# henryxrl/Listening-to-Sound-of-Silence-for-Speech-Denoising

Measured on AMD Instinct MI355X. Metric: utterances/sec (2 s clips), training step: detector + denoiser forward/backward/Adam, higher is better.
Workload: dtype fp16

## Files before the change

### include/sos_hip.h

```cpp
#ifndef SOS_HIP_H
#define SOS_HIP_H

#include <stdint.h>

#ifdef __cplusplus
extern "C" {
#endif

typedef void* sos_stream_t;

enum { SOS_OK = 0, SOS_EINVAL = -22, SOS_ELAUNCH = -5, SOS_ENOSPC = -28 };

enum { SOS_ACT_NONE = 0, SOS_ACT_RELU = 1, SOS_ACT_PRELU = 2, SOS_ACT_SIGMOID = 3 };
enum { SOS_PAD_ZERO = 0, SOS_PAD_REFLECT = 1 };
enum { SOS_DT_BF16 = 0, SOS_DT_BF16X3 = 1, SOS_DT_F32 = 2 };

int sos_abi_version(void);
int sos_struct_size(int which);
const char* sos_last_error(void);
const char* sos_storage_dtype(void);

int64_t sos_stft_matrix_bytes(int n_fft, int hop, int win_length);
int sos_stft_pack_matrix(int n_fft, int hop, int win_length, void* hi , void* lo );
int sos_stft_f32(const float* wave, int64_t batch, int64_t n_samples, int64_t wave_stride,
// ... 18 lines not shown
int sos_crm_target_f32(const float* clean, const float* mix, float* out, int64_t batch, int64_t plane,
                       float a, float b, sos_stream_t stream);

int sos_bits_to_mask(const uint8_t* bits, int64_t batch, int64_t n_frames, double ratio,
                     int64_t n_samples, float* mask, const float* sig, float* masked,
                     const int32_t* clip_frames, const int32_t* clip_samples ,
                     sos_stream_t stream);

int sos_add_signals_f32(const float* signal, const float* noises, const float* snr_db, int64_t batch, int n_noises,
                        int64_t n, float norm, float* mixed, float* signal_out, float* noises_out, sos_stream_t stream);

int sos_threshold_bits(const float* logits, int64_t n, float threshold, uint8_t* bits, float* conf,
                       sos_stream_t stream);
int sos_logit_band_mark(const float* logits, const float* scale, int64_t batch, int64_t n, const int32_t* n_valid,
                        float band_rel, const int32_t* tabs_in, int32_t* tabs_out, int ntab, int32_t* mark, int32_t* count,
                        sos_stream_t stream);

int sos_pack_nchw_to_nhwc(const float* in, int64_t B, int C, int64_t H, int64_t W, void* out, int cs,
                          int dtype, const float* mul ,
                          sos_stream_t stream);
int sos_pack_nchw_wtaps(const float* in, int64_t B, int C, int64_t H, int64_t W, int kw, int pad_left, int pad_mode,
                        const int32_t* clip_w, void* out, int cs, int dtype, const float* mul, sos_stream_t stream);

typedef struct sos_conv_desc {
    const void* in;
    int32_t B, H, W;
    int32_t in_cs;
    int32_t cin_off, cin;
    int32_t in_nseg;
    int32_t in_seg_stride;
    const int32_t* w_gather;
    int32_t Wl;
    const void* wgt;
    int32_t kh, kw, cout, cout_pad;
    int32_t stride, dil_h, dil_w, pad_top, pad_left, pad_mode;
    int32_t Ho, Wo;
    void* out;
    int32_t out_dtype;
    int64_t out_sb, out_sh, out_sw, out_sc;
    int32_t out_c_off;
    int32_t cout_store;
    int64_t out_third;
    const float* scale;
    const float* shift;
    int32_t act;
    const float* act_param;
    int32_t accumulate;
    float* stats;
    int32_t stats_c;
    const int32_t* wl_tab;
    const int32_t* wo_tab;
    int32_t w_gather_stride;
    int32_t t_frames, t_taps, t_pad;
    void* fold_pad_out;
    int32_t fold_pad, fold_H, fold_W, fold_sy, fold_oy, fold_sx, fold_ox, fold_row;
    int64_t fold_third;
    const float* in_scale;
    const float* in_shift;
} sos_conv_desc;

int sos_conv2d_fwd(const sos_conv_desc* desc , sos_stream_t stream);
int64_t sos_conv2d_tile_count(const sos_conv_desc* desc);

int sos_conv2d_tune(const sos_conv_desc* desc, int max_candidates, int iters, float* best_ms,
                    sos_stream_t stream);
int sos_conv2d_tune_save(const char* path);
int sos_conv2d_tune_load(const char* path);

int64_t sos_lstm_pack_bytes(int H, int backward);
int sos_lstm_pack_whh(const float* whh, int H, void* fwd_hi, void* fwd_lo, void* bwd_hi, void* bwd_lo,
                      sos_stream_t stream);
int sos_lstm_bidir_fwd(const float* xproj, const void* wpk_hi, const void* wpk_lo , int64_t B, int64_t T,
                       int H, void* out_bf16, int out_cs, int out_dtype, int64_t out_third,
                       float* save_gates ,
                       float* save_c ,
                       const int32_t* lengths ,
                       sos_stream_t stream);

typedef struct sos_view {
    void* ptr;
    int64_t npix;
    int32_t row, c_off, C, x3;
    int64_t third;
} sos_view;

int sos_bn_stats_blocks(int64_t npix);
int sos_bn_stats(const sos_view* x, float* partial, sos_stream_t stream);
int sos_bn_finalize(const float* partial, int nblk, int C, int64_t count, const float* gamma, const float* beta,
                    float eps, float momentum, float* running_mean, float* running_var, int64_t* num_batches_tracked,
                    float* scale, float* shift, float* save_mean, float* save_invstd, sos_stream_t stream);
int sos_bn_act_apply(const sos_view* x, const float* scale, const float* shift, int act, const float* slope,
                     const sos_view* y, int feat_H, int feat_W, int feat_Wo, const int32_t* gather,
                     sos_stream_t stream);

typedef struct sos_wgrad_desc {
    const void* g;
    int32_t B, Hg, Wg, g_cs, g_off;
    const void* x;
    int32_t Hx, Wx, x_cs, x_off;
    int32_t M, N, kh, kw, stride, dil_h, dil_w, pad_top, pad_left, pad_mode;
    int32_t ksplit;
    float* partial;
    float* dw;
    int32_t accumulate;
    float scale;
    const float* scale_dev;
    int32_t t_frames, t_taps, t_pad, t_cin;
} sos_wgrad_desc;
int64_t sos_wgrad_workspace_bytes(const sos_wgrad_desc* desc);
int sos_conv2d_wgrad(const sos_wgrad_desc* desc, sos_stream_t stream);
int sos_conv2d_wgrad_partial(const sos_wgrad_desc* desc, sos_stream_t stream);
int sos_conv2d_wgrad_reduce(const sos_wgrad_desc* desc, sos_stream_t stream);
int sos_wgrad_tune(const sos_wgrad_desc* desc, int iters, float* best_ms, sos_stream_t stream);
int sos_wgrad_tune_save(const char* path);
int sos_wgrad_tune_load(const char* path);

int sos_bn_bwd(const sos_view* dy, const sos_view* x, const float* scale, const float* shift, const float* mean,
               const float* invstd, const float* gamma, int act, const float* slope, float* partial, float* coef,
               float* dgamma, float* dbeta, float* dslope, const sos_view* dx,
               const float* out_scale ,
               sos_stream_t stream);
int sos_act_bwd_from_y(const sos_view* dy, const sos_view* y, int act, const sos_view* dz, sos_stream_t stream);
int sos_pack_grad_f32(const float* g, const float* y, int act, int64_t outer, int64_t inner, int C, int64_t so,
                      int64_t st, int64_t sc, const sos_view* out, const float* mul ,
                      sos_stream_t stream);
int sos_feat_to_nhwc(const sos_view* feat, int B, int H, int W, int Wo, const int32_t* lo, const int32_t* hi,
                     const sos_view* out, sos_stream_t stream);
int sos_lstm_bidir_bwd(const void* dh_out, int dh_cs, int dh_dtype, int64_t dh_third, const float* gates,
                       const float* csave, const void* wtk_hi, const void* wtk_lo , int64_t B, int64_t T,
                       int H, float* dgates, sos_stream_t stream);
int sos_mse_loss(const float* a, const float* b, int64_t n, float upstream, float* loss, float* grad, float* partial,
                 sos_stream_t stream);
int sos_bce_logits_loss(const float* x, const float* y, int64_t n, float upstream, float* loss, float* grad,
                        float* partial, sos_stream_t stream);
int sos_amax_f32(const float* x, int64_t n, float* amax, sos_stream_t stream);
int sos_loss_scale(const float* amax, float target, float* scale2, const float* guard , sos_stream_t stream);
int sos_scale_f32(float* x, int64_t n, const float* s , sos_stream_t stream);
#define SOS_GUARD_FLOATS 5
#define SOS_GUARD_GROWTH 200
int sos_grad_guard(const float* g, int64_t n, float* guard, int finalize, sos_stream_t stream);
int sos_adam_step(float* p, const float* g, float* m, float* v, int64_t n, float lr, float beta1, float beta2,
                  float eps, float weight_decay, int64_t step, float grad_scale, const float* skip, sos_stream_t stream);

#define SOS_ADAM_CHUNK 16384
typedef struct sos_adam_tensor { float* p; const float* g; float* m; float* v; int64_t n; } sos_adam_tensor;
int sos_adam_multi_step(const sos_adam_tensor* tensors, int n_tensors, const int32_t* chunks, int64_t n_chunks, float lr,
                        float beta1, float beta2, float eps, float weight_decay, int64_t step, float grad_scale,
                        const float* skip , sos_stream_t stream);

typedef struct sos_pack_entry { const int64_t* idx; void* out; int64_t n; } sos_pack_entry;
int sos_gather_pack_multi(const sos_pack_entry* entries, int n_entries, const int32_t* chunks, int64_t n_chunks,
                          sos_stream_t stream);

int sos_reflect_fold(const sos_view* padded, int H, int W, int pad, const sos_view* out, int accumulate,
                     sos_stream_t stream);
int sos_reflect_fold_border(const sos_view* padded, int H, int W, int pad, const sos_view* out, sos_stream_t stream);
int sos_copy_crop(const sos_view* src, int Hs, int Ws, const sos_view* dst, int Hd, int Wd, sos_stream_t stream);

enum { SOS_PCM_S16 = 0, SOS_PCM_S32 = 1, SOS_PCM_F32 = 2, SOS_PCM_U8 = 3 };
int sos_pcm_to_mono_f32(const void* pcm, int format, int channels, int64_t n_frames, float* out, sos_stream_t stream);
int sos_resample_f32(const float* x, int64_t n_in, double ratio, const float* win, int nwin, int num_table,
                     float* out, int64_t n_out, sos_stream_t stream);
#define SOS_RESAMPLE_CHUNK 4096
int sos_resample_batch_f32(const float* x, const int64_t* table, const int64_t* table_host, int nclips, double ratio,
                           const float* win, int nwin, int num_table, float* out, sos_stream_t stream);
int sos_resample_time_segments(double ratio, int64_t n_out, int64_t* k0, double* s0, double* d, int capacity);

int sos_time_stack(const void* in, int64_t B, int T, int64_t HW, int C, int in_cs, int nseg, int kt, void* out,
                   int out_cs, sos_stream_t stream);
int sos_spatial_mean(const void* in, int64_t N, int64_t HW, int C, int in_cs, int nseg, void* out, int64_t out_row,
                     int out_third, int out_c_off, sos_stream_t stream);
int sos_time_unstack(const void* d_stacked, int64_t B, int T, int64_t HW, int C, int st_cs, int nseg, int kt,
                     void* d_in, int in_cs, sos_stream_t stream);
int sos_spatial_mean_bwd(const void* dfeat, int64_t N, int64_t HW, int C, int64_t f_row, int f_third, int f_c_off,
                         int nseg, void* dy, int cs, sos_stream_t stream);

int sos_metric_totals(const float* ref, const float* deg, int64_t n, double* out3, sos_stream_t stream);
int sos_metric_frame_energy(const float* ref, const float* deg, int64_t n, int winlength, int skip, int64_t num_frames,
                            const double* window, double* out, sos_stream_t stream);
int sos_metric_compact(const float* clean, const float* proc, int64_t n, float thr, float* out_clean, float* out_proc,
                       int64_t* count, sos_stream_t stream);
int sos_metric_llr(const float* ref, const float* deg, int64_t n, int winlength, int skip, int64_t num_frames,
                   const double* window, int P, float* out, sos_stream_t stream);
int sos_metric_wss(const float* ref, const float* deg, int64_t n, int winlength, int skip, int64_t num_frames,
                   const double* window, int n_fft, const float* crit_filter, double eps, float* out, sos_stream_t stream);
int sos_metric_l1(const float* output, int64_t n_out, const float* target, int64_t n_t, double* result, sos_stream_t stream);

int64_t sos_metric_batch_workspace_bytes(const int64_t* lengths_host, int nclips, int winlength, int skip, int n_fft);
int sos_metric_batch(const float* clean, const float* noisy, const int64_t* offsets, const int64_t* lengths,
                     const int64_t* lengths_host, int nclips, int winlength, int skip, int n_fft, int P, const double* window,
                     const float* crit_filter, double eps, void* workspace, int64_t workspace_bytes, void* out, int64_t out_bytes,
                     sos_stream_t stream);

int64_t sos_stoi_workspace_bytes(const int64_t* lengths_host, int nclips, int p, int q);
int sos_stoi_batch(const float* x, const float* y, const int64_t* offsets, const int64_t* lengths, const int64_t* lengths_host,
                   int nclips, int p, int q, const double* taps, int ntaps, int extended, void* workspace, int64_t workspace_bytes,
                   double* out, sos_stream_t stream);

enum { SOS_SDR_CORRELATE = 1, SOS_SDR_SOLVE = 2 };
int64_t sos_sdr_workspace_bytes(const int64_t* lengths_host, int nclips, int filter_length);
int sos_sisdr_batch(const float* x, const float* y, const int64_t* offsets, const int64_t* lengths, const int64_t* lengths_host,
                    int nclips, int zero_mean, void* workspace, int64_t workspace_bytes, double* out, sos_stream_t stream);
int sos_sdr_batch(const float* x, const float* y, const int64_t* offsets, const int64_t* lengths, const int64_t* lengths_host,
                  int nclips, int filter_length, int stages, void* workspace, int64_t workspace_bytes, double* out,
                  sos_stream_t stream);

int sos_ragged_stage_f32(const float* x, const int64_t* table, const int64_t* table_host, int nclips, const uint8_t* bits,
                         const double* ratios, const double* ratios_host, int64_t stride, float* wave, float* masked,
                         float* mask, sos_stream_t stream);
int sos_ragged_unpack_f32(const float* rows, int64_t n_rows, int64_t stride, const int64_t* table, const int64_t* table_host,
                          int nentries, float* out, sos_stream_t stream);

int64_t sos_silence_label_workspace_bytes(const int64_t* table_host, int nclips);
int sos_silence_label_batch(const float* x, const int64_t* table, const int64_t* table_host, int nclips, const double* params,
                            const double* params_host, void* workspace, int64_t workspace_bytes, uint8_t* bits, double* energy,
                            double* out, sos_stream_t stream);

#define SOS_MIX_CHUNK 4096
int64_t sos_ragged_mix_workspace_bytes(const int64_t* table_host, int nclips);
int sos_ragged_mix_f32(const float* clips, const int64_t* table, const int64_t* table_host, int nclips, const float* noise,
                       int64_t noise_total, const int64_t* noise_table, const int64_t* noise_table_host, const uint8_t* bits,
                       const double* params, const double* params_host, double norm, void* workspace, int64_t workspace_bytes,
                       float* mixed, float* clean, float* noise_out, double* out, sos_stream_t stream);

int sos_window_stage_f32(const float* x, int64_t total, const int64_t* table, const int64_t* table_host, int nwin, int64_t stride,
                         float* rows, sos_stream_t stream);
int sos_window_stitch_f32(const float* rows, int64_t n_rows, int64_t stride, const int64_t* table, const int64_t* table_host,
                          int nwin, int64_t context, float* out, sos_stream_t stream);

int sos_window_stitch_planes_f32(const float* rows, int planes, int64_t n_rows, int64_t stride, const int64_t* table,
                                 const int64_t* table_host, int nwin, int64_t context, const int64_t* recs,
                                 const int64_t* recs_host, int nrec, int64_t out_total, float* out, sos_stream_t stream);

int sos_window_frames_stitch_f32(const float* rows, int64_t n_rows, int64_t stride, const int64_t* table, const int64_t* table_host,
                                 const int64_t* frames, const int64_t* frames_host, int nwin, const int64_t* recs,
                                 const int64_t* recs_host, const double* ratios, const double* ratios_host, int nrec, int64_t core,
                                 int64_t context, float* out, sos_stream_t stream);
int sos_window_stage_masked_f32(const float* x, const uint8_t* bits, const int64_t* clips, const int64_t* clips_host,
                                const double* ratios, const double* ratios_host, int nrec, const int64_t* table,
                                const int64_t* table_host, int nwin, int64_t stride, float* wave, float* masked,
                                sos_stream_t stream);

int sos_stream_push_f32(const float* flat, int64_t total, const int64_t* table, const int64_t* table_host, int nrows, float* ring,
                        int64_t slots, int64_t cap, sos_stream_t stream);
int sos_stream_stage_f32(const float* ring, int64_t slots, int64_t cap, const int64_t* table, const int64_t* table_host, int nwin,
                         int64_t stride, float* rows, sos_stream_t stream);
int sos_stream_stitch_f32(const float* rows, int64_t n_rows, int64_t stride, const int64_t* table, const int64_t* table_host,
                          int nwin, int64_t slots, int64_t context, float* tail, float* out, int64_t out_stride,
                          sos_stream_t stream);

#ifdef __cplusplus
}
#endif
#endif
```

### listening-to-sound-of-silence-for-speech-denoising_amd/_lib.py

```python
import ctypes as C
import os

_HERE = os.path.dirname(os.path.abspath(__file__))
LIB_PATH = os.environ.get("SOS_HIP_LIB", os.path.join(_HERE, "libsos_hip.so"))
LIB_PATH_F16 = os.environ.get("SOS_HIP_LIB_F16", os.path.join(_HERE, "libsos_hip_f16.so"))

ACT_NONE, ACT_RELU, ACT_PRELU, ACT_SIGMOID = 0, 1, 2, 3
PAD_ZERO, PAD_REFLECT = 0, 1
DT_BF16, DT_BF16X3, DT_F32 = 0, 1, 2
SDR_CORRELATE, SDR_SOLVE = 1, 2


class ConvDesc(C.Structure):
    _fields_ = [
        ("in_", C.c_void_p),
        ("B", C.c_int32), ("H", C.c_int32), ("W", C.c_int32),
        ("in_cs", C.c_int32), ("cin_off", C.c_int32), ("cin", C.c_int32),
        ("in_nseg", C.c_int32), ("in_seg_stride", C.c_int32),
        ("w_gather", C.c_void_p), ("Wl", C.c_int32),
        ("wgt", C.c_void_p),
        ("kh", C.c_int32), ("kw", C.c_int32), ("cout", C.c_int32), ("cout_pad", C.c_int32),
        ("stride", C.c_int32), ("dil_h", C.c_int32), ("dil_w", C.c_int32),
        ("pad_top", C.c_int32), ("pad_left", C.c_int32), ("pad_mode", C.c_int32),
        ("Ho", C.c_int32), ("Wo", C.c_int32),
        ("out", C.c_void_p), ("out_dtype", C.c_int32),
        ("out_sb", C.c_int64), ("out_sh", C.c_int64), ("out_sw", C.c_int64), ("out_sc", C.c_int64),
        ("out_c_off", C.c_int32), ("cout_store", C.c_int32), ("out_third", C.c_int64),
        ("scale", C.c_void_p), ("shift", C.c_void_p),
        ("act", C.c_int32), ("act_param", C.c_void_p), ("accumulate", C.c_int32),
        ("stats", C.c_void_p), ("stats_c", C.c_int32),
        ("wl_tab", C.c_void_p), ("wo_tab", C.c_void_p), ("w_gather_stride", C.c_int32),
        ("t_frames", C.c_int32), ("t_taps", C.c_int32), ("t_pad", C.c_int32),
        ("fold_pad_out", C.c_void_p),
        ("fold_pad", C.c_int32), ("fold_H", C.c_int32), ("fold_W", C.c_int32), ("fold_sy", C.c_int32), ("fold_oy", C.c_int32),
        ("fold_sx", C.c_int32), ("fold_ox", C.c_int32), ("fold_row", C.c_int32), ("fold_third", C.c_int64),
        ("in_scale", C.c_void_p), ("in_shift", C.c_void_p),
    ]


class View(C.Structure):
    _fields_ = [("ptr", C.c_void_p), ("npix", C.c_int64), ("row", C.c_int32), ("c_off", C.c_int32),
                ("C", C.c_int32), ("x3", C.c_int32), ("third", C.c_int64)]


class WgradDesc(C.Structure):
    _fields_ = [("g", C.c_void_p), ("B", C.c_int32), ("Hg", C.c_int32), ("Wg", C.c_int32), ("g_cs", C.c_int32),
                ("g_off", C.c_int32), ("x", C.c_void_p), ("Hx", C.c_int32), ("Wx", C.c_int32), ("x_cs", C.c_int32),
                ("x_off", C.c_int32), ("M", C.c_int32), ("N", C.c_int32), ("kh", C.c_int32), ("kw", C.c_int32),
                ("stride", C.c_int32), ("dil_h", C.c_int32), ("dil_w", C.c_int32), ("pad_top", C.c_int32),
                ("pad_left", C.c_int32), ("pad_mode", C.c_int32), ("ksplit", C.c_int32), ("partial", C.c_void_p),
                ("dw", C.c_void_p), ("accumulate", C.c_int32), ("scale", C.c_float), ("scale_dev", C.c_void_p),
                ("t_frames", C.c_int32), ("t_taps", C.c_int32), ("t_pad", C.c_int32), ("t_cin", C.c_int32)]


_P, _I, _L, _F, _D = C.c_void_p, C.c_int, C.c_int64, C.c_float, C.c_double
ADAM_CHUNK = 16384
GUARD_FLOATS = 5
RESAMPLE_CHUNK = 4096
MIX_CHUNK = 4096
EXPECTED_ABI = 10

SIGNATURES = {
    "sos_abi_version": [],
    "sos_struct_size": [_I],
    "sos_stft_matrix_bytes": [_I, _I, _I],
    "sos_stft_pack_matrix": [_I, _I, _I, _P, _P],
    "sos_stft_f32": [_P, _L, _L, _L, _P, _P, _I, _I, _I, _P, _L, _P, _P],
    "sos_istft_matrix_bytes": [_I, _I, _I],
    "sos_istft_pack_matrix": [_I, _I, _I, _P, _P, _P],
    "sos_istft_f32": [_P, _L, _L, _P, _P, _P, _I, _I, _I, _P, _L, _P, _P],
    "sos_power_law_f32": [_P, _L, _F, _P, _P],
    "sos_crm_apply_f32": [_P, _P, _P, _L, _L, _F, _F, _P],
    "sos_crm_apply_bwd_f32": [_P, _P, _P, _P, _L, _L, _F, _P],
    "sos_crm_target_f32": [_P, _P, _P, _L, _L, _F, _F, _P],
    "sos_bits_to_mask": [_P, _L, _L, _D, _L, _P, _P, _P, _P, _P, _P],
    "sos_threshold_bits": [_P, _L, _F, _P, _P, _P],
    "sos_logit_band_mark": [_P, _P, _L, _L, _P, _F, _P, _P, _I, _P, _P, _P],
    "sos_add_signals_f32": [_P, _P, _P, _L, _I, _L, _F, _P, _P, _P, _P],
    "sos_storage_dtype": [],
    "sos_pack_nchw_to_nhwc": [_P, _L, _I, _L, _L, _P, _I, _I, _P, _P],
    "sos_pack_nchw_wtaps": [_P, _L, _I, _L, _L, _I, _I, _I, _P, _P, _I, _I, _P, _P],
    "sos_conv2d_fwd": [C.POINTER(ConvDesc), _P],
    "sos_conv2d_tune": [C.POINTER(ConvDesc), _I, _I, C.POINTER(C.c_float), _P],
    "sos_conv2d_tune_save": [C.c_char_p],
    "sos_conv2d_tune_load": [C.c_char_p],
    "sos_conv2d_tile_count": [C.POINTER(ConvDesc)],
    "sos_lstm_pack_bytes": [_I, _I],
    "sos_lstm_pack_whh": [_P, _I, _P, _P, _P, _P, _P],
    "sos_lstm_bidir_fwd": [_P, _P, _P, _L, _L, _I, _P, _I, _I, _L, _P, _P, _P, _P],
    "sos_bn_bwd": [C.POINTER(View), C.POINTER(View), _P, _P, _P, _P, _P, _I, _P, _P, _P, _P, _P, _P, C.POINTER(View), _P, _P],
    "sos_act_bwd_from_y": [C.POINTER(View), C.POINTER(View), _I, C.POINTER(View), _P],
    "sos_pack_grad_f32": [_P, _P, _I, _L, _L, _I, _L, _L, _L, C.POINTER(View), _P, _P],
    "sos_feat_to_nhwc": [C.POINTER(View), _I, _I, _I, _I, _P, _P, C.POINTER(View), _P],
    "sos_reflect_fold": [C.POINTER(View), _I, _I, _I, C.POINTER(View), _I, _P],
    "sos_reflect_fold_border": [C.POINTER(View), _I, _I, _I, C.POINTER(View), _P],
    "sos_copy_crop": [C.POINTER(View), _I, _I, C.POINTER(View), _I, _I, _P],
    "sos_lstm_bidir_bwd": [_P, _I, _I, _L, _P, _P, _P, _P, _L, _L, _I, _P, _P],
    "sos_mse_loss": [_P, _P, _L, _F, _P, _P, _P, _P],
    "sos_bce_logits_loss": [_P, _P, _L, _F, _P, _P, _P, _P],
    "sos_grad_guard": [_P, _L, _P, _I, _P],
    "sos_adam_step": [_P, _P, _P, _P, _L, _F, _F, _F, _F, _F, _L, _F, _P, _P],
    "sos_adam_multi_step": [_P, _I, _P, _L, _F, _F, _F, _F, _F, _L, _F, _P, _P],
    "sos_gather_pack_multi": [_P, _I, _P, _L, _P],
    "sos_amax_f32": [_P, _L, _P, _P],
    "sos_loss_scale": [_P, _F, _P, _P, _P],
    "sos_scale_f32": [_P, _L, _P, _P],
    "sos_bn_stats_blocks": [_L],
    "sos_bn_stats": [C.POINTER(View), _P, _P],
    "sos_bn_finalize": [_P, _I, _I, _L, _P, _P, _F, _F, _P, _P, _P, _P, _P, _P, _P, _P],
    "sos_bn_act_apply": [C.POINTER(View), _P, _P, _I, _P, C.POINTER(View), _I, _I, _I, _P, _P],
    "sos_wgrad_workspace_bytes": [C.POINTER(WgradDesc)],
    "sos_conv2d_wgrad": [C.POINTER(WgradDesc), _P],
    "sos_conv2d_wgrad_partial": [C.POINTER(WgradDesc), _P],
    "sos_conv2d_wgrad_reduce": [C.POINTER(WgradDesc), _P],
    "sos_wgrad_tune": [C.POINTER(WgradDesc), _I, C.POINTER(C.c_float), _P],
    "sos_wgrad_tune_save": [C.c_char_p],
    "sos_wgrad_tune_load": [C.c_char_p],
    "sos_pcm_to_mono_f32": [_P, _I, _I, _L, _P, _P],
    "sos_resample_f32": [_P, _L, _D, _P, _I, _I, _P, _L, _P],
    "sos_resample_batch_f32": [_P, _P, _P, _I, _D, _P, _I, _I, _P, _P],
    "sos_resample_time_segments": [_D, _L, _P, _P, _P, _I],
    "sos_time_stack": [_P, _L, _I, _L, _I, _I, _I, _I, _P, _I, _P],
    "sos_spatial_mean": [_P, _L, _L, _I, _I, _I, _P, _L, _I, _I, _P],
    "sos_metric_totals": [_P, _P, _L, _P, _P],
    "sos_metric_frame_energy": [_P, _P, _L, _I, _I, _L, _P, _P, _P],
    "sos_metric_compact": [_P, _P, _L, _F, _P, _P, _P, _P],
    "sos_metric_llr": [_P, _P, _L, _I, _I, _L, _P, _I, _P, _P],
    "sos_metric_wss": [_P, _P, _L, _I, _I, _L, _P, _I, _P, _D, _P, _P],
    "sos_metric_l1": [_P, _L, _P, _L, _P, _P],
    "sos_metric_batch_workspace_bytes": [_P, _I, _I, _I, _I],
    "sos_metric_batch": [_P, _P, _P, _P, _P, _I, _I, _I, _I, _I, _P, _P, _D, _P, _L, _P, _L, _P],
    "sos_stoi_workspace_bytes": [_P, _I, _I, _I],
    "sos_stoi_batch": [_P, _P, _P, _P, _P, _I, _I, _I, _P, _I, _I, _P, _L, _P, _P],
    "sos_sdr_workspace_bytes": [_P, _I, _I],
    "sos_sisdr_batch": [_P, _P, _P, _P, _P, _I, _I, _P, _L, _P, _P],
    "sos_sdr_batch": [_P, _P, _P, _P, _P, _I, _I, _I, _P, _L, _P, _P],
    "sos_ragged_stage_f32": [_P, _P, _P, _I, _P, _P, _P, _L, _P, _P, _P, _P],
    "sos_ragged_unpack_f32": [_P, _L, _L, _P, _P, _I, _P, _P],
    "sos_silence_label_workspace_bytes": [_P, _I],
    "sos_silence_label_batch": [_P, _P, _P, _I, _P, _P, _P, _L, _P, _P, _P, _P],
    "sos_ragged_mix_workspace_bytes": [_P, _I],
    "sos_ragged_mix_f32": [_P, _P, _P, _I, _P, _L, _P, _P, _P, _P, _P, _D, _P, _L, _P, _P, _P, _P, _P],
    "sos_window_stage_f32": [_P, _L, _P, _P, _I, _L, _P, _P],
    "sos_window_stitch_f32": [_P, _L, _L, _P, _P, _I, _L, _P, _P],
    "sos_window_stitch_planes_f32": [_P, _I, _L, _L, _P, _P, _I, _L, _P, _P, _I, _L, _P, _P],
    "sos_window_frames_stitch_f32": [_P, _L, _L, _P, _P, _P, _P, _I, _P, _P, _P, _P, _I, _L, _L, _P, _P],
    "sos_window_stage_masked_f32": [_P, _P, _P, _P, _P, _P, _I, _P, _P, _I, _L, _P, _P, _P],
    "sos_stream_push_f32": [_P, _L, _P, _P, _I, _P, _L, _L, _P],
    "sos_stream_stage_f32": [_P, _L, _L, _P, _P, _I, _L, _P, _P],
    "sos_stream_stitch_f32": [_P, _L, _L, _P, _P, _I, _L, _L, _P, _P, _L, _P],
    "sos_time_unstack": [_P, _L, _I, _L, _I, _I, _I, _I, _P, _I, _P],
    "sos_spatial_mean_bwd": [_P, _L, _L, _I, _L, _I, _I, _I, _P, _I, _P],
}

_libs = {}


def _load(path, want_dtype):
    if not os.path.exists(path):
        raise ImportError(
            f"{path} is missing: build it with `python -c 'import __graft_entry__ as g; g.build()'` "
            "(hipcc --offload-arch=gfx950).  This package has no CPU fallback.")
    import torch
    h = C.CDLL(path)
    for name, argtypes in SIGNATURES.items():
        fn = getattr(h, name)
        fn.argtypes = argtypes
        fn.restype = C.c_int64 if name in ("sos_wgrad_workspace_bytes", "sos_lstm_pack_bytes", "sos_conv2d_tile_count",
                                             "sos_stft_matrix_bytes", "sos_istft_matrix_bytes",
                                             "sos_stoi_workspace_bytes", "sos_metric_batch_workspace_bytes",
                                             "sos_sdr_workspace_bytes", "sos_silence_label_workspace_bytes",
                                             "sos_ragged_mix_workspace_bytes") else C.c_int
    if h.sos_abi_version() != EXPECTED_ABI:
        raise ImportError(f"{path} exports ABI version {h.sos_abi_version()}, this binding was written for {EXPECTED_ABI} "
                          "(the argument lists differ: rebuild the library, or drop the SOS_HIP_LIB / SOS_HIP_LIB_F16 override)")
    h.sos_last_error.restype = C.c_char_p
    h.sos_last_error.argtypes = []
    h.sos_storage_dtype.restype = C.c_char_p
    got = h.sos_storage_dtype().decode()
    if got != want_dtype:
        raise ImportError(f"{path} computes on {got} storage, expected {want_dtype}")
    for which, mirror in ((0, View), (1, ConvDesc), (2, WgradDesc)):
        if h.sos_struct_size(which) != C.sizeof(mirror):
            raise ImportError(f"{path}: {mirror.__name__} is {C.sizeof(mirror)} bytes here but {h.sos_struct_size(which)} in the "
                              "library (include/sos_hip.h and _lib.py have drifted apart, or the library is stale: rebuild it)")
    return h


def lib():
    from . import get_precision
    which = "fp16" if get_precision() == "fp16" else "bf16"
    h = _libs.get(which)
    if h is None:
        h = _libs[which] = _load(LIB_PATH_F16 if which == "fp16" else LIB_PATH, which)
    return h


def check(rc, what=""):
    if rc != 0:
        msg = lib().sos_last_error().decode("utf-8", "replace")
        raise RuntimeError(f"libsos_hip {what} failed (rc={rc}): {msg}")


def stream_ptr():
    import torch
    return C.c_void_p(torch.cuda.current_stream().cuda_stream)


def require_cuda(*tensors):
    for t in tensors:
        if t is not None and not t.is_cuda:
            raise RuntimeError("sos_amd: tensors must live on an MI355X (no CPU fallback); got device "
                               f"{t.device}")


def ptr(t):
    return C.c_void_p(t.data_ptr()) if t is not None else C.c_void_p(0)
```

### listening-to-sound-of-silence-for-speech-denoising_amd/agent.py

```python
import os

import torch
import torch.distributed as dist

from . import _lib as L
from . import transform
from .engine import bump_version

PHASE_TRAINING, PHASE_TESTING = "training", "testing"


class TrainClock(object):

    def __init__(self):
        self.epoch, self.minibatch, self.step = 1, 0, 0

    def tick(self):
        self.minibatch += 1
        self.step += 1

    def tock(self):
        self.epoch += 1
        self.minibatch = 0

    def make_checkpoint(self):
        return {"epoch": self.epoch, "minibatch": self.minibatch, "step": self.step}

    def restore_checkpoint(self, clock_dict):
        self.epoch, self.minibatch, self.step = clock_dict["epoch"], clock_dict["minibatch"], clock_dict["step"]


def _scale_by(grad, g):
    out = grad.clone()
    g = g.detach().reshape(1).to(device=grad.device, dtype=torch.float32)
    L.check(L.lib().sos_scale_f32(L.ptr(out), out.numel(), L.ptr(g), L.stream_ptr()), "sos_scale_f32")
    return out


class _MSE(torch.autograd.Function):
    @staticmethod
    def forward(ctx, a, b):
        L.require_cuda(a, b)
        a, b = a.contiguous().float(), b.contiguous().float()
        loss = torch.empty(1, dtype=torch.float32, device=a.device)
        grad = torch.empty_like(a)
        partial = torch.empty(1024, dtype=torch.float32, device=a.device)
        L.check(L.lib().sos_mse_loss(L.ptr(a), L.ptr(b), a.numel(), 1.0, L.ptr(loss), L.ptr(grad), L.ptr(partial),
                                     L.stream_ptr()), "sos_mse_loss")
        ctx.save_for_backward(grad)
        return loss[0]

    @staticmethod
    def backward(ctx, g):
        (grad,) = ctx.saved_tensors
        return _scale_by(grad, g), None


class _BCE(torch.autograd.Function):
    @staticmethod
    def forward(ctx, x, y):
        L.require_cuda(x, y)
        x, y = x.contiguous().float(), y.contiguous().float()
        loss = torch.empty(1, dtype=torch.float32, device=x.device)
        grad = torch.empty_like(x)
        partial = torch.empty(1024, dtype=torch.float32, device=x.device)
        L.check(L.lib().sos_bce_logits_loss(L.ptr(x), L.ptr(y), x.numel(), 1.0, L.ptr(loss), L.ptr(grad), L.ptr(partial),
                                            L.stream_ptr()), "sos_bce_logits_loss")
        ctx.save_for_backward(grad)
        return loss[0]

    @staticmethod
    def backward(ctx, g):
        (grad,) = ctx.saved_tensors
        return _scale_by(grad, g), None


def mse_loss(a, b):
    return _MSE.apply(a, b)


def bce_with_logits_loss(x, y):
    return _BCE.apply(x, y)


class FusedAdam(torch.optim.Optimizer):

    def __init__(self, params, lr=1e-3, betas=(0.9, 0.999), eps=1e-8, weight_decay=0.0):
        super().__init__(params, dict(lr=lr, betas=betas, eps=eps, weight_decay=weight_decay))
        self.grad_scale = 1.0
        self.guard = None
        self._tables = {}
        self._calls = 0
        self._skip_base = {}

    def _table(self, gi, ps):
        key = tuple((p.data_ptr(), self.state[p]["exp_avg"].data_ptr(), self.state[p]["exp_avg_sq"].data_ptr()) for p in ps)
        ent = self._tables.get(gi)
        if ent is None or ent["key"] != key:
            dev = ps[0].device
            sizes = [p.numel() for p in ps]
            flat_g = torch.empty(sum(sizes), dtype=torch.float32, device=dev)
            rows, chunks, off = [], [], 0
            for ti, p in enumerate(ps):
                st = self.state[p]
                rows.append([p.data_ptr(), flat_g.data_ptr() + 4 * off, st["exp_avg"].data_ptr(), st["exp_avg_sq"].data_ptr(), sizes[ti]])
                chunks += [[ti, c] for c in range((sizes[ti] + L.ADAM_CHUNK - 1) // L.ADAM_CHUNK)]
                off += sizes[ti]
            ent = self._tables[gi] = dict(key=key, flat_g=flat_g, n=len(ps), nchunks=len(chunks),
                                          views=list(torch.split(flat_g, sizes)),
                                          tab=torch.tensor(rows, dtype=torch.int64, device=dev),
                                          chunks=torch.tensor(chunks, dtype=torch.int32, device=dev))
        return ent

    @torch.no_grad()
    def step(self, closure=None):
        work = []
        self._calls += 1
        for gi, group in enumerate(self.param_groups):
            ps = [p for p in group["params"] if p.grad is not None]
            if not ps:
                continue
            L.require_cuda(*ps)
            for p in ps:
                st = self.state[p]
                if not st:
                    st["step"] = torch.zeros((), dtype=torch.float32)
                    st["exp_avg"] = torch.zeros_like(p, memory_format=torch.contiguous_format)
                    st["exp_avg_sq"] = torch.zeros_like(p, memory_format=torch.contiguous_format)
                    if self.guard is not None and self._calls > 1:
                        self._skip_base[p] = self.guard[3:4].clone()
                st["step"] += 1
            ent = self._table(gi, ps)
            torch._foreach_copy_(ent["views"], [p.grad.reshape(-1) for p in ps])
            work.append((group, ps, ent))
        skip = None
        if self.guard is not None and work:
            for k, (_, _, ent) in enumerate(work):
                L.check(L.lib().sos_grad_guard(L.ptr(ent["flat_g"]), ent["flat_g"].numel(), L.ptr(self.guard),
                                               1 if k == len(work) - 1 else 0, L.stream_ptr()), "sos_grad_guard")
            skip = self.guard
        for group, ps, ent in work:
            b1, b2 = group["betas"]
            steps = {int(self.state[p]["step"]) for p in ps}
            if len(steps) == 1 and not any(p in self._skip_base for p in ps):
                L.check(L.lib().sos_adam_multi_step(L.ptr(ent["tab"]), ent["n"], L.ptr(ent["chunks"]), ent["nchunks"],
                                                    float(group["lr"]), float(b1), float(b2), float(group["eps"]),
                                                    float(group["weight_decay"]), steps.pop(), float(self.grad_scale),
                                                    L.ptr(skip), L.stream_ptr()), "sos_adam_multi_step")
            else:
                for p, g in zip(ps, ent["views"]):
                    st = self.state[p]
                    sk = skip
                    if skip is not None and p in self._skip_base:
                        sk = skip.clone()
                        sk[3:4].sub_(self._skip_base[p])
                    L.check(L.lib().sos_adam_step(L.ptr(p), L.ptr(g), L.ptr(st["exp_avg"]), L.ptr(st["exp_avg_sq"]), p.numel(),
                                                  float(group["lr"]), float(b1), float(b2), float(group["eps"]),
                                                  float(group["weight_decay"]), int(st["step"]), float(self.grad_scale),
                                                  L.ptr(sk), L.stream_ptr()), "sos_adam_step")
            for p in ps:
                bump_version(p)
        return None


class GradBucketer:

    def __init__(self, named_params, bucket_bytes=25 * 1024 * 1024, group=None):
        self.group = group
        self.world = dist.get_world_size(group) if dist.is_initialized() else 1
        self.collective = dist.is_initialized() and (self.world > 1 or os.environ.get("SOS_FORCE_BUCKETS") == "1")
        self.shapes = {n: p.shape for n, p in named_params}
        self.params = dict(named_params)
        self.bucket_bytes = bucket_bytes
        self._comm = None
        self._flush_stream = None
        self._inline_streams = set()
        self.profile = os.environ.get("SOS_DDP_PROFILE") == "1"
        self._prof, self._prof_steps, self._prof_host_s = [], 0, 0.0
        self.reset()

    def reset(self):
        self.buckets, self.cur, self.cur_fill, self.handles, self.views = [], None, 0, [], {}
        self.pending, self.pending_streams = ([], []), []

    COMM_MODE = os.environ.get("SOS_DDP_COMM", "inline")
    _shared_comm = {}

    def _comm_stream(self):
        if self.COMM_MODE == "own":
            if self._comm is None:
                self._comm = torch.cuda.Stream()
            return self._comm
        dev = torch.cuda.current_device()
        st = GradBucketer._shared_comm.get(dev)
        if st is None:
            st = GradBucketer._shared_comm[dev] = torch.cuda.Stream()
        self._comm = st
        return st

    def _flush_pending(self):
        if not self.pending[0]:
            return
        streams = {s_ for s_ in self.pending_streams if s_ is not None}
        if streams and self.COMM_MODE == "inline":
            (st,) = streams
            with torch.cuda.stream(st):
                torch._foreach_copy_(self.pending[0], self.pending[1])
        elif streams:
            comm = self._comm_stream()
            for st in streams:
                comm.wait_event(st.record_event())
            for g in self.pending[1]:
                g.record_stream(comm)
            with torch.cuda.stream(comm):
                torch._foreach_copy_(self.pending[0], self.pending[1])
        else:
            torch._foreach_copy_(self.pending[0], self.pending[1])
        self._flush_stream = next(iter(streams)) if streams else None
        self.pending, self.pending_streams = ([], []), []

    def _launch(self, flat, fill):
        self._flush_pending()
        if not flat.is_cuda:
            if self.collective:
                self.handles.append(dist.all_reduce(flat[:fill], op=dist.ReduceOp.SUM, group=self.group, async_op=True))
                if self.profile:
                    self._prof.append((None, None, fill * 4))
            return
        inline = self.COMM_MODE == "inline"
        st = self._flush_stream if inline else self._comm_stream()
        if not inline:
            flat.record_stream(st)
        elif self._flush_stream is not None:
            self._inline_streams.add(self._flush_stream)
        if self.collective:
            with torch.cuda.stream(st):
                e0 = e1 = None
                if self.profile:
                    e0, e1 = torch.cuda.Event(enable_timing=True), torch.cuda.Event(enable_timing=True)
                    e0.record(st)
                if self.COMM_MODE == "own":
                    h = dist.all_reduce(flat[:fill], op=dist.ReduceOp.SUM, group=self.group, async_op=True)
                    self.handles.append(h)
                    if self.profile:
                        h.wait()
                else:
                    dist.all_reduce(flat[:fill], op=dist.ReduceOp.SUM, group=self.group, async_op=False)
                if self.profile:
                    e1.record(st)
                    self._prof.append((e0, e1, fill * 4))

    def ready(self, name, g):
        n = g.numel()
        cap = max(self.bucket_bytes // 4, n)
        here = torch.cuda.current_stream() if g.is_cuda else None
        if (self.COMM_MODE == "inline" and self.cur is not None and self.pending_streams and here is not None
                and self.pending_streams[-1] != here):
            self._launch(self.cur, self.cur_fill)
            self.cur = None
        if self.cur is None or self.cur_fill + n > self.cur.numel():
            if self.cur is not None:
                self._launch(self.cur, self.cur_fill)
            self.cur = torch.empty(cap, dtype=torch.float32, device=g.device)
            self.cur_fill = 0
            self.buckets.append(self.cur)
        v = self.cur[self.cur_fill:self.cur_fill + n]
        self.pending[0].append(v)
        self.pending[1].append(g.reshape(-1))
        self.pending_streams.append(here)
        self.cur_fill += n
        self.views[name] = v.view(self.shapes[name])
        return self.views[name]

    def finalize(self):
        if self.cur is not None and self.cur_fill:
            self._launch(self.cur, self.cur_fill)
        else:
            self._flush_pending()
        if self.profile and self.handles and not any(e is not None for e, _, _ in self._prof[-1:]):
            import time as _time
            t0 = _time.perf_counter()
            for h in self.handles:
                h.wait()
            self._prof_host_s += _time.perf_counter() - t0
        for h in self.handles:
            h.wait()
# ... 17 lines not shown
        ms = 1e3 * self._prof_host_s
        if any(e0 is not None for e0, _, _ in self._prof):
            torch.cuda.synchronize()
            ms = sum(e0.elapsed_time(e1) for e0, e1, _ in self._prof if e0 is not None)
        return {"mode": self.COMM_MODE, "world": self.world, "steps": self._prof_steps, "collective": bool(self.collective),
                "buckets_per_step": len(self._prof) / steps, "bytes_per_step": sum(b for _, _, b in self._prof) / steps,
                "comm_ms_per_step": ms / steps, "bucket_bytes_cap": self.bucket_bytes}

    def reset_keep_views(self):
        self.cur, self.cur_fill, self.handles, self.buckets, self.views = None, 0, [], [], {}
        self.pending, self.pending_streams = ([], []), []


class GradSink(dict):

    def __init__(self, bucketer):
        super().__init__()
        self.bucketer = bucketer

    def __setitem__(self, k, v):
        super().__setitem__(k, self.bucketer.ready(k, v) if self.bucketer is not None else v)


def broadcast_module_state(net, src=0, group=None):
    if not (dist.is_available() and dist.is_initialized()) or dist.get_world_size(group) == 1:
        return
    for t in list(net.parameters()) + list(net.buffers()):
        dist.broadcast(t.data, src=src, group=group)


class BaseAgent(object):

    def __init__(self, net, lr=1e-3, lr_step_size=15, model_dir=None, device=None):
        self.device = torch.device("cuda", torch.cuda.current_device()) if device is None else device
        self.net = net.to(self.device)
        self.clock = TrainClock()
        self.model_dir = model_dir
        self.world = dist.get_world_size() if dist.is_initialized() else 1
        force = dist.is_initialized() and os.environ.get("SOS_FORCE_BUCKETS") == "1"
        self.group = None
        if dist.is_initialized() and (self.world > 1 or force) and os.environ.get("SOS_SHARED_GROUP") != "1":
            self.group = dist.new_group()
        broadcast_module_state(self.net, group=self.group)
        self.optimizer = FusedAdam(self.net.parameters(), lr)
        self.optimizer.grad_scale = 1.0 / self.world
        from .engine import guard_state
        self.optimizer.guard = guard_state(self.net)
        self.scheduler = torch.optim.lr_scheduler.StepLR(self.optimizer, lr_step_size)
        self.bucketer = GradBucketer(list(self.net.named_parameters()), group=self.group) if (self.world > 1 or force) else None
        self.net.grad_sink_factory = (lambda: GradSink(self.bucketer)) if self.bucketer is not None else None

    def save_ckpt(self, name=None):
        path = os.path.join(self.model_dir, f"ckpt_epoch{self.clock.epoch}.pth" if name is None else f"{name}.pth")
        from .engine import guard_state
        guard = guard_state(self.net).detach().cpu().clone()
        skipped = float(guard[3])
        osd = self.optimizer.state_dict()
        if skipped:
            order = [p for g_ in self.optimizer.param_groups for p in g_["params"]]
            base = {i: float(self.optimizer._skip_base[p]) for i, p in enumerate(order) if p in self.optimizer._skip_base}
            osd = dict(osd, state={k: (dict(v, step=v["step"] - (skipped - base.get(k, 0.0))) if "step" in v else v)
                                   for k, v in osd["state"].items()})
        guard[3] = 0.0
        guard[0] = 0.0
        torch.save({"clock": self.clock.make_checkpoint(),
                    "model_state_dict": {k: v.detach().cpu() for k, v in self.net.state_dict().items()},
                    "optimizer_state_dict": osd,
                    "scheduler_state_dict": self.scheduler.state_dict(),
                    "overflow_guard": guard}, path)
        return path

    def load_ckpt(self, name=None):
        name = name if name == "latest" else f"ckpt_epoch{name}"
        path = os.path.join(self.model_dir, f"{name}.pth")
        if not os.path.exists(path):
            raise ValueError("Checkpoint {} not exists.".format(path))
        ck = torch.load(path, map_location=self.device)
        self.net.load_state_dict(ck["model_state_dict"])
        self.optimizer.load_state_dict(ck["optimizer_state_dict"])
        self.optimizer._skip_base.clear()
        self.optimizer._calls = 1 if self.optimizer.state else 0
        for st in self.optimizer.state.values():
            if torch.is_tensor(st.get("step")):
                st["step"] = st["step"].detach().cpu()
        self.scheduler.load_state_dict(ck["scheduler_state_dict"])
        self.clock.restore_checkpoint(ck["clock"])
        from .engine import guard_state
        g = guard_state(self.net)
        g.zero_()
        if ck.get("overflow_guard") is not None:
            g.copy_(ck["overflow_guard"].to(g.device, torch.float32))

    def update_network(self, loss_dict):
        loss = sum(loss_dict.values())
        self.optimizer.zero_grad(set_to_none=True)
        if self.bucketer is not None:
            self.bucketer.reset()
        gate = getattr(self, "backward_gate", None)
        if gate is not None:
            torch.cuda.current_stream().wait_event(gate)
        loss.backward()
        if self.bucketer is not None:
            self.bucketer.finalize()
        self.optimizer.step()

    def update_learning_rate(self):
        self.scheduler.step()

    def train_func(self, data):
        self.net.train()
        outputs, losses = self.forward(data)
        self.update_network(losses)
        return outputs, losses

    def val_func(self, data):
        self.net.eval()
        with torch.no_grad():
            return self.forward(data)


_job_streams = {}


def _job_stream(device, k, prio=0):
    key = (torch.device(device).index if torch.device(device).index is not None else torch.cuda.current_device(), k, prio)
    st = _job_streams.get(key)
    if st is None:
        st = _job_streams[key] = torch.cuda.Stream(device=device, priority=prio)
    return st


def train_concurrent(jobs):
    cur = torch.cuda.current_stream()
    outs = []
    gate = gate_f = None
    mode = os.environ.get("SOS_STREAM_OVERLAP", "split")
    for k, (ag, data) in enumerate(jobs):
        prio = -1 if (k == 0 and os.environ.get("SOS_STREAM_PRIO") == "1") else 0
        ag.stream = _job_stream(ag.device, k, prio)
        ag.stream.wait_stream(cur)
        net = getattr(ag, "net", None)
        ag.backward_gate = None
        if k == 0 and len(jobs) > 1 and getattr(net, "ANNOUNCES_STAGE2_BACKWARD", False) and mode != "full":
            gate = torch.cuda.Event()
            net.after_stage2_backward = gate.record
            if mode == "split" and getattr(net, "ANNOUNCES_LSTM_FORWARD", False):
                gate_f = torch.cuda.Event()
                net.before_lstm_forward = gate_f.record
        elif gate_f is not None:
            ag.stream.wait_event(gate_f)
            ag.backward_gate = gate
        elif gate is not None:
            ag.stream.wait_event(gate)
        try:
            with torch.cuda.stream(ag.stream):
                outs.append(ag.train_func(data))
        finally:
            ag.backward_gate = None
            if k == 0 and gate is not None:
                net.after_stage2_backward = None
                net.before_lstm_forward = None
    for ag, _ in jobs:
        cur.wait_stream(ag.stream)
    return outs


class DetectorAgent(BaseAgent):

    def forward(self, data):
        label = data["label"].to(self.device)
        audio = data["audio"].to(self.device)
        if "frames" in data:
            output = self.net(audio, v=data["frames"].to(self.device))
        else:
            output = self.net(audio) if label.shape[1] == 60 else self.net(audio, label.shape[1])
        return output, {"bce": bce_with_logits_loss(output, label)}


class DenoiserAgent(BaseAgent):

    def forward(self, data):
        mixed, noise = data["mixed"].to(self.device), data["noise"].to(self.device)
        clean, full_noise = data["clean"].to(self.device), data["full_noise"].to(self.device)
        pred_noise, outputs = self.net(mixed, noise)
        rec = transform.batch_fast_icRM_sigmoid(mixed, outputs)
        return (pred_noise, outputs), {"stage1": mse_loss(pred_noise, full_noise), "stage2": mse_loss(rec, clean)}
```

### listening-to-sound-of-silence-for-speech-denoising_amd/common_nets.py

```python
import numpy as np
import torch
import torch.nn as nn

from . import _lib as L
from . import engine as E


class Conv2dBlock(nn.Module):

    def __init__(self, in_channels, out_channels, kernel_size, dilation):
        super().__init__()
        pad = ((kernel_size[0] - 1) // 2 * dilation[0], (kernel_size[1] - 1) // 2 * dilation[1])
        self.block = nn.Sequential(
            nn.Conv2d(in_channels, out_channels, kernel_size, 1, pad, dilation, bias=False),
            nn.BatchNorm2d(out_channels),
            nn.ReLU())

    def forward(self, x):
        raise RuntimeError("Conv2dBlock is executed by its parent network through libsos_hip")


def make_encoder(kernel_sizes, dilations, nf, outf):
    blocks = []
    for i, (k, d) in enumerate(zip(kernel_sizes, dilations)):
        blocks.append(Conv2dBlock(2 if i == 0 else nf, nf, k, d))
    blocks.append(Conv2dBlock(nf, outf, (1, 1), (1, 1)))
    return nn.Sequential(*blocks)


class Conv3dBlock(nn.Module):

    def __init__(self, in_channels, out_channels, kernel_size, stride):
        super().__init__()
        pad = tuple((k - 1) // 2 for k in kernel_size)
        self.block = nn.Sequential(nn.Conv3d(in_channels, out_channels, kernel_size, stride, pad, bias=False),
                                   nn.BatchNorm3d(out_channels), nn.ReLU())

    def forward(self, x):
        raise RuntimeError("Conv3dBlock is executed by its parent network through libsos_hip")


VIDEO_KERNEL_SIZES = [(5, 7, 7), (5, 3, 3), (3, 3, 3), (3, 3, 3), (3, 3, 3), (3, 3, 3), (1, 3, 3)]
VIDEO_STRIDES = [(1, 2, 2), (1, 1, 1), (1, 2, 2), (1, 2, 2), (1, 2, 2), (1, 3, 3), (1, 3, 3)]


def make_video_branch(kernel_sizes, strides, nf=256, outf=256):
    blocks = [Conv3dBlock(3 if i == 0 else nf, nf, k, s) for i, (k, s) in enumerate(zip(kernel_sizes, strides))]
    blocks.append(Conv3dBlock(nf, outf, (1, 1, 1), (1, 1, 1)))
    return nn.Sequential(*blocks)


NO_TEMPORAL_TAPS = __import__("os").environ.get("SOS_VIDEO_STACK") == "1"


def video_plan(enc, x3):
    plan = []
    for blk in enc:
        conv, bn = blk.block[0], blk.block[1]
        kt, kh, kw = conv.kernel_size
        if conv.stride[0] != 1 or conv.stride[1] != conv.stride[2] or conv.dilation != (1, 1, 1):
            raise NotImplementedError("video branch: temporal stride 1, square spatial stride, no dilation")
        O, I = conv.out_channels, conv.in_channels
        w2 = conv.weight.detach().permute(0, 2, 1, 3, 4).reshape(O, kt * I, kh, kw)
        cin_store = E.pad_to(kt * I, 16)
        w = E.pack_weight(w2, cin_store, x3)
        scale, shift = E.fold_bn(bn, w.shape[1])
        plan.append(dict(w=w, scale=scale, shift=shift, kt=kt, kh=kh, kw=kw, stride=conv.stride[1], cin=I, cout=O,
                         cin_store=cin_store, pad=(conv.padding[1], conv.padding[2])))
    return plan


def run_video_branch(plan, frames, B, T, feat, feat_row, feat_third, feat_c_off, x3):
    dev = frames.t.device
    cur, C = frames, 3
    for lp in plan:
        H, W = cur.H, cur.W
        native = lp["kt"] > 1 and C % 16 == 0 and cur.cs == C and lp["cin_store"] == lp["kt"] * C and not NO_TEMPORAL_TAPS
        if native:
            s = lp["stride"]
            Ho = (H + 2 * lp["pad"][0] - lp["kh"]) // s + 1
            Wo = (W + 2 * lp["pad"][1] - lp["kw"]) // s + 1
            dst = E.Act(B * T, Ho, Wo, E.pad_to(lp["cout"], 16), x3, dev)
            E.conv_to_act(cur, 0, C, lp["w"], lp["kh"], lp["kw"], lp["cout"], lp["scale"], lp["shift"], L.ACT_RELU, dst,
                          cout_store=dst.cs, stride=s, pad=lp["pad"], Ho=Ho, Wo=Wo, temporal=(T, lp["kt"]))
            cur, C = dst, lp["cout"]
            continue
        if lp["kt"] > 1 or cur.cs != lp["cin_store"]:
            st = E.Act(B * T, H, W, lp["cin_store"], x3, dev)
            L.check(L.lib().sos_time_stack(L.ptr(cur.t), B, T, H * W, C, cur.cs, cur.nseg, lp["kt"], L.ptr(st.t),
                                           st.cs, L.stream_ptr()), "sos_time_stack")
            cur = st
        s = lp["stride"]
        Ho = (H + 2 * lp["pad"][0] - lp["kh"]) // s + 1
        Wo = (W + 2 * lp["pad"][1] - lp["kw"]) // s + 1
        dst = E.Act(B * T, Ho, Wo, E.pad_to(lp["cout"], 16), x3, dev)
        E.conv_to_act(cur, 0, lp["cin_store"], lp["w"], lp["kh"], lp["kw"], lp["cout"], lp["scale"], lp["shift"],
                      L.ACT_RELU, dst, cout_store=dst.cs, stride=s, pad=lp["pad"], Ho=Ho, Wo=Wo)
        cur, C = dst, lp["cout"]
    L.check(L.lib().sos_spatial_mean(L.ptr(cur.t), B * T, cur.H * cur.W, C, cur.cs, cur.nseg, L.ptr(feat), feat_row,
                                     feat_third, feat_c_off, L.stream_ptr()), "sos_spatial_mean")


def encoder_plan(enc, x3):
    plan = []
    for i, blk in enumerate(enc):
        conv, bn = blk.block[0], blk.block[1]
        wf = E.wfold_spec(conv, conv.padding[1], L.PAD_ZERO) if i == 0 else None
        if wf is not None:
            cin_store = E.pad_to(wf["kw"] * wf["I"], 16)
            w = E.pack_weight(lambda: wf["fold"](conv.weight.detach().float()), cin_store, x3)
            scale, shift = E.fold_bn(bn, w.shape[1])
            plan.append(dict(w=w, scale=scale, shift=shift, kh=conv.kernel_size[0], kw=1, dil=(conv.dilation[0], 1),
                             pad=(conv.padding[0], 0), cout=conv.out_channels, cin_store=cin_store, wtaps=wf["wtaps"]))
            continue
        cin_store = E.pad_to(conv.in_channels, 16)
        w = E.pack_weight(conv.weight, cin_store, x3)
        scale, shift = E.fold_bn(bn, w.shape[1])
        plan.append(dict(w=w, scale=scale, shift=shift, kh=conv.kernel_size[0], kw=conv.kernel_size[1],
                         dil=tuple(conv.dilation), pad=tuple(conv.padding), cout=conv.out_channels,
                         cin_store=cin_store))
    return plan


def pack_encoder_input(plan, x, x3, rag=None, mul=None):
    wt = plan[0].get("wtaps")
    return E.pack_input(x, x3, mul=mul, wtaps=wt, clip_w=(rag.level(0) if (rag is not None and wt is not None) else None))


def run_encoder(plan, a, feat, feat_row, feat_third, feat_c_off, x3, w_gather=None, T_out=None, rag=None, rag_out=None):
    B, H, W = a.B, a.H, a.W
    rk = rag.kw(0) if rag is not None else {}
    cur = a
    bufs = [None, None]
    for i, lp in enumerate(plan[:-1]):
        dst = bufs[i & 1]
        cs = E.pad_to(lp["cout"], 16)
        if dst is None or dst.cs != cs:
            dst = E.Act(B, H, W, cs, x3, a.t.device)
            bufs[i & 1] = dst
        E.conv_to_act(cur, 0, lp["cin_store"], lp["w"], lp["kh"], lp["kw"], lp["cout"], lp["scale"], lp["shift"],
                      L.ACT_RELU, dst, cout_store=cs, dil=lp["dil"], pad=lp["pad"], Ho=H, Wo=W, **rk)
        cur = dst
    lp = plan[-1]
    Wo = W if T_out is None else T_out
    if rag is not None and rag_out is not None:
        rk = dict(wl_tab=rag_out[0], wo_tab=rag_out[0], wg_stride=rag_out[1], valid_cols=sum(rag.n_vframes))
    E.conv(cur, 0, lp["cin_store"], lp["w"], 1, 1, lp["cout"], lp["scale"], lp["shift"], L.ACT_RELU,
           out=feat, out_dtype=L.DT_BF16X3 if x3 else L.DT_BF16, sb=Wo * feat_row, sh=1, sw=feat_row, sc=H,
           c_off=feat_c_off, third=feat_third, Ho=H, Wo=Wo, w_gather=w_gather, **rk)


def lstm_plan(lstm, cin_store, x3):
    H = lstm.hidden_size
    perm, _ = E.lstm_gate_perm(H, lstm.weight_ih_l0.device)
    w_ih = torch.cat([lstm.weight_ih_l0, lstm.weight_ih_l0_reverse], dim=0).detach()[perm]
    bias = torch.cat([lstm.bias_ih_l0 + lstm.bias_hh_l0, lstm.bias_ih_l0_reverse + lstm.bias_hh_l0_reverse]).detach()[perm]
    w = E.pack_weight(w_ih[:, :, None, None], cin_store, x3)
    return dict(w=w, scale=E.pad_vec(torch.ones(8 * H, device=w.device), w.shape[1], 1.0),
                shift=E.pad_vec(bias, w.shape[1]), wpk=E.lstm_pack(lstm, x3), H=H, cin_store=cin_store)


def run_lstm(lp, feat_dims, B, T, x3, device, lengths=None):
    H = lp["H"]
    xproj = torch.empty((B, T, 8 * H), dtype=torch.float32, device=device)
    E.conv(None, 0, lp["cin_store"], lp["w"], 1, 1, 8 * H, lp["scale"], lp["shift"], L.ACT_NONE,
           out=xproj, out_dtype=L.DT_F32, sb=T * 8 * H, sh=0, sw=8 * H, sc=1, Ho=1, Wo=T, in_dims=feat_dims)
    h = E.Act(B, 1, T, E.pad_to(2 * H, 16), x3, device, zero=True)
    E.lstm(xproj, lp["wpk"], B, T, H, h, lengths=lengths)
    return h


def linear_plan(lin, cin_store, x3, absolute=False):
    wt, bias = (lin.weight.abs(), lin.bias.abs()) if absolute else (lin.weight, lin.bias)
    w = E.pack_weight(wt[:, :, None, None], cin_store, x3)
    return dict(w=w, scale=E.pad_vec(torch.ones(lin.out_features, device=w.device), w.shape[1], 1.0),
                shift=E.pad_vec(bias, w.shape[1]), cout=lin.out_features, cin_store=cin_store)


_nearest_tables = {}


def nearest_index(in_size, out_size, device):
    key = (int(in_size), int(out_size), str(device))
    if key not in _nearest_tables:
        scale = np.float32(in_size) / np.float32(out_size)
        idx = np.minimum(np.floor(np.arange(out_size, dtype=np.float32) * scale).astype(np.int64), in_size - 1)
        _nearest_tables[key] = torch.from_numpy(idx.astype(np.int32)).to(device)
    return _nearest_tables[key]


_gather_range_tables = {}


def nearest_ranges(in_size, out_size, device):
    key = (int(in_size), int(out_size), str(device))
    if key not in _gather_range_tables:
        scale = np.float32(in_size) / np.float32(out_size)
        idx = np.minimum(np.floor(np.arange(out_size, dtype=np.float32) * scale).astype(np.int64), in_size - 1)
        cols = np.arange(in_size)
        lo = np.searchsorted(idx, cols, side="left").astype(np.int32)
        hi = np.searchsorted(idx, cols, side="right").astype(np.int32)
        _gather_range_tables[key] = (torch.from_numpy(lo).to(device), torch.from_numpy(hi).to(device))
    return _gather_range_tables[key]


def nearest_index_ragged(rag, n_max, device):
    key = ("nearest", n_max)
    rag = getattr(rag, "base", rag)
    t = rag._tabs.get(key)
    if t is None:
        rows = np.zeros((len(rag.T), n_max), dtype=np.int32)
        for b, (Tc, nc) in enumerate(zip(rag.T, rag.n_vframes)):
            scale = np.float32(Tc) / np.float32(nc)
            rows[b, :nc] = np.minimum(np.floor(np.arange(nc, dtype=np.float32) * scale).astype(np.int64), Tc - 1)
        t = rag._tabs[key] = E.upload(rows, torch.int32, device)
    return t
```

### listening-to-sound-of-silence-for-speech-denoising_amd/csrc/train.hip

```cpp
#include "sos_common.h"

#define LOSS_BLOCKS 1024

__global__ __launch_bounds__(256) void mse_kernel(const float* __restrict__ a, const float* __restrict__ b, long long n,
                                                  float gscale, float* __restrict__ grad, float* __restrict__ partial) {
    __shared__ float red[256];
    float acc = 0.f;
    for (long long i = (long long)blockIdx.x * 256 + threadIdx.x; i < n; i += (long long)gridDim.x * 256) {
        const float d = a[i] - b[i];
        acc = fmaf(d, d, acc);
        if (grad) grad[i] = gscale * d;
    }
    red[threadIdx.x] = acc;
    __syncthreads();
    for (int s = 128; s > 0; s >>= 1) {
        if ((int)threadIdx.x < s) red[threadIdx.x] += red[threadIdx.x + s];
        __syncthreads();
    }
    if (threadIdx.x == 0) partial[blockIdx.x] = red[0];
}

__global__ __launch_bounds__(256) void bce_kernel(const float* __restrict__ x, const float* __restrict__ y, long long n,
                                                  float gscale, float* __restrict__ grad, float* __restrict__ partial) {
    __shared__ float red[256];
// ... 88 lines not shown
    if (!x || !s || n < 1) { sos_set_error("sos_scale_f32: bad args"); return SOS_EINVAL; }
    long long gb = (n + 255) / 256;
    if (gb > 2048) gb = 2048;
    hipLaunchKernelGGL(scale_kernel, dim3((unsigned)gb), dim3(256), 0, (hipStream_t)stream, x, (long long)n, s);
    return sos_check_launch("sos_scale_f32");
}

__global__ __launch_bounds__(256) void grad_guard_kernel(const float* __restrict__ g, long long n, unsigned* __restrict__ raw) {
    int bad = 0;
    for (long long i = (long long)blockIdx.x * 256 + threadIdx.x; i < n; i += (long long)gridDim.x * 256)
        bad |= (__float_as_uint(g[i]) & 0x7f800000u) == 0x7f800000u;
    if (__syncthreads_or(bad) && threadIdx.x == 0) atomicOr(raw, 1u);
}
__global__ void grad_guard_finalize_kernel(float* __restrict__ st) {
    unsigned* raw = (unsigned*)(st + 4);
    const unsigned bad = *raw;
    *raw = 0u;
    float b = st[1] > 0.f ? st[1] : 1.f;
    if (bad) {
        st[0] = 1.f;
        st[3] += 1.f;
        st[2] = 0.f;
        b = fmaxf(0.5f * b, 9.5367431640625e-07f);
    } else {
        st[0] = 0.f;
        st[2] += 1.f;
        if (st[2] >= (float)SOS_GUARD_GROWTH && b < 1.f) { b = fminf(1.f, 2.f * b); st[2] = 0.f; }
    }
    st[1] = b;
}
extern "C" int sos_grad_guard(const float* g, int64_t n, float* guard, int finalize, sos_stream_t stream) {
    if (!g || !guard || n < 1) { sos_set_error("sos_grad_guard: bad args"); return SOS_EINVAL; }
    hipLaunchKernelGGL(grad_guard_kernel, dim3(loss_blocks(n)), dim3(256), 0, (hipStream_t)stream, g, (long long)n,
                       (unsigned*)(guard + 4));
    if (finalize) hipLaunchKernelGGL(grad_guard_finalize_kernel, dim3(1), dim3(1), 0, (hipStream_t)stream, guard);
    return sos_check_launch("sos_grad_guard");
}

__device__ __forceinline__ void adam_applied_steps(const float* __restrict__ skip, float step, float b1, float b2, float& bc1,
                                                   float& bc2_sqrt) {
    if (skip && skip[3] != 0.f) {
        const float applied = fmaxf(step - skip[3], 1.f);
        bc1 = 1.0f - powf(b1, applied);
        bc2_sqrt = sqrtf(1.0f - powf(b2, applied));
    }
}

__global__ void adam_kernel(float* __restrict__ p, const float* __restrict__ g, float* __restrict__ m,
                            float* __restrict__ v, long long n, float lr, float b1, float b2, float eps, float wd,
                            float bc1, float bc2_sqrt, float gscale, const float* __restrict__ skip, float step) {
    if (skip && skip[0] != 0.f) return;
    adam_applied_steps(skip, step, b1, b2, bc1, bc2_sqrt);
    for (long long i = (long long)blockIdx.x * blockDim.x + threadIdx.x; i < n; i += (long long)gridDim.x * blockDim.x) {
        float gi = g[i] * gscale;
        const float pi = p[i];
        if (wd != 0.f) gi = fmaf(wd, pi, gi);
        const float mi = b1 * m[i] + (1.f - b1) * gi;
        const float vi = b2 * v[i] + (1.f - b2) * gi * gi;
        m[i] = mi;
        v[i] = vi;
        const float denom = sqrtf(vi) / bc2_sqrt + eps;
        p[i] = pi - (lr / bc1) * (mi / denom);
    }
}

extern "C" int sos_adam_step(float* p, const float* g, float* m, float* v, int64_t n, float lr, float beta1, float beta2,
                             float eps, float weight_decay, int64_t step, float grad_scale, const float* skip,
                             sos_stream_t stream) {
    if (!p || !g || !m || !v || n < 1 || step < 1) { sos_set_error("sos_adam_step: bad args"); return SOS_EINVAL; }
    const float bc1 = 1.0f - powf(beta1, (float)step);
    const float bc2 = 1.0f - powf(beta2, (float)step);
    long long gb = (n + 255) / 256;
    if (gb > 2048) gb = 2048;
    hipLaunchKernelGGL(adam_kernel, dim3((unsigned)gb), dim3(256), 0, (hipStream_t)stream, p, g, m, v, (long long)n, lr,
                       beta1, beta2, eps, weight_decay, bc1, sqrtf(bc2), grad_scale, skip, (float)step);
    return sos_check_launch("sos_adam_step");
}


struct AdamTensor { float* p; const float* g; float* m; float* v; long long n; };
__global__ __launch_bounds__(256) void adam_multi_kernel(const AdamTensor* __restrict__ tab, const int2* __restrict__ chunks,
                                                         float lr, float b1, float b2, float eps, float wd, float bc1,
                                                         float bc2_sqrt, float gscale, const float* __restrict__ skip, float step) {
    if (skip && skip[0] != 0.f) return;
    adam_applied_steps(skip, step, b1, b2, bc1, bc2_sqrt);
    const int2 c = chunks[blockIdx.x];
    const AdamTensor t = tab[c.x];
    const long long lo = (long long)c.y * SOS_ADAM_CHUNK;
    const long long hi = lo + SOS_ADAM_CHUNK < t.n ? lo + SOS_ADAM_CHUNK : t.n;
    for (long long i = lo + threadIdx.x; i < hi; i += 256) {
        float gi = t.g[i] * gscale;
        const float pi = t.p[i];
        if (wd != 0.f) gi = fmaf(wd, pi, gi);
        const float mi = b1 * t.m[i] + (1.f - b1) * gi;
        const float vi = b2 * t.v[i] + (1.f - b2) * gi * gi;
        t.m[i] = mi;
        t.v[i] = vi;
        const float denom = sqrtf(vi) / bc2_sqrt + eps;
        t.p[i] = pi - (lr / bc1) * (mi / denom);
    }
}

extern "C" int sos_adam_multi_step(const sos_adam_tensor* tensors, int n_tensors, const int32_t* chunks, int64_t n_chunks,
                                   float lr, float beta1, float beta2, float eps, float weight_decay, int64_t step,
                                   float grad_scale, const float* skip, sos_stream_t stream) {
    static_assert(sizeof(sos_adam_tensor) == sizeof(AdamTensor), "sos_adam_tensor layout");
    if (!tensors || !chunks || n_tensors < 1 || n_chunks < 1 || n_chunks > 0x7fffffff || step < 1) {
        sos_set_error("sos_adam_multi_step: bad args");
        return SOS_EINVAL;
    }
    const float bc1 = 1.0f - powf(beta1, (float)step);
    const float bc2 = 1.0f - powf(beta2, (float)step);
    hipLaunchKernelGGL(adam_multi_kernel, dim3((unsigned)n_chunks), dim3(256), 0, (hipStream_t)stream,
                       (const AdamTensor*)tensors, (const int2*)chunks, lr, beta1, beta2, eps, weight_decay, bc1, sqrtf(bc2),
                       grad_scale, skip, (float)step);
    return sos_check_launch("sos_adam_multi_step");
}


struct PackEntry { const long long* idx; bf16_t* out; long long n; };
__global__ __launch_bounds__(256) void gather_pack_kernel(const PackEntry* __restrict__ tab, const int2* __restrict__ chunks) {
    const int2 c = chunks[blockIdx.x];
    const PackEntry e = tab[c.x];
    const long long lo = (long long)c.y * SOS_ADAM_CHUNK;
    const long long hi = lo + SOS_ADAM_CHUNK < e.n ? lo + SOS_ADAM_CHUNK : e.n;
    for (long long i0 = lo + threadIdx.x; i0 < hi; i0 += 4 * 256) {
        long long a[4];
        float v[4];
#pragma unroll
        for (int u = 0; u < 4; ++u) a[u] = i0 + u * 256 < hi ? e.idx[i0 + u * 256] : 0;
#pragma unroll
        for (int u = 0; u < 4; ++u) v[u] = a[u] ? *(const float*)(a[u] > 0 ? a[u] : -a[u]) : 0.f;
#pragma unroll
        for (int u = 0; u < 4; ++u) {
            if (i0 + u * 256 >= hi) continue;
            bf16_t r = 0;
            if (a[u] > 0) r = f2bf(v[u]);
            else if (a[u] < 0) r = f2bf(v[u] - bf2f(f2bf(v[u])));
            e.out[i0 + u * 256] = r;
        }
    }
}
extern "C" int sos_gather_pack_multi(const sos_pack_entry* entries, int n_entries, const int32_t* chunks, int64_t n_chunks,
                                     sos_stream_t stream) {
    static_assert(sizeof(sos_pack_entry) == sizeof(PackEntry), "sos_pack_entry layout");
    if (!entries || !chunks || n_entries < 1 || n_chunks < 1 || n_chunks > 0x7fffffff) {
        sos_set_error("sos_gather_pack_multi: bad args");
        return SOS_EINVAL;
    }
    hipLaunchKernelGGL(gather_pack_kernel, dim3((unsigned)n_chunks), dim3(256), 0, (hipStream_t)stream,
                       (const PackEntry*)entries, (const int2*)chunks);
    return sos_check_launch("sos_gather_pack_multi");
}
```

### listening-to-sound-of-silence-for-speech-denoising_amd/denoiser/networks.py

```python
import torch
import torch.nn as nn

from .. import _lib as L
from .. import get_precision, precision_scope
from .. import common_nets as CN
from .. import engine as E
from .. import train_ops as TO


def get_network(config):
    return JointModel(config)


class DownConvBlock(nn.Module):

    def __init__(self, in_channels, out_channels, kernel_size, stride, dilation=1, norm_fn='bn', act='prelu'):
        super().__init__()
        pad = (kernel_size - 1) // 2 * dilation
        block = [nn.ReflectionPad2d(pad),
                 nn.Conv2d(in_channels, out_channels, kernel_size, stride, 0, dilation, bias=norm_fn is None)]
        if norm_fn == 'bn':
            block.append(nn.BatchNorm2d(out_channels))
        if act == 'prelu':
            block.append(nn.PReLU())
        self.block = nn.Sequential(*block)

    def forward(self, x):
        raise RuntimeError("DownConvBlock is executed by InpaintNet through libsos_hip")


class UpConvBlock(nn.Module):

    def __init__(self, in_channels, out_channels, kernel_size, stride, dilation=1):
        super().__init__()
        pad = (kernel_size - 1) // 2 * dilation
        self.block = nn.Sequential(
            nn.ConvTranspose2d(in_channels, out_channels, kernel_size, stride, pad, dilation, bias=False),
            nn.BatchNorm2d(out_channels),
            nn.PReLU())

    def forward(self, x):
        raise RuntimeError("UpConvBlock is executed by InpaintNet through libsos_hip")


def _down_plan(blk, x3, in_perm=None, first=False):
    conv = blk.block[1]
    k0 = conv.kernel_size[0]
    wf = E.wfold_spec(conv, (k0 - 1) // 2 * conv.dilation[0], L.PAD_REFLECT) if (first and in_perm is None) else None
    if wf is not None:
        cin_store = E.pad_to(wf["kw"] * wf["I"], 16)
        w = E.pack_weight(lambda: wf["fold"](conv.weight.detach().float()), cin_store, x3)
    else:
        cin_store = E.pad_to(conv.in_channels, 16)
        w = E.pack_weight(conv.weight, cin_store, x3, in_perm)
    has_bn = len(blk.block) > 2 and isinstance(blk.block[2], nn.BatchNorm2d)
    if has_bn:
        scale, shift = E.fold_bn(blk.block[2], w.shape[1])
    else:
        scale = E.pad_vec(torch.ones(conv.out_channels, device=w.device), w.shape[1], 1.0)
        shift = E.pad_vec(conv.bias, w.shape[1])
    prelu = blk.block[-1] if isinstance(blk.block[-1], nn.PReLU) else None
    k = conv.kernel_size[0]
    pad = (k - 1) // 2 * conv.dilation[0]
    return dict(w=w, scale=scale, shift=shift, k=k, kw=1 if wf is not None else k, stride=conv.stride[0], dil=conv.dilation[0],
                pad=pad, pad_w=0 if wf is not None else pad, cout=conv.out_channels, cin_store=cin_store,
                wtaps=wf["wtaps"] if wf is not None else None,
                slope=prelu.weight.detach().float() if prelu is not None else None,
                act=L.ACT_PRELU if prelu is not None else L.ACT_NONE)


_PHASE_TAPS = {0: [1], 1: [2, 0]}


def _up_plan(blk, x3):
    ct, bn, prelu = blk.block[0], blk.block[1], blk.block[2]
    assert ct.kernel_size == (3, 3) and ct.stride == (2, 2) and ct.padding == (1, 1) and ct.output_padding == (1, 1)
    cin_store = E.pad_to(ct.in_channels, 16)
    w = ct.weight.detach().float()
    phases = {}
    for ph in (0, 1):
        for pw in (0, 1):
            a, b = _PHASE_TAPS[ph], _PHASE_TAPS[pw]
            sub = w[:, :, a][:, :, :, b].permute(1, 0, 2, 3).contiguous()
            phases[(ph, pw)] = E.pack_weight(sub, cin_store, x3)
    cout_pad = E.pad_to(ct.out_channels, 32)
    scale, shift = E.fold_bn(bn, cout_pad)
    return dict(phases=phases, scale=scale, shift=shift, cout=ct.out_channels, cin_store=cin_store,
                slope=prelu.weight.detach().float())


def _run_down(lp, src, cin_off, dst, c_off, Ho, Wo, rk=None):
    E.conv_to_act(src, cin_off, lp["cin_store"], lp["w"], lp["k"], lp["kw"], lp["cout"], lp["scale"], lp["shift"],
                  lp["act"], dst, c_off=c_off, cout_store=lp["cout"], stride=lp["stride"], dil=(lp["dil"], lp["dil"]),
                  pad=(lp["pad"], lp["pad_w"]), pad_mode=L.PAD_REFLECT, slope=lp["slope"], Ho=Ho, Wo=Wo, **(rk or {}))


def _run_up(lp, src, dst, c_off, rag=None, lsrc=0, ldst=0):
    row = dst.nseg * dst.cs
    for (ph, pw), w in lp["phases"].items():
        Ho = min(src.H, (dst.H - ph + 1) // 2)
        Wo = min(src.W, (dst.W - pw + 1) // 2)
        if Ho <= 0 or Wo <= 0:
            continue
        rk = {}
        if rag is not None:
            ws, wd = rag.widths(lsrc), rag.widths(ldst)
            wo = [min(a, (b - pw + 1) // 2) for a, b in zip(ws, wd)]
            rk = dict(wl_tab=rag.tab(ws), wo_tab=rag.tab(wo), valid_cols=sum(wo))
        E.conv(src, 0, lp["cin_store"], w, 1 + ph, 1 + pw, lp["cout"], lp["scale"], lp["shift"], L.ACT_PRELU,
               out=dst.t, out_dtype=dst.dtype_code, sb=dst.H * dst.W * row, sh=2 * dst.W * row, sw=2 * row, sc=1,
               c_off=c_off, cout_store=lp["cout"], third=dst.cs, slope=lp["slope"], Ho=Ho, Wo=Wo,
               out_elem_offset=(ph * dst.W + pw) * row, **rk)


class InpaintNet(nn.Module):

    def __init__(self):
        super().__init__()
        ch1, ch2, ch3 = 64, 128, 256
        self.down1 = nn.Sequential(DownConvBlock(2, ch1, 5, 1))
        self.down2 = nn.Sequential(DownConvBlock(ch1, ch2, 5, 2), DownConvBlock(ch2, ch2, 5, 1))
        self.down3 = nn.Sequential(DownConvBlock(2, ch1, 5, 1))
        self.down4 = nn.Sequential(DownConvBlock(ch1, ch2, 5, 2), DownConvBlock(ch2, ch2, 5, 1))
        self.mid = nn.Sequential(
            DownConvBlock(ch2 * 2, ch3, 3, 2),
            DownConvBlock(ch3, ch3, 3, 1),
            DownConvBlock(ch3, ch3, 3, 1, dilation=2),
            DownConvBlock(ch3, ch3, 3, 1, dilation=4),
            DownConvBlock(ch3, ch3, 3, 1, dilation=8),
            DownConvBlock(ch3, ch3, 3, 1, dilation=16),
            DownConvBlock(ch3, ch3, 3, 1),
            DownConvBlock(ch3, ch3, 3, 1),
            UpConvBlock(ch3, ch2, 3, 2))
        self.up1 = nn.Sequential(DownConvBlock(ch2 * 2, ch2, 3, 1), UpConvBlock(ch2, ch1, 3, 2))
        self.up2 = nn.Sequential(DownConvBlock(ch1 * 2, ch1, 3, 1), DownConvBlock(ch1, 2, 3, 1, norm_fn=None, act=None))

    def build_plan(self, x3):
        perm_up1 = list(range(128, 256)) + list(range(0, 128))
        return dict(
            down1=_down_plan(self.down1[0], x3, first=True), down2_0=_down_plan(self.down2[0], x3),
            down2_1=_down_plan(self.down2[1], x3), down3=_down_plan(self.down3[0], x3, first=True),
            down4_0=_down_plan(self.down4[0], x3), down4_1=_down_plan(self.down4[1], x3),
            mid=[_down_plan(self.mid[i], x3) for i in range(8)], mid8=_up_plan(self.mid[8], x3),
            up1_0=_down_plan(self.up1[0], x3, perm_up1), up1_1=_up_plan(self.up1[1], x3),
            up2_0=_down_plan(self.up2[0], x3), up2_1=_down_plan(self.up2[1], x3))

    def run(self, plan, x, y, x3, rag=None):
        dev = x.device
        B, _, H, W = x.shape
        H1, W1 = (H + 1) // 2, (W + 1) // 2
        H2, W2 = (H1 + 1) // 2, (W1 + 1) // 2
        cw = rag.level(0) if rag is not None else None
        ax = E.pack_input(x, x3, wtaps=plan["down1"]["wtaps"], clip_w=cw if plan["down1"]["wtaps"] else None)
        ay = E.pack_input(y, x3, wtaps=plan["down3"]["wtaps"], clip_w=cw if plan["down3"]["wtaps"] else None)
        d1 = E.Act(B, H, W, 64, x3, dev)
        U2 = E.Act(B, H, W, 128, x3, dev)
        X = E.Act(B, H1, W1, 384, x3, dev)
        t128 = E.Act(B, H1, W1, 128, x3, dev)
        k = (lambda a, b=None: rag.kw(a, b)) if rag is not None else (lambda a, b=None: None)
        _run_down(plan["down1"], ax, 0, d1, 0, H, W, k(0))
        _run_down(plan["down2_0"], d1, 0, t128, 0, H1, W1, k(0, 1))
        _run_down(plan["down2_1"], t128, 0, X, 0, H1, W1, k(1))
        _run_down(plan["down3"], ay, 0, U2, 64, H, W, k(0))
        _run_down(plan["down4_0"], U2, 64, t128, 0, H1, W1, k(0, 1))
        _run_down(plan["down4_1"], t128, 0, X, 128, H1, W1, k(1))
        m = [E.Act(B, H2, W2, 256, x3, dev), E.Act(B, H2, W2, 256, x3, dev)]
        _run_down(plan["mid"][0], X, 0, m[0], 0, H2, W2, k(1, 2))
        for i in range(1, 8):
            _run_down(plan["mid"][i], m[(i - 1) & 1], 0, m[i & 1], 0, H2, W2, k(2))
        _run_up(plan["mid8"], m[1], X, 256, rag, 2, 1)
        _run_down(plan["up1_0"], X, 128, t128, 0, H1, W1, k(1))
        _run_up(plan["up1_1"], t128, U2, 0, rag, 1, 0)
        _run_down(plan["up2_0"], U2, 0, d1, 0, H, W, k(0))
        lp = plan["up2_1"]
        out = torch.empty((B, 2, H, W), dtype=torch.float32, device=dev)
        E.conv(d1, 0, lp["cin_store"], lp["w"], 3, 3, 2, lp["scale"], lp["shift"], L.ACT_NONE, out=out,
               out_dtype=L.DT_F32, sb=2 * H * W, sh=W, sw=1, sc=H * W, pad=(1, 1), pad_mode=L.PAD_REFLECT, Ho=H, Wo=W,
               **(k(0) or {}))
        return out

    _LAYERS = ["down1.0", "down2.0", "down2.1", "down3.0", "down4.0", "down4.1"] + [f"mid.{i}" for i in range(8)]

    def build_train_plan(self, x3):
        perm_up1 = list(range(128, 256)) + list(range(0, 128))
        P = TO.down_train_plan
        return dict(down1=P(self.down1[0], x3, first=True), down2_0=P(self.down2[0], x3), down2_1=P(self.down2[1], x3),
                    down3=P(self.down3[0], x3, first=True), down4_0=P(self.down4[0], x3), down4_1=P(self.down4[1], x3),
                    mid=[P(self.mid[i], x3) for i in range(8)], mid8=TO.up_train_plan(self.mid[8], x3),
                    up1_0=P(self.up1[0], x3, perm_up1), up1_1=TO.up_train_plan(self.up1[1], x3),
                    up2_0=P(self.up2[0], x3), up2_1=_down_plan(self.up2[1], x3),
                    up2_1_wd=E.pack_weight(lambda: self.up2[1].block[1].weight.detach().float().flip(2, 3).transpose(0, 1).contiguous(),
                                           16, x3))

    def forward_train(self, plan, x, y, x3):
        dev = x.device
        B, _, H, W = x.shape
        H1, W1 = (H + 1) // 2, (W + 1) // 2
        H2, W2 = (H1 + 1) // 2, (W1 + 1) // 2
        ax = E.pack_input(x, x3, wtaps=plan["down1"].get("wtaps"))
        ay = E.pack_input(y, x3, wtaps=plan["down3"].get("wtaps"))
        d1 = E.Act(B, H, W, 64, x3, dev)
        U2 = E.Act(B, H, W, 128, x3, dev)
        X = E.Act(B, H1, W1, 384, x3, dev)
        ta, tb = E.Act(B, H1, W1, 128, x3, dev), E.Act(B, H1, W1, 128, x3, dev)
        F_ = TO.down_forward_train
        tape = []
        tape.append(("down1.0", F_(plan["down1"], ax, 0, d1, 0, H, W, x3)))
        tape.append(("down2.0", F_(plan["down2_0"], d1, 0, ta, 0, H1, W1, x3)))
        tape.append(("down2.1", F_(plan["down2_1"], ta, 0, X, 0, H1, W1, x3)))
        tape.append(("down3.0", F_(plan["down3"], ay, 0, U2, 64, H, W, x3)))
        tape.append(("down4.0", F_(plan["down4_0"], U2, 64, tb, 0, H1, W1, x3)))
        tape.append(("down4.1", F_(plan["down4_1"], tb, 0, X, 128, H1, W1, x3)))
        prev, cin_off = X, 0
        for i in range(8):
            m = E.Act(B, H2, W2, 256, x3, dev)
            tape.append((f"mid.{i}", F_(plan["mid"][i], prev, cin_off, m, 0, H2, W2, x3)))
            prev = m
        tape.append(("mid.8", TO.up_forward_train(plan["mid8"], prev, X, 256, x3)))
        u128 = E.Act(B, H1, W1, 128, x3, dev)
        tape.append(("up1.0", F_(plan["up1_0"], X, 128, u128, 0, H1, W1, x3)))
        tape.append(("up1.1", TO.up_forward_train(plan["up1_1"], u128, U2, 0, x3)))
        u64 = E.Act(B, H, W, 64, x3, dev)
        tape.append(("up2.0", F_(plan["up2_0"], U2, 0, u64, 0, H, W, x3)))
        lp = plan["up2_1"]
        out = torch.empty((B, 2, H, W), dtype=torch.float32, device=dev)
        E.conv(u64, 0, lp["cin_store"], lp["w"], 3, 3, 2, lp["scale"], lp["shift"], L.ACT_NONE, out=out,
               out_dtype=L.DT_F32, sb=2 * H * W, sh=W, sw=1, sc=H * W, pad=(1, 1), pad_mode=L.PAD_REFLECT, Ho=H, Wo=W)
        return out, dict(layers=tape, u64=u64, packed=(ax, ay))

    def backward(self, plan, tape, d_out, grads, x3, prefix="stage1"):
        dev = d_out.t.device
        gb = TO.GradBufs(x3)
        u64 = tape["u64"]
        grads[f"{prefix}.up2.1.block.1.bias"] = TO.colsum(d_out, 0, 2)
        dw = torch.empty((2, 64, 3, 3), dtype=torch.float32, device=dev)
        E.wgrad(d_out, 0, 2, u64, 0, 64, 3, 3, dw, pad=(1, 1), pad_mode=L.PAD_REFLECT, defer=type(grads) is dict)
        grads[f"{prefix}.up2.1.block.1.weight"] = dw
        last = dict(wd=plan["up2_1_wd"], pad=1, k=3, dil=1, stride=1, cin=64)
        TO._reflect_dgrad(last, d_out, u64, 0, gb, x3)
        no_src_grad = {"down1.0", "down3.0"}
        for name, t in reversed(tape["layers"]):
            full = f"{prefix}.{name}"
            if t["kind"] == "up":
                TO.up_backward(t, gb, grads, full, x3)
            else:
                TO.down_backward(t, gb, grads, full, x3, need_src_grad=name not in no_src_grad)

    def forward(self, x, y):
        raise RuntimeError("call InpaintNet through JointModel (libsos_hip path)")


class ContextAggNet(nn.Module):

    def __init__(self, kernel_sizes, dilations, freq_bins=256, nf=96):
        super().__init__()
        self.encoder_x = CN.make_encoder(kernel_sizes, dilations, nf, 8)
        self.encoder_n = CN.make_encoder(kernel_sizes, dilations, nf // 2, 4)
        self.lstm = nn.LSTM(input_size=8 * freq_bins + 4 * freq_bins, hidden_size=200, bidirectional=True)
        self.fc = nn.Sequential(nn.Linear(400, 600), nn.ReLU(True), nn.Linear(600, 600), nn.ReLU(True),
                                nn.Linear(600, freq_bins * 2), nn.Sigmoid())
        self.freq_bins = freq_bins

    def build_plan(self, x3):
        return dict(enc_x=CN.encoder_plan(self.encoder_x, x3), enc_n=CN.encoder_plan(self.encoder_n, x3),
                    lstm=CN.lstm_plan(self.lstm, 12 * self.freq_bins, x3),
                    fc0=CN.linear_plan(self.fc[0], 400, x3), fc2=CN.linear_plan(self.fc[2], E.pad_to(600, 16), x3),
                    fc4=CN.linear_plan(self.fc[4], E.pad_to(600, 16), x3))

    def start_x(self, plan, x, x3, rag, side):
        B, _, F, T = x.shape
        nseg = 3 if x3 else 1
        nfeat = 12 * F
        feat = (torch.empty if rag is None else torch.zeros)((B, T, nseg * nfeat), dtype=E.act_dtype(), device=x.device)
        cur = torch.cuda.current_stream(x.device)
        side.wait_stream(cur)
        with torch.cuda.stream(side):
            CN.run_encoder(plan["enc_x"], CN.pack_encoder_input(plan["enc_x"], x, x3, rag), feat, nseg * nfeat, nfeat, 0, x3, rag=rag)
        return dict(feat=feat, side=side, x=x, x3=x3, mode=get_precision())

    def run(self, plan, x, n, x3, rag=None, started=None):
        dev = x.device
        B, _, F, T = x.shape
        nseg = 3 if x3 else 1
        nfeat = 12 * F
        lengths = rag.level(0) if rag is not None else None
        if started is not None:
            feat = started["feat"]
        else:
            feat = (torch.empty if rag is None else torch.zeros)((B, T, nseg * nfeat), dtype=E.act_dtype(), device=dev)
            CN.run_encoder(plan["enc_x"], CN.pack_encoder_input(plan["enc_x"], x, x3, rag), feat, nseg * nfeat, nfeat, 0, x3, rag=rag)
        CN.run_encoder(plan["enc_n"], CN.pack_encoder_input(plan["enc_n"], n, x3, rag), feat, nseg * nfeat, nfeat, 8, x3, rag=rag)
        if started is not None:
            torch.cuda.current_stream(dev).wait_stream(started["side"])
        h = CN.run_lstm(plan["lstm"], (feat, B, 1, T, nfeat, nseg), B, T, x3, dev, lengths=lengths)
        f0, f2, f4 = plan["fc0"], plan["fc2"], plan["fc4"]
        a0 = E.Act(B, 1, T, E.pad_to(600, 16), x3, dev)
        a1 = E.Act(B, 1, T, E.pad_to(600, 16), x3, dev)
        E.conv_to_act(h, 0, f0["cin_store"], f0["w"], 1, 1, 600, f0["scale"], f0["shift"], L.ACT_RELU, a0,
                      cout_store=a0.cs, Ho=1, Wo=T)
        E.conv_to_act(a0, 0, f2["cin_store"], f2["w"], 1, 1, 600, f2["scale"], f2["shift"], L.ACT_RELU, a1,
                      cout_store=a1.cs, Ho=1, Wo=T)
        out = torch.empty((B, 2, F, T), dtype=torch.float32, device=dev)
        E.conv(a1, 0, f4["cin_store"], f4["w"], 1, 1, 2 * F, f4["scale"], f4["shift"], L.ACT_SIGMOID, out=out,
               out_dtype=L.DT_F32, sb=2 * F * T, sh=0, sw=1, sc=T, Ho=1, Wo=T)
        return out

    def build_train_plan(self, x3):
        return dict(enc_x=TO.encoder_train_plan(self.encoder_x, x3), enc_n=TO.encoder_train_plan(self.encoder_n, x3),
                    lstm=TO.lstm_train_plan(self.lstm, 12 * self.freq_bins, x3),
                    fc0=TO.linear_train_plan(self.fc[0], 400, x3), fc2=TO.linear_train_plan(self.fc[2], E.pad_to(600, 16), x3),
                    fc4=TO.linear_train_plan(self.fc[4], E.pad_to(600, 16), x3))

    def forward_train(self, plan, x, n, x3, before_lstm=None, side=None):
        dev = x.device
        B, _, F, T = x.shape
        nseg = 3 if x3 else 1
        nfeat = 12 * F
        feat = torch.empty((B, T, nseg * nfeat), dtype=E.act_dtype(), device=dev)
        fs = dict(t=feat, row=nseg * nfeat, third=nfeat, H=F, W=T, Wo=T, gather=None, x3=x3)
        n_extra = None
        if side is not None:
            cur = torch.cuda.current_stream(dev)
            side.wait_stream(cur)
            with torch.cuda.stream(side):
                if callable(n):
                    n, n_extra = n()
                tn = TO.encoder_forward_train(plan["enc_n"], CN.pack_encoder_input(plan["enc_n"], n, x3), dict(fs, c_off=8), x3)
            tx = TO.encoder_forward_train(plan["enc_x"], CN.pack_encoder_input(plan["enc_x"], x, x3), dict(fs, c_off=0), x3)
            cur.wait_stream(side)
        else:
            if callable(n):
                n, n_extra = n()
            tx = TO.encoder_forward_train(plan["enc_x"], CN.pack_encoder_input(plan["enc_x"], x, x3), dict(fs, c_off=0), x3)
            tn = TO.encoder_forward_train(plan["enc_n"], CN.pack_encoder_input(plan["enc_n"], n, x3), dict(fs, c_off=8), x3)
        if before_lstm is not None:
            before_lstm()
        h, tl = TO.lstm_forward_train(plan["lstm"], (feat, B, 1, T, nfeat, nseg), B, T, x3, dev)
        f0, f2, f4 = plan["fc0"], plan["fc2"], plan["fc4"]
        a0 = E.Act(B, 1, T, E.pad_to(600, 16), x3, dev)
        a1 = E.Act(B, 1, T, E.pad_to(600, 16), x3, dev)
        E.conv_to_act(h, 0, f0["cin_store"], f0["w"], 1, 1, 600, f0["scale"], f0["shift"], L.ACT_RELU, a0,
                      cout_store=a0.cs, Ho=1, Wo=T)
        E.conv_to_act(a0, 0, f2["cin_store"], f2["w"], 1, 1, 600, f2["scale"], f2["shift"], L.ACT_RELU, a1,
                      cout_store=a1.cs, Ho=1, Wo=T)
        out = torch.empty((B, 2, F, T), dtype=torch.float32, device=dev)
        E.conv(a1, 0, f4["cin_store"], f4["w"], 1, 1, 2 * F, f4["scale"], f4["shift"], L.ACT_SIGMOID, out=out,
               out_dtype=L.DT_F32, sb=2 * F * T, sh=0, sw=1, sc=T, Ho=1, Wo=T)
        return out, dict(tx=tx, tn=tn, tl=tl, h=h, a0=a0, a1=a1, out=out, dims=(B, F, T), n=n, n_extra=n_extra)

    def backward(self, plan, tape, g_out, grads, x3, prefix="stage2", side=None, tail=None, before_join=None):
        B, F, T = tape["dims"]
        dev = g_out.device
        nseg = 3 if x3 else 1
        dz4 = E.Act(B, 1, T, 2 * F, x3, dev)
        TO.pack_grad(g_out.contiguous().float(), tape["out"], L.ACT_SIGMOID, B, T, 2 * F, 2 * F * T, 1, T, dz4)
        d_a1 = TO.linear_backward(plan["fc4"], tape["a1"], dz4, grads, f"{prefix}.fc.4", x3, dev)
        dz2 = E.Act(B, 1, T, tape["a1"].cs, x3, dev, zero=True)
        TO.act_bwd_from_y(d_a1, tape["a1"], L.ACT_RELU, dz2, 600)
        d_a0 = TO.linear_backward(plan["fc2"], tape["a0"], dz2, grads, f"{prefix}.fc.2", x3, dev)
        dz0 = E.Act(B, 1, T, tape["a0"].cs, x3, dev, zero=True)
        TO.act_bwd_from_y(d_a0, tape["a0"], L.ACT_RELU, dz0, 600)
        dh = TO.linear_backward(plan["fc0"], tape["h"], dz0, grads, f"{prefix}.fc.0", x3, dev)
        dfeat = TO.lstm_backward(plan["lstm"], tape["tl"], dh, grads, f"{prefix}.lstm", B, T, x3, dev)
        nfeat = 12 * F
        if side is not None:
            cur = torch.cuda.current_stream(dev)
            side.wait_stream(cur)
            with torch.cuda.stream(side):
                dyn = TO.feat_grad_to_nhwc(dfeat, nseg * nfeat, nfeat, 8, 4, B, F, T, T, x3)
                d_n = TO.encoder_backward(plan["enc_n"], tape["tn"], dyn, grads, f"{prefix}.encoder_n", x3, need_input_grad=True)
                if tail is not None:
                    tail(d_n)
            dyx = TO.feat_grad_to_nhwc(dfeat, nseg * nfeat, nfeat, 0, 8, B, F, T, T, x3)
            TO.encoder_backward(plan["enc_x"], tape["tx"], dyx, grads, f"{prefix}.encoder_x", x3)
            if before_join is not None:
                before_join()
            cur.wait_stream(side)
            return d_n
        dyx = TO.feat_grad_to_nhwc(dfeat, nseg * nfeat, nfeat, 0, 8, B, F, T, T, x3)
        TO.encoder_backward(plan["enc_x"], tape["tx"], dyx, grads, f"{prefix}.encoder_x", x3)
        dyn = TO.feat_grad_to_nhwc(dfeat, nseg * nfeat, nfeat, 8, 4, B, F, T, T, x3)
        d_n = TO.encoder_backward(plan["enc_n"], tape["tn"], dyn, grads, f"{prefix}.encoder_n", x3, need_input_grad=True)
        if tail is not None:
            tail(d_n)
        return d_n

    def forward(self, x, n):
        raise RuntimeError("call ContextAggNet through JointModel (libsos_hip path)")


class _JointTrainFn(torch.autograd.Function):

    @staticmethod
    def forward(ctx, net, x, n, *params):
        (n_pred, out), tape = net._forward_train(x, n)
        ctx.net, ctx.tape = net, tape
        return n_pred, out

    @staticmethod
    def backward(ctx, g_npred, g_out):
        with E.deferred_reductions():
            grads = ctx.net._backward(ctx.tape, g_npred, g_out)
        ctx.tape = None
        if getattr(ctx.net, "grad_sink_factory", None) is not None:
            return (None, None, None) + (None,) * len(list(ctx.net.parameters()))
        return (None, None, None) + tuple(grads[name].reshape(p.shape) for name, p in ctx.net.named_parameters())


class JointModel(nn.Module):

    ANNOUNCES_STAGE2_BACKWARD = True
    ANNOUNCES_LSTM_FORWARD = True

    def __init__(self, config):
        super().__init__()
        self.stage1 = InpaintNet()
        self.stage2 = ContextAggNet(config.kernel_sizes, config.dilations)
        self._cache = E.PlanCache()
        self._tcache = E.PlanCache(record=True)

    def _build_plan(self):
        x3 = E.is_x3()
        return dict(x3=x3, s1=self.stage1.build_plan(x3), s2=self.stage2.build_plan(x3))

    def _build_train_plan(self):
        x3 = E.is_x3()
        return dict(x3=x3, s1=self.stage1.build_train_plan(x3), s2=self.stage2.build_train_plan(x3))

    BRANCH_STREAMS = __import__("os").environ.get("SOS_BRANCH_STREAMS", "1") != "0"

    _SIDE_STREAMS = {}

    def _side_stream(self, dev):
        if not self.BRANCH_STREAMS or torch.cuda.is_current_stream_capturing():
            return None
        cur = torch.cuda.current_stream(dev)
        key = (dev.index, cur.cuda_stream)
        ss = JointModel._SIDE_STREAMS
        if key not in ss:
            ss[key] = torch.cuda.Stream(device=dev)
        self.__dict__["_used_side_stream"] = True
        return ss[key]

    def _forward_train(self, x, n):
        plan = self._tcache.get(self, self._build_train_plan)
        x3 = plan["x3"]
        out, t2 = self.stage2.forward_train(plan["s2"], x, lambda: self.stage1.forward_train(plan["s1"], n, x, x3), x3,
                                            before_lstm=getattr(self, "before_lstm_forward", None), side=self._side_stream(x.device))
        n_pred, t1 = t2.pop("n"), t2.pop("n_extra")
        return (n_pred, out), dict(plan=plan, t1=t1, t2=t2, x3=x3, mode=get_precision())

    def _backward(self, tape, g_npred, g_out):
        g_npred = g_npred.contiguous().float() if g_npred is not None else None
        g_out = g_out.contiguous().float() if g_out is not None else None
        E.check_tape_weights(self, tape)
        with precision_scope(tape.get("mode")), E.backward_scale(g_npred, g_out, guard=E.guard_state(self)):
            return self._backward_scaled(tape, g_npred, g_out)

    def _backward_scaled(self, tape, g_npred, g_out):
        plan, x3 = tape["plan"], tape["x3"]
        factory = getattr(self, "grad_sink_factory", None)
        grads = factory() if factory is not None else {}
        dev = tape["t2"]["out"].device
        B, F, T = tape["t2"]["dims"]
        if g_out is None:
            g_out = torch.zeros((B, 2, F, T), dtype=torch.float32, device=dev)
        def stage1_tail(d_np):
            if g_npred is not None:
                direct = E.pack_input(g_npred, x3, mul=E.cur_gs().mul)
                TO.reflect_fold(direct, F, T, 0, d_np, 0, 2, accumulate=True)
            self.stage1.backward(plan["s1"], tape["t1"], d_np, grads, x3)

        side = self._side_stream(dev)
        hook = getattr(self, "after_stage2_backward", None)
        if side is None:
            d_np = self.stage2.backward(plan["s2"], tape["t2"], g_out, grads, x3)
            if hook is not None:
                hook()
            stage1_tail(d_np)
        else:
            self.stage2.backward(plan["s2"], tape["t2"], g_out, grads, x3, side=side, tail=stage1_tail, before_join=hook)
        return grads

    @torch.no_grad()
    def begin_x(self, x, rag=None):
        if self.training or x.dim() != 4:
            return None
        side = self._side_stream(x.device)
        if side is None:
            return None
        plan = self._cache.get(self, self._build_plan)
        x = x.contiguous().float()
        return self.stage2.start_x(plan["s2"], x, plan["x3"], rag, side)

    def forward(self, x, n, rag=None, started=None):
        L.require_cuda(x, n)
        if x.dim() != 4 or x.shape[1] != 2 or x.shape != n.shape:
            raise ValueError(f"expected two (B, 2, F, T) inputs, got {tuple(x.shape)} and {tuple(n.shape)}")
        if rag is not None and (self.training or len(rag.T) != x.shape[0] or max(rag.T) != x.shape[3]):
            raise ValueError("ragged batches are an inference feature; rag must describe this batch")
        if self.training:
            return _JointTrainFn.apply(self, x.contiguous().float(), n.contiguous().float(), *self.parameters())
        plan = self._cache.get(self, self._build_plan)
        x3 = plan["x3"]
        x = x.contiguous().float()
        n = n.contiguous().float()
        if started is not None and (started["x"].data_ptr() != x.data_ptr() or started["x3"] != x3 or
                                    started.get("mode", get_precision()) != get_precision()):
            raise ValueError("forward(started=): the handle belongs to another input or precision mode")
        n_pred = self.stage1.run(plan["s1"], n, x, x3, rag)
        out = self.stage2.run(plan["s2"], x, n_pred, x3, rag, started=started)
        return n_pred, out
```

### listening-to-sound-of-silence-for-speech-denoising_amd/detector/networks.py

```python
import torch
import torch.nn as nn

from .. import _lib as L
from .. import detector_precision, precision_scope
from .. import common_nets as CN
from .. import engine as E
from .. import train_ops as TO


def get_network(video=False):
    return AudioVisualNet(video=video)


class _TrainFn(torch.autograd.Function):

    @staticmethod
    def forward(ctx, net, s, n, v, *params):
        mode = detector_precision()
        with precision_scope(mode):
            out, tape = net._forward_train(s, n, v)
        tape["mode"] = mode
        ctx.net, ctx.tape = net, tape
        return out

    @staticmethod
    def backward(ctx, g):
        with E.deferred_reductions():
            grads = ctx.net._backward(ctx.tape, g)
        ctx.tape = None
        if getattr(ctx.net, "grad_sink_factory", None) is not None:
            return (None, None, None, None) + (None,) * len(list(ctx.net.parameters()))
        return (None, None, None, None) + tuple(grads[name].reshape(p.shape) for name, p in ctx.net.named_parameters())


class AudioVisualNet(nn.Module):

    def __init__(self, freq_bins=256, time_bins=178, nf=96, video=False):
        super().__init__()
        audio_kernel_sizes = [(1, 7), (7, 1)] + [(5, 5)] * 9
        audio_dilations = [(1, 1), (1, 1), (1, 1), (2, 1), (4, 1), (8, 1), (16, 1), (32, 1), (1, 1), (2, 2), (4, 4)]
        self.encoder_audio = CN.make_encoder(audio_kernel_sizes, audio_dilations, nf=48, outf=8)
        self.video_feat = 256 if video else 0
        self.lstm = nn.LSTM(input_size=8 * freq_bins + self.video_feat, hidden_size=100, bidirectional=True)
        self.fc1 = nn.Sequential(nn.Linear(200, 100), nn.ReLU(True), nn.Linear(100, 1))
        if video:
            self.encoder_video = CN.make_video_branch(CN.VIDEO_KERNEL_SIZES, CN.VIDEO_STRIDES, nf=128, outf=256)
        self.freq_bins = freq_bins
        self._caches = {}
        self._tcache = E.PlanCache(record=True)

    @property
    def _cache(self):
        from .. import get_precision
        c = self._caches.get(get_precision())
        if c is None:
            c = self._caches[get_precision()] = E.PlanCache()
        return c

    def _build_plan(self):
        x3 = E.is_x3()
        return dict(x3=x3,
                    enc=CN.encoder_plan(self.encoder_audio, x3),
                    vid=CN.video_plan(self.encoder_video, x3) if self.video_feat else None,
                    lstm=CN.lstm_plan(self.lstm, 8 * self.freq_bins + self.video_feat, x3),
                    fc0=CN.linear_plan(self.fc1[0], E.pad_to(200, 16), x3),
                    fc2=CN.linear_plan(self.fc1[2], E.pad_to(100, 16), x3),
                    fc2abs=CN.linear_plan(self.fc1[2], E.pad_to(100, 16), x3, absolute=True))

    def _build_train_plan(self):
        x3 = E.is_x3()
        return dict(x3=x3, enc=TO.encoder_train_plan(self.encoder_audio, x3),
                    vid=TO.video_train_plan(self.encoder_video, x3) if self.video_feat else None,
                    lstm=TO.lstm_train_plan(self.lstm, 8 * self.freq_bins + self.video_feat, x3),
                    fc0=TO.linear_train_plan(self.fc1[0], E.pad_to(200, 16), x3),
                    fc2=TO.linear_train_plan(self.fc1[2], E.pad_to(100, 16), x3))

    def _forward_train(self, s, n, v=None):
        plan = self._tcache.get(self, self._build_train_plan)
        x3 = plan["x3"]
        dev = s.device
        B, _, F, T = s.shape
        nseg = 3 if x3 else 1
        nfeat = 8 * F + self.video_feat
        a = CN.pack_encoder_input(plan["enc"], s, x3)
        feat = torch.empty((B, n, nseg * nfeat), dtype=E.act_dtype(), device=dev)
        gather = CN.nearest_index(T, n, dev)
        fspec = dict(t=feat, row=nseg * nfeat, third=nfeat, c_off=0, H=F, W=T, Wo=n, gather=gather, x3=x3)
        tape_enc = TO.encoder_forward_train(plan["enc"], a, fspec, x3)
        tape_vid = None
        if self.video_feat:
            frames = E.pack_input(v.float().permute(0, 2, 1, 3, 4).reshape(B * n, 3, v.shape[3], v.shape[4]), x3)
            tape_vid = TO.video_forward_train(plan["vid"], frames, B, n, feat, nseg * nfeat, nfeat, 8 * F, x3)
        h, tape_lstm = TO.lstm_forward_train(plan["lstm"], (feat, B, 1, n, nfeat, nseg), B, n, x3, dev)
        f0, f2 = plan["fc0"], plan["fc2"]
        m = E.Act(B, 1, n, E.pad_to(f0["cout"], 16), x3, dev, zero=True)
        E.conv_to_act(h, 0, f0["cin_store"], f0["w"], 1, 1, f0["cout"], f0["scale"], f0["shift"], L.ACT_RELU, m,
                      cout_store=m.cs, Ho=1, Wo=n)
        out = torch.empty((B, n), dtype=torch.float32, device=dev)
        E.conv(m, 0, f2["cin_store"], f2["w"], 1, 1, 1, f2["scale"], f2["shift"], L.ACT_NONE, out=out,
               out_dtype=L.DT_F32, sb=n, sh=0, sw=1, sc=1, Ho=1, Wo=n)
        tape = dict(plan=plan, enc=tape_enc, vid=tape_vid, lstm=tape_lstm, h=h, m=m, gather=gather, dims=(B, F, T, n), x3=x3)
        return out, tape

    def _backward(self, tape, g):
        g = g.contiguous().float()
        E.check_tape_weights(self, tape)
        with precision_scope(tape.get("mode")), E.backward_scale(g, guard=E.guard_state(self)):
            return self._backward_scaled(tape, g)

    def _backward_scaled(self, tape, g):
        plan, x3 = tape["plan"], tape["x3"]
        B, F, T, n = tape["dims"]
        dev = g.device
        factory = getattr(self, "grad_sink_factory", None)
        grads = factory() if factory is not None else {}
        dz2 = E.Act(B, 1, n, 16, x3, dev, zero=True)
        TO.pack_grad(g, None, L.ACT_NONE, B, n, 1, n, 1, 1, dz2)
        d_m = TO.linear_backward(plan["fc2"], tape["m"], dz2, grads, "fc1.2", x3, dev)
        dz0 = E.Act(B, 1, n, tape["m"].cs, x3, dev, zero=True)
        TO.act_bwd_from_y(d_m, tape["m"], L.ACT_RELU, dz0, plan["fc0"]["cout"])
        dh = TO.linear_backward(plan["fc0"], tape["h"], dz0, grads, "fc1.0", x3, dev)
        dfeat = TO.lstm_backward(plan["lstm"], tape["lstm"], dh, grads, "lstm", B, n, x3, dev)
        lo, hi = CN.nearest_ranges(T, n, dev)
        nseg = 3 if x3 else 1
        nfeat = 8 * F + self.video_feat
        dy = TO.feat_grad_to_nhwc(dfeat, nseg * nfeat, nfeat, 0, 8, B, F, T, n, x3,
                                  lo, hi)
        TO.encoder_backward(plan["enc"], tape["enc"], dy, grads, "encoder_audio", x3)
        if self.video_feat:
            TO.video_backward(plan["vid"], tape["vid"], dfeat, nseg * nfeat, nfeat, 8 * F, grads, "encoder_video", B, n, x3)
        return grads

    def forward(self, s, v_num_frames=60, v=None, rag=None, before_lstm=None, return_scale=False):
        L.require_cuda(s, v)
        if s.dim() != 4 or s.shape[1] != 2 or s.shape[2] != self.freq_bins:
            raise ValueError(f"expected (B, 2, {self.freq_bins}, T) input, got {tuple(s.shape)}")
        if self.video_feat:
            if v is None or v.dim() != 5 or v.shape[0] != s.shape[0] or v.shape[1] != 3:
                raise ValueError("the audio-visual variant needs video frames v of shape (B, 3, Tv, H, W)")
            v_num_frames = v.shape[2]
        elif v is not None:
            raise ValueError("this network was built without the video branch (get_network(video=True))")
        if rag is not None and (self.training or self.video_feat):
            raise ValueError("ragged batches are an inference feature of the audio-only network")
        if return_scale and self.training:
            raise ValueError("return_scale is an inference feature")
        if self.training:
            return _TrainFn.apply(self, s.contiguous().float(), int(v_num_frames),
                                  v.contiguous().float() if v is not None else None, *self.parameters())
        with precision_scope(detector_precision()):
            return self._forward_eval(s, int(v_num_frames), v, rag, before_lstm, return_scale)

    def _forward_eval(self, s, n, v, rag, before_lstm=None, return_scale=False):
        plan = self._cache.get(self, self._build_plan)
        x3 = plan["x3"]
        dev = s.device
        B, _, F, T = s.shape
        a = CN.pack_encoder_input(plan["enc"], s, x3, rag)
        nseg = 3 if x3 else 1
        nfeat = 8 * F + self.video_feat
        lengths = None
        if rag is None:
            feat = torch.empty((B, n, nseg * nfeat), dtype=E.act_dtype(), device=dev)
            gather = CN.nearest_index(T, n, dev)
            CN.run_encoder(plan["enc"], a, feat, nseg * nfeat, nfeat, 0, x3, w_gather=gather, T_out=n)
        else:
            if len(rag.T) != B or max(rag.T) != T or max(rag.n_vframes) != n:
                raise ValueError("rag does not describe this batch")
            feat = torch.zeros((B, n, nseg * nfeat), dtype=E.act_dtype(), device=dev)
            gather = CN.nearest_index_ragged(rag, n, dev)
            lengths = rag.tab(rag.n_vframes)
            CN.run_encoder(plan["enc"], a, feat, nseg * nfeat, nfeat, 0, x3, w_gather=gather, T_out=n, rag=rag,
                           rag_out=(lengths, n))
        if self.video_feat:
            frames = E.pack_input(v.float().permute(0, 2, 1, 3, 4).reshape(B * n, 3, v.shape[3], v.shape[4]), x3)
            CN.run_video_branch(plan["vid"], frames, B, n, feat, nseg * nfeat, nfeat, 8 * F, x3)
        if before_lstm is not None:
            before_lstm()
        h = CN.run_lstm(plan["lstm"], (feat, B, 1, n, nfeat, nseg), B, n, x3, dev, lengths=lengths)
        f0, f2 = plan["fc0"], plan["fc2"]
        m = E.Act(B, 1, n, E.pad_to(f0["cout"], 16), x3, dev)
        E.conv_to_act(h, 0, f0["cin_store"], f0["w"], 1, 1, f0["cout"], f0["scale"], f0["shift"], L.ACT_RELU, m,
                      cout_store=m.cs, Ho=1, Wo=n)
        out = torch.empty((B, n), dtype=torch.float32, device=dev)
        E.conv(m, 0, f2["cin_store"], f2["w"], 1, 1, 1, f2["scale"], f2["shift"], L.ACT_NONE, out=out,
# ... 9 lines not shown
```

### listening-to-sound-of-silence-for-speech-denoising_amd/engine.py

```python
import ctypes as C

import torch

from . import _lib as L
from . import get_precision

BN_EPS = 1e-5


class LaunchProfiler:

    def __init__(self, only=None):
        self.only = only
        self.records = {}

    def bracket(self, sig, flops):
        if self.only is not None and sig != self.only:
            return None
        s, e = torch.cuda.Event(enable_timing=True), torch.cuda.Event(enable_timing=True)
        self.records.setdefault(sig, [flops, []])[1].append((s, e))
        s.record()
        return e

    def summary(self):
# ... 137 lines not shown
        _TLS.gs = self.prev
        return False


def cur_gs():
    return getattr(_TLS, "gs", NO_SCALE)


def guard_state(net):
    dev = next(net.parameters()).device
    g = net.__dict__.get("_sos_guard")
    if g is None or g.device != dev:
        g = net.__dict__["_sos_guard"] = torch.zeros(L.GUARD_FLOATS, dtype=torch.float32, device=dev)
    return g


WFOLD = _os.environ.get("SOS_WFOLD", "1") != "0"


def pack_input(x, x3=None, mul=None, wtaps=None, clip_w=None):
    L.require_cuda(x)
    x3 = is_x3() if x3 is None else x3
    x = x.contiguous().float()
    B, Cc, H, W = x.shape
    if wtaps is not None:
        kw, pad_left, pad_mode = wtaps
        a = Act(B, H, W, pad_to(kw * Cc, 16), x3, x.device)
        L.check(L.lib().sos_pack_nchw_wtaps(L.ptr(x), B, Cc, H, W, kw, pad_left, pad_mode, L.ptr(clip_w), L.ptr(a.t),
                                            a.nseg * a.cs, a.dtype_code, L.ptr(mul), L.stream_ptr()), "sos_pack_nchw_wtaps")
        return a
    a = Act(B, H, W, pad_to(Cc, 16), x3, x.device)
    L.check(L.lib().sos_pack_nchw_to_nhwc(L.ptr(x), B, Cc, H, W, L.ptr(a.t), a.nseg * a.cs, a.dtype_code,
                                          L.ptr(mul), L.stream_ptr()), "sos_pack_nchw_to_nhwc")
    return a


def wfold_spec(conv, pad_left, pad_mode):
    O, I, kh, kw = conv.weight.shape
    if (not WFOLD or kw < 2 or kw * I > 16 or conv.dilation[1] != 1 or conv.stride[1] != 1 or conv.stride[0] != 1):
        return None
    return dict(kw=kw, I=I, wtaps=(kw, pad_left, pad_mode),
                fold=lambda w: w.permute(0, 3, 1, 2).reshape(O, kw * I, kh, 1),
                unfold=lambda dw: dw.reshape(O, kw, I, kh).permute(0, 2, 3, 1).contiguous())


def pack_weight(w, cin_store, x3, in_perm=None):
    rec = getattr(_TLS, "pack_rec", None)
    if rec is not None and rec.mode == "replay":
        return rec.next_out()
    if callable(w):
        w = w()
    O, I, kh, kw = w.shape
    w = w.detach().float()
    if in_perm is not None:
        w = w[:, in_perm]
    wp = w.permute(2, 3, 0, 1).reshape(kh * kw, O, I)
    Op = pad_to(O, 32)
    full = torch.zeros((kh * kw, Op, cin_store), dtype=torch.float32, device=w.device)
    full[:, :O, :I] = wp
    if rec is not None and rec.mode == "index":
        rec.idx.append(torch.cat([full, -full, full], dim=2).contiguous() if x3 else full.contiguous())
        return full
    hi = full.to(act_dtype())
    if not x3:
        out = hi.contiguous()
    else:
        lo = (full - hi.float()).to(act_dtype())
        out = torch.cat([hi, lo, hi], dim=2).contiguous()
    if rec is not None and rec.mode == "value":
        rec.outs.append(out)
    return out


class PackRecorder:

    ENABLED = _os.environ.get("SOS_PACK_GATHER", "1") != "0"

    def __init__(self, module, build):
        self.mode, self.outs, self.idx, self.k, self.ok = "value", [], [], 0, False
        params = [p for p in module.parameters()]
        prev = getattr(_TLS, "pack_rec", None)
        _TLS.pack_rec = self
        try:
            self.plan = build()
            if not self.ENABLED or not self.outs or sum(p.numel() for p in params) >= (1 << 24):
                return
            saved, start = [], 0
            starts = []
            for p in params:
                saved.append(p.data)
                starts.append(start)
                p.data = torch.arange(start + 1, start + 1 + p.numel(), dtype=torch.float32, device=p.device).reshape(p.shape)
                start += p.numel()
            self.mode = "index"
            try:
                build()
            finally:
                for p, d in zip(params, saved):
                    p.data = d
        finally:
            _TLS.pack_rec = prev
            self.mode = "idle"
        if len(self.idx) != len(self.outs) or any(i.shape != o.shape for i, o in zip(self.idx, self.outs)):
            return
        dev = self.outs[0].device
        ptrs = torch.tensor([p.data_ptr() for p in params], dtype=torch.int64, device=dev)
        st = torch.tensor(starts, dtype=torch.int64, device=dev)
        tabs, rows, chunks = [], [], []
        for ei, (ids, out) in enumerate(zip(self.idx, self.outs)):
            a = ids.reshape(-1).abs().round().to(torch.int64)
            pi = torch.bucketize(a, st, right=False) - 1
            pi = pi.clamp_(min=0)
            addr = ptrs[pi] + 4 * (a - 1 - st[pi])
            addr = torch.where(a == 0, torch.zeros_like(addr), torch.where(ids.reshape(-1) < 0, -addr, addr)).contiguous()
            tabs.append(addr)
            rows.append([addr.data_ptr(), out.data_ptr(), out.numel()])
            chunks += [[ei, c] for c in range((out.numel() + L.ADAM_CHUNK - 1) // L.ADAM_CHUNK)]
        self.idx = None
        self.tabs = tabs
        self.table = torch.tensor(rows, dtype=torch.int64, device=dev)
        self.chunks = torch.tensor(chunks, dtype=torch.int32, device=dev)
        self.n, self.nchunks = len(rows), len(chunks)
        keep = [o.clone() for o in self.outs]
        for o in self.outs:
            o.zero_()
        self.refresh()
        self.ok = all(torch.equal(a, b) for a, b in zip(self.outs, keep))
        if not self.ok:
            for o, kcopy in zip(self.outs, keep):
                o.copy_(kcopy)

    def refresh(self):
        L.check(L.lib().sos_gather_pack_multi(L.ptr(self.table), self.n, L.ptr(self.chunks), self.nchunks, L.stream_ptr()),
                "sos_gather_pack_multi")

    def next_out(self):
        o = self.outs[self.k]
        self.k += 1
        return o

    def replay(self, build):
        self.refresh()
        prev = getattr(_TLS, "pack_rec", None)
        _TLS.pack_rec, self.mode, self.k = self, "replay", 0
        try:
            plan = build()
        finally:
            _TLS.pack_rec, self.mode = prev, "idle"
        if self.k != len(self.outs):
            raise RuntimeError("PackRecorder: the plan builder changed its pack_weight sequence")
        return plan


def pad_vec(v, n, fill=0.0):
    out = torch.full((n,), fill, dtype=torch.float32, device=v.device)
    out[:v.numel()] = v.detach().float().reshape(-1)
    return out


def fold_bn(bn, cout_pad):
    scale = bn.weight.detach().float() * torch.rsqrt(bn.running_var.detach().float() + bn.eps)
    shift = bn.bias.detach().float() - bn.running_mean.detach().float() * scale
    return pad_vec(scale, cout_pad, 1.0), pad_vec(shift, cout_pad, 0.0)


def conv(src, cin_off, cin, wgt, kh, kw, cout, scale, shift, act, *, out, out_dtype, sb, sh, sw, sc,
         Ho, Wo, c_off=0, cout_store=None, third=0, stride=1, dil=(1, 1), pad=(0, 0), pad_mode=L.PAD_ZERO,
         slope=None, w_gather=None, out_elem_offset=0, in_dims=None, accumulate=False, stats_c=0, wl_tab=None,
         wo_tab=None, wg_stride=0, valid_cols=None, temporal=None, fold=None, in_bn=None):
    d = L.ConvDesc()
    if in_dims is None:
        t, B, H, W, cs, nseg = src.t, src.B, src.H, src.W, src.cs, src.nseg
    else:
        t, B, H, W, cs, nseg = in_dims
    Bp, Wop = B, Wo
    if (FLATTEN_1X1 and kh == 1 and kw == 1 and stride == 1 and pad == (0, 0) and H == 1 and Ho == 1 and Wo == W and B > 1
            and w_gather is None and wl_tab is None and temporal is None and fold is None and not stats_c and sb == Wo * sw
            and B * W * nseg * cs * 2 < 0xfff00000 and B * Wo * sw < 0x7ffffff0):
        B, W, Wo = 1, B * W, B * Wo
    d.in_ = t.data_ptr()
    d.B, d.H, d.W = B, H, W
    d.in_cs = nseg * cs
    d.cin_off, d.cin, d.in_nseg, d.in_seg_stride = cin_off, cin, nseg, cs
    if w_gather is not None:
        d.w_gather = w_gather.data_ptr()
        d.Wl = w_gather.numel()
    else:
        d.w_gather = None
        d.Wl = W
    d.wgt = wgt.data_ptr()
    d.kh, d.kw, d.cout, d.cout_pad = kh, kw, cout, wgt.shape[1]
    d.stride, d.dil_h, d.dil_w = stride, dil[0], dil[1]
    d.pad_top, d.pad_left, d.pad_mode = pad[0], pad[1], pad_mode
    d.Ho, d.Wo = Ho, Wo
    esize = 4 if out_dtype == L.DT_F32 else 2
    d.out = out.data_ptr() + out_elem_offset * esize
    d.out_dtype = out_dtype
    d.out_sb, d.out_sh, d.out_sw, d.out_sc = sb, sh, sw, sc
    d.out_c_off = c_off
    d.cout_store = cout if cout_store is None else cout_store
    d.out_third = third
    d.scale, d.shift = (scale.data_ptr(), shift.data_ptr()) if scale is not None else (None, None)
    d.act = act
    d.act_param = slope.data_ptr() if slope is not None else None
    d.accumulate = 1 if accumulate else 0
    if temporal is not None and temporal[1] > 1:
        d.t_frames, d.t_taps, d.t_pad = temporal[0], temporal[1], (temporal[1] - 1) // 2
    if wl_tab is not None:
        d.wl_tab, d.wo_tab, d.w_gather_stride = wl_tab.data_ptr(), wo_tab.data_ptr(), wg_stride
    if in_bn is not None:
        d.in_scale, d.in_shift = in_bn[0].data_ptr(), in_bn[1].data_ptr()
    if fold is not None:
        fa, fp, fH, fW, fsy, foy, fsx, fox = fold
        d.fold_pad_out, d.fold_pad, d.fold_H, d.fold_W = fa.t.data_ptr(), fp, fH, fW
        d.fold_sy, d.fold_oy, d.fold_sx, d.fold_ox = fsy, foy, fsx, fox
        d.fold_row, d.fold_third = fa.nseg * fa.cs, fa.cs
    _load_tune_cache()
    if AUTOTUNE:
        key = (B, H, W, d.Wl, cin, d.in_nseg, d.cout_pad, cout, kh, kw, stride, dil, Ho, Wo, out_dtype, sc == 1, pad_mode,
               w_gather is not None, d.t_taps)
        if key not in _tuned and not torch.cuda.is_current_stream_capturing():
            _tuned.add(key)
            if accumulate or fold is not None:
                scratch = torch.empty_like(out)
                real_out, real_acc = d.out, d.accumulate
                d.out = scratch.data_ptr() + out_elem_offset * esize
                d.accumulate = 0
                L.check(L.lib().sos_conv2d_tune(C.byref(d), TUNE_CANDIDATES, 3, None, L.stream_ptr()), "sos_conv2d_tune")
                d.out, d.accumulate = real_out, real_acc
            else:
                L.check(L.lib().sos_conv2d_tune(C.byref(d), TUNE_CANDIDATES, 3, None, L.stream_ptr()), "sos_conv2d_tune")
    end = None
    if PROFILER is not None or _LAUNCH_LOG is not None:
        cols = Bp * Wop if valid_cols is None else valid_cols
        kin = d.in_nseg * max(1, d.t_taps) * cin
        sig = ("conv", kh, kw, dil[0], dil[1], stride, kin, cout, Bp, Ho, Wop) + (() if valid_cols is None else ("ragged", cols))
        if _LAUNCH_LOG is not None:
            _log_launch("conv", sig, 2.0 * Ho * cols * cout * kin * kh * kw)
        if PROFILER is not None:
            end = PROFILER.bracket(sig, 2.0 * Ho * cols * cout * kin * kh * kw)
    stats = None
    if stats_c:
        tiles = L.lib().sos_conv2d_tile_count(C.byref(d))
        if tiles < 1:
            raise RuntimeError("sos_conv2d_tile_count: " + (L.lib().sos_last_error() or b"").decode())
        stats = (torch.empty((2, stats_c, tiles), dtype=torch.float32, device=out.device), int(tiles))
        d.stats, d.stats_c = stats[0].data_ptr(), stats_c
    L.check(L.lib().sos_conv2d_fwd(C.byref(d), L.stream_ptr()), "sos_conv2d_fwd")
    if end is not None:
        end.record()
    return stats


def conv_to_act(src, cin_off, cin, wgt, kh, kw, cout, scale, shift, act, dst, c_off=0, cout_store=None, **kw_):
    row = dst.nseg * dst.cs
    return conv(src, cin_off, cin, wgt, kh, kw, cout, scale, shift, act, out=dst.t, out_dtype=dst.dtype_code,
                sb=dst.H * dst.W * row, sh=dst.W * row, sw=row, sc=1, c_off=c_off,
                cout_store=cout if cout_store is None else cout_store, third=dst.cs, **kw_)


def lstm_gate_perm(H, device):
    n = torch.arange(8 * H, device=device)
    d, r = n // (4 * H), n % (4 * H)
    perm = d * 4 * H + (r % 4) * H + r // 4
    inv = torch.empty_like(perm)
    inv[perm] = n
    return perm, inv


def lstm_pack(lstm_mod, x3):
    H = lstm_mod.hidden_size
    whh = torch.stack([lstm_mod.weight_hh_l0.detach(), lstm_mod.weight_hh_l0_reverse.detach()]).float().contiguous()
    L.require_cuda(whh)
    nf, nb = L.lib().sos_lstm_pack_bytes(H, 0), L.lib().sos_lstm_pack_bytes(H, 1)
    if nf < 0:
        raise RuntimeError(f"LSTM hidden size {H} not supported (multiple of 4, <= 256)")
    mk = lambda n: torch.empty(n // 2, dtype=torch.bfloat16, device=whh.device)
    pk = dict(fh=mk(nf), bh=mk(nb), fl=mk(nf) if x3 else None, bl=mk(nb) if x3 else None)
    L.check(L.lib().sos_lstm_pack_whh(L.ptr(whh), H, L.ptr(pk["fh"]), L.ptr(pk["fl"]), L.ptr(pk["bh"]), L.ptr(pk["bl"]),
                                      L.stream_ptr()), "sos_lstm_pack_whh")
    return pk


def lstm(xproj, wpk, B, T, H, out_act, save_gates=None, save_c=None, lengths=None):
    L.check(L.lib().sos_lstm_bidir_fwd(L.ptr(xproj), L.ptr(wpk["fh"]), L.ptr(wpk["fl"]), B, T, H, L.ptr(out_act.t),
                                       out_act.nseg * out_act.cs, out_act.dtype_code, out_act.cs,
                                       L.ptr(save_gates), L.ptr(save_c), L.ptr(lengths), L.stream_ptr()), "sos_lstm_bidir_fwd")


def upload(values, dtype, device):
    h = torch.as_tensor(values, dtype=dtype)
    if torch.cuda.is_current_stream_capturing():
        return h.to(device)
    hp = torch.empty(h.shape, dtype=dtype, pin_memory=True)
    hp.copy_(h)
    return hp.to(device, non_blocking=True)


class Ragged:

    def __init__(self, T, device, n_vframes=None, n_samples=None):
        self.T = [int(t) for t in T]
        self.device = device
        self.n_vframes = None if n_vframes is None else [int(n) for n in n_vframes]
        self.n_samples = None if n_samples is None else [int(n) for n in n_samples]
        self._tabs = {}

    def widths(self, level):
        w = self.T
        for _ in range(level):
            w = [(x + 1) // 2 for x in w]
        return w

    def tab(self, widths):
        key = tuple(int(x) for x in widths)
        t = self._tabs.get(key)
        if t is None:
            t = self._tabs[key] = upload(key, torch.int32, self.device)
        return t

    def level(self, k):
        return self.tab(self.widths(k))

    def kw(self, lin, lout=None):
        lout = lin if lout is None else lout
        return dict(wl_tab=self.level(lin), wo_tab=self.level(lout), valid_cols=sum(self.widths(lout)))


class MaskedRagged(Ragged):

    def __init__(self, base, mark, tabs):
        super().__init__(base.T, base.device, n_vframes=base.n_vframes, n_samples=base.n_samples)
        self.base, self.mark = base, mark
        self._tabs.update(tabs)
        for k, v in base._tabs.items():
            if isinstance(k, tuple) and k and isinstance(k[0], str):
                self._tabs.setdefault(k, v)

    def tab(self, widths):
        key = tuple(int(x) for x in widths)
        t = self._tabs.get(key)
        if t is None:
            t = self._tabs[key] = self.base.tab(widths) * self.mark
        return t


_band_count = {}


def band_count(device):
    key = str(device)
    if key not in _band_count:
        _band_count[key] = torch.zeros(2, dtype=torch.int32, device=device)
    return _band_count[key]


def mask_ragged(base, logits, band_rel, width_lists, scale=None):
    B, n = logits.shape
    if scale is not None and (scale.shape != logits.shape or scale.dtype != torch.float32 or not scale.is_contiguous()):
        raise ValueError("mask_ragged: scale must be a contiguous float32 tensor of the logits' shape")
    tabs_in = torch.stack([base.tab(w) for w in width_lists]).contiguous()
    tabs_out = torch.empty_like(tabs_in)
    mark = torch.empty(B, dtype=torch.int32, device=logits.device)
    nv = base.tab(base.n_vframes) if base.n_vframes is not None else None
    L.check(L.lib().sos_logit_band_mark(L.ptr(logits), L.ptr(scale), B, n, L.ptr(nv), float(band_rel), L.ptr(tabs_in), L.ptr(tabs_out),
                                        len(width_lists), L.ptr(mark), L.ptr(band_count(logits.device)), L.stream_ptr()),
            "sos_logit_band_mark")
    tabs = {tuple(int(x) for x in w): tabs_out[k] for k, w in enumerate(width_lists)}
    return MaskedRagged(base, mark, tabs), mark


class PlanCache:

    def __init__(self, record=False):
        self.key = None
        self.plan = None
        self.rec = None
        self.record = record
        self.rec_failed = set()

    def get(self, module, build):
        ts = list(module.parameters()) + list(module.buffers())
        base = (get_precision(), str(ts[0].device), tuple(t.data_ptr() for t in ts), tuple(tuple(t.shape) for t in ts))
        key = (base, tuple(t._version for t in ts))
        if key != self.key:
            with torch.no_grad():
                if self.rec is not None and self.rec.ok and self.rec_base == base:
                    self.plan = self.rec.replay(build)
                elif self.record and base not in self.rec_failed:
                    self.rec, self.rec_base = PackRecorder(module, build), base
                    self.plan = self.rec.plan
                    self.rec.plan = None
                    if not self.rec.ok:
                        self.rec_failed.add(base)
                else:
                    self.plan = build()
            self.key = key
            if isinstance(self.plan, dict):
                self.plan["_wver"] = tuple(p._version for p in module.parameters())
        return self.plan


def check_tape_weights(module, tape):
    want = tape["plan"].get("_wver")
    if want is not None and want != tuple(p._version for p in module.parameters()):
        raise RuntimeError("sos_amd: the parameters changed (optimizer step / load_state_dict) between this forward pass and "
                           "its backward pass; run backward before stepping the optimizer")


def view(act, c_off=0, C=None, third_index=None):
    v = L.View()
    v.ptr = act.t.data_ptr()
    v.npix = act.B * act.H * act.W
    v.row = act.nseg * act.cs
# ... 169 lines not shown
```

### listening-to-sound-of-silence-for-speech-denoising_amd/train_ops.py

```python
import ctypes
import os

import numpy as np
import torch

from . import _lib as L
from . import engine as E




FUSED_STATS = __import__("os").environ.get("SOS_FUSED_STATS", "1") != "0"
FUSED_STATS_UNET = __import__("os").environ.get("SOS_FUSED_STATS_UNET", "0") == "1"


def ones_zeros(n, device):
    return None, None


def colsum(act, c_off, C):
    dev = act.t.device
    v = E.view(act, c_off, C)
    nblk = L.lib().sos_bn_stats_blocks(v.npix)
    partial = torch.empty((2, C, nblk), dtype=torch.float32, device=dev)
    L.check(L.lib().sos_bn_stats(ctypes.byref(v), L.ptr(partial), L.stream_ptr()), "sos_bn_stats")
    out = torch.empty(C, dtype=torch.float32, device=dev)
    scratch = torch.empty((2, C), dtype=torch.float32, device=dev)
    L.check(L.lib().sos_bn_finalize(L.ptr(partial), nblk, C, 1, None, None, 1.0, 0.0, None, None, None, L.ptr(scratch[0]),
                                    L.ptr(scratch[1]), L.ptr(out), None, L.stream_ptr()), "sos_bn_finalize(colsum)")
    return E.cur_gs().unscale(out)


def pack_grad(g, y, act, outer, inner, C, so, st, sc, dst, c_off=0, scaled=False):
    v = E.view(dst, c_off, C)
    mul = None if scaled else E.cur_gs().mul
    L.check(L.lib().sos_pack_grad_f32(L.ptr(g), L.ptr(y), act, outer, inner, C, so, st, sc, ctypes.byref(v),
                                      L.ptr(mul), L.stream_ptr()), "sos_pack_grad_f32")


def bn_bwd(dy, dy_off, raw, raw_off, C, saved, gamma, act, slope, dx, dx_off=0):
    dev = raw.t.device
    dyv, xv, dxv = E.view(dy, dy_off, C), E.view(raw, raw_off, C), E.view(dx, dx_off, C)
    nblk = L.lib().sos_bn_stats_blocks(xv.npix)
    partial = torch.empty((3, C, nblk), dtype=torch.float32, device=dev)
    coef = torch.empty((4, C), dtype=torch.float32, device=dev)
    dgamma = torch.empty(C, dtype=torch.float32, device=dev)
    dbeta = torch.empty(C, dtype=torch.float32, device=dev)
    dslope = torch.empty(1, dtype=torch.float32, device=dev) if slope is not None else None
    L.check(L.lib().sos_bn_bwd(ctypes.byref(dyv), ctypes.byref(xv), L.ptr(saved["scale"]), L.ptr(saved["shift"]),
                               L.ptr(saved.get("mean")), L.ptr(saved.get("invstd")), L.ptr(gamma), act, L.ptr(slope),
                               L.ptr(partial), L.ptr(coef), L.ptr(dgamma), L.ptr(dbeta), L.ptr(dslope), ctypes.byref(dxv),
                               L.ptr(E.cur_gs().inv), L.stream_ptr()), "sos_bn_bwd")
    return dgamma, dbeta, dslope


def act_bwd_from_y(dy, y, act, dz, C):
    a, b, c = E.view(dy, 0, C), E.view(y, 0, C), E.view(dz, 0, C)
    L.check(L.lib().sos_act_bwd_from_y(ctypes.byref(a), ctypes.byref(b), act, ctypes.byref(c), L.stream_ptr()),
            "sos_act_bwd_from_y")


def dgrad_weight(w, x3):
    return E.pack_weight(lambda: w.detach().float().flip(2, 3).transpose(0, 1).contiguous(), E.pad_to(w.shape[0], 16), x3)


WGRAD_SIDE = os.environ.get("SOS_WGRAD_SIDE", "0") == "1"
_SIDE = {}


def _side_stream(dev, cur):
    key = (dev.index, cur.cuda_stream)
    s = _SIDE.get(key)
    if s is None:
        s = _SIDE[key] = torch.cuda.Stream(device=dev)
    return s


def encoder_train_plan(enc, x3):
    plan = []
    for i, blk in enumerate(enc):
        conv, bn = blk.block[0], blk.block[1]
        wf = E.wfold_spec(conv, conv.padding[1], L.PAD_ZERO) if i == 0 else None
        if wf is not None:
            cin_store = E.pad_to(wf["kw"] * wf["I"], 16)
            plan.append(dict(w=E.pack_weight(lambda conv=conv, wf=wf: wf["fold"](conv.weight.detach().float()), cin_store, x3),
                             wd=dgrad_weight(conv.weight, x3), conv=conv, bn=bn, kh=conv.kernel_size[0], kw=1,
                             dil=(conv.dilation[0], 1), pad=(conv.padding[0], 0), cout=conv.out_channels,
                             cin=wf["kw"] * wf["I"], cin_store=cin_store, wtaps=wf["wtaps"], unfold=wf["unfold"],
                             dg=dict(kh=conv.kernel_size[0], kw=conv.kernel_size[1], dil=tuple(conv.dilation),
                                     pad=tuple(conv.padding), cin=conv.in_channels)))
            continue
        cin_store = E.pad_to(conv.in_channels, 16)
        plan.append(dict(w=E.pack_weight(conv.weight, cin_store, x3), wd=dgrad_weight(conv.weight, x3), conv=conv, bn=bn,
                         kh=conv.kernel_size[0], kw=conv.kernel_size[1], dil=tuple(conv.dilation),
                         pad=tuple(conv.padding), cout=conv.out_channels, cin=conv.in_channels, cin_store=cin_store))
    return plan


def encoder_forward_train(plan, a, feat, x3):
    dev = a.t.device
    B, H, W = a.B, a.H, a.W
    tape = []
    cur = a
    for i, lp in enumerate(plan):
        cs = E.pad_to(lp["cout"], 16)
        one, zero = ones_zeros(lp["w"].shape[1], dev)
        raw = E.Act(B, H, W, cs, x3, dev)
        st = E.conv_to_act(cur, 0, lp["cin_store"], lp["w"], lp["kh"], lp["kw"], lp["cout"], one, zero, L.ACT_NONE, raw,
                           cout_store=cs, dil=lp["dil"], pad=lp["pad"], Ho=H, Wo=W, stats_c=lp["cout"] if FUSED_STATS else 0)
        last = i == len(plan) - 1
        y = None if last else E.Act(B, H, W, cs, x3, dev, zero=cs > E.pad_to(lp["cout"], 8))
        saved = E.bn_train(raw, 0, lp["cout"], lp["bn"], L.ACT_RELU, None, y, 0, feat if last else None, stats=st)
        tape.append(dict(inp=cur, raw=raw, saved=saved))
        cur = y
    return tape


def encoder_backward(plan, tape, dy, grads, prefix, x3, need_input_grad=False):
    dev = dy.t.device
    cur = torch.cuda.current_stream(dev)
    side = _side_stream(dev, cur) if (WGRAD_SIDE and type(grads) is dict and not torch.cuda.is_current_stream_capturing()) else None
    gs = E.cur_gs()
    try:
        return _encoder_backward(plan, tape, dy, grads, prefix, x3, need_input_grad, dev, cur, side, gs)
    finally:
        if side is not None:
            cur.wait_stream(side)


def _encoder_backward(plan, tape, dy, grads, prefix, x3, need_input_grad, dev, cur, side, gs):
    for i in range(len(plan) - 1, -1, -1):
        lp, tp = plan[i], tape[i]
        raw = tp["raw"]
        d_raw = E.Act(raw.B, raw.H, raw.W, raw.cs, x3, dev, zero=raw.cs > E.pad_to(lp["cout"], 8))
        dgamma, dbeta, _ = bn_bwd(dy, 0, raw, 0, lp["cout"], tp["saved"], lp["bn"].weight, L.ACT_RELU, None, d_raw)
        grads[f"{prefix}.{i}.block.1.weight"] = dgamma
        grads[f"{prefix}.{i}.block.1.bias"] = dbeta
        dw_shape = (lp["cout"], lp["cin"], lp["kh"], lp["kw"])
        if side is not None and "unfold" not in lp:
            side.wait_stream(cur)
            with torch.cuda.stream(side):
                dw = torch.empty(dw_shape, dtype=torch.float32, device=dev)
                E.wgrad(d_raw, 0, lp["cout"], tp["inp"], 0, lp["cin"], lp["kh"], lp["kw"], dw, dil=lp["dil"], pad=lp["pad"], gs=gs)
            d_raw.t.record_stream(side)
            dw.record_stream(cur)
        else:
            dw = torch.empty(dw_shape, dtype=torch.float32, device=dev)
            E.wgrad(d_raw, 0, lp["cout"], tp["inp"], 0, lp["cin"], lp["kh"], lp["kw"], dw, dil=lp["dil"], pad=lp["pad"],
                    defer="unfold" not in lp and type(grads) is dict)
        grads[f"{prefix}.{i}.block.0.weight"] = lp["unfold"](dw) if "unfold" in lp else dw
        if i == 0 and not need_input_grad:
            break
        inp = tp["inp"]
        d_in = E.Act(inp.B, inp.H, inp.W, inp.cs, x3, dev)
        one, zero = ones_zeros(lp["wd"].shape[1], dev)
        dg = lp.get("dg", lp)
        E.conv_to_act(d_raw, 0, d_raw.cs, lp["wd"], dg["kh"], dg["kw"], dg["cin"], one, zero, L.ACT_NONE, d_in,
                      cout_store=inp.cs, dil=dg["dil"],
                      pad=(dg["dil"][0] * (dg["kh"] - 1) - dg["pad"][0], dg["dil"][1] * (dg["kw"] - 1) - dg["pad"][1]),
                      Ho=inp.H, Wo=inp.W)
        dy = d_in
    return dy


def _phase_dgrad_weights(w2, s, pad, cout_cs, x3):
    O, I, kh, kw = w2.shape
    wt = w2.detach().float().transpose(0, 1)

    def axis(r, k, p):
        k0 = (r + p) % s
        taps = list(range(k0, k, s))
        c = (r + p - k0) // s
        return taps, c

    phases = {}
    for rh in range(s):
        th, ch = axis(rh, kh, pad[0])
        for rw in range(s):
            tw, cw = axis(rw, kw, pad[1])
            if not th or not tw:
                continue
            sub = wt[:, :, th[::-1]][:, :, :, tw[::-1]].contiguous()
            phases[(rh, rw)] = (E.pack_weight(sub, cout_cs, x3), len(th), len(tw), len(th) - 1 - ch, len(tw) - 1 - cw)
    return phases


def video_train_plan(enc, x3):
    from .common_nets import NO_TEMPORAL_TAPS
    plan = []
    for blk in enc:
        conv, bn = blk.block[0], blk.block[1]
        kt, kh, kw = conv.kernel_size
        O, I, s = conv.out_channels, conv.in_channels, conv.stride[1]
        w2 = conv.weight.detach().permute(0, 2, 1, 3, 4).reshape(O, kt * I, kh, kw)
        cin_store = E.pad_to(kt * I, 16)
        pad = (conv.padding[1], conv.padding[2])
        lp = dict(w=E.pack_weight(w2, cin_store, x3), conv=conv, bn=bn, kt=kt, kh=kh, kw=kw, stride=s, pad=pad, cin=I,
                  cout=O, cin_store=cin_store)
        cout_cs = E.pad_to(O, 16)
        lp["native"] = kt > 1 and I % 128 == 0 and O % 16 == 0 and s <= 2 and not NO_TEMPORAL_TAPS
        if lp["native"]:
            w2n = conv.weight.detach().flip(2).permute(2, 0, 1, 3, 4).reshape(kt * O, I, kh, kw)
            if s == 1:
                lp["wd"] = dgrad_weight(w2n, x3)
            else:
                lp["wd_phases"] = _phase_dgrad_weights(w2n, s, pad, kt * cout_cs, x3)
        elif s == 1:
            lp["wd"] = dgrad_weight(w2, x3)
        else:
            lp["wd_phases"] = _phase_dgrad_weights(w2, s, pad, cout_cs, x3)
        plan.append(lp)
    return plan


def video_forward_train(plan, frames, B, T, feat, feat_row, feat_third, feat_c_off, x3):
    dev = frames.t.device
    tape = []
    cur, C = frames, 3
    for lp in plan:
        H, W = cur.H, cur.W
        st = cur
        if lp["native"]:
            st = None
        elif lp["kt"] > 1 or cur.cs != lp["cin_store"]:
            st = E.Act(B * T, H, W, lp["cin_store"], x3, dev)
            L.check(L.lib().sos_time_stack(L.ptr(cur.t), B, T, H * W, C, cur.cs, cur.nseg, lp["kt"], L.ptr(st.t), st.cs,
                                           L.stream_ptr()), "sos_time_stack")
        s = lp["stride"]
        Ho = (H + 2 * lp["pad"][0] - lp["kh"]) // s + 1
        Wo = (W + 2 * lp["pad"][1] - lp["kw"]) // s + 1
        cs = E.pad_to(lp["cout"], 16)
        one, zero = ones_zeros(lp["w"].shape[1], dev)
        raw = E.Act(B * T, Ho, Wo, cs, x3, dev)
        if lp["native"]:
            E.conv_to_act(cur, 0, C, lp["w"], lp["kh"], lp["kw"], lp["cout"], one, zero, L.ACT_NONE, raw,
                          cout_store=cs, stride=s, pad=lp["pad"], Ho=Ho, Wo=Wo, temporal=(T, lp["kt"]))
        else:
            E.conv_to_act(st, 0, lp["cin_store"], lp["w"], lp["kh"], lp["kw"], lp["cout"], one, zero, L.ACT_NONE, raw,
                          cout_store=cs, stride=s, pad=lp["pad"], Ho=Ho, Wo=Wo)
        y = E.Act(B * T, Ho, Wo, cs, x3, dev, zero=cs > E.pad_to(lp["cout"], 8))
        saved = E.bn_train(raw, 0, lp["cout"], lp["bn"], L.ACT_RELU, None, y, 0)
        tape.append(dict(src=cur, src_C=C, stacked=st, raw=raw, saved=saved))
        cur, C = y, lp["cout"]
    L.check(L.lib().sos_spatial_mean(L.ptr(cur.t), B * T, cur.H * cur.W, C, cur.cs, cur.nseg, L.ptr(feat), feat_row,
                                     feat_third, feat_c_off, L.stream_ptr()), "sos_spatial_mean")
    return dict(blocks=tape, out=cur)


def video_backward(plan, tape, dfeat, f_row, f_third, f_c_off, grads, prefix, B, T, x3):
    dev = dfeat.device
    last = tape["out"]
    C = plan[-1]["cout"]
    dy = E.Act(last.B, last.H, last.W, last.cs, x3, dev)
    L.check(L.lib().sos_spatial_mean_bwd(L.ptr(dfeat), B * T, last.H * last.W, C, f_row, f_third, f_c_off, dy.nseg,
                                         L.ptr(dy.t), dy.cs, L.stream_ptr()), "sos_spatial_mean_bwd")
    for i in range(len(plan) - 1, -1, -1):
        lp, tp = plan[i], tape["blocks"][i]
        raw, st = tp["raw"], tp["stacked"]
        d_raw = E.Act(raw.B, raw.H, raw.W, raw.cs, x3, dev, zero=raw.cs > E.pad_to(lp["cout"], 8))
        dgamma, dbeta, _ = bn_bwd(dy, 0, raw, 0, lp["cout"], tp["saved"], lp["bn"].weight, L.ACT_RELU, None, d_raw)
        grads[f"{prefix}.{i}.block.1.weight"], grads[f"{prefix}.{i}.block.1.bias"] = dgamma, dbeta
        kt, I, O = lp["kt"], lp["cin"], lp["cout"]
        dw2 = torch.empty((O, kt * I, lp["kh"], lp["kw"]), dtype=torch.float32, device=dev)
        if lp["native"]:
            src = tp["src"]
            E.wgrad(d_raw, 0, O, src, 0, kt * I, lp["kh"], lp["kw"], dw2, stride=lp["stride"], pad=lp["pad"],
                    temporal=(T, kt, I))
        elif lp["stride"] >= 3:
            sd_, (ph_, pw_) = lp["stride"], lp["pad"]
            xp = torch.nn.functional.pad(st.t, (0, 0, pw_, pw_ + sd_, ph_, ph_ + sd_))
            for a in range(lp["kh"]):
                for b_ in range(lp["kw"]):
                    sub = E.Act(st.B, raw.H, raw.W, st.cs, x3, dev)
                    sub.t.copy_(xp[:, a:a + sd_ * raw.H:sd_, b_:b_ + sd_ * raw.W:sd_, :])
                    dwa = torch.empty((O, kt * I, 1, 1), dtype=torch.float32, device=dev)
                    E.wgrad(d_raw, 0, O, sub, 0, kt * I, 1, 1, dwa)
                    dw2[:, :, a:a + 1, b_:b_ + 1] = dwa
        else:
            E.wgrad(d_raw, 0, O, st, 0, kt * I, lp["kh"], lp["kw"], dw2, stride=lp["stride"], pad=lp["pad"])
        grads[f"{prefix}.{i}.block.0.weight"] = dw2.reshape(O, kt, I, lp["kh"], lp["kw"]).permute(0, 2, 1, 3, 4).contiguous()
        if i == 0:
            break
        if lp["native"]:
            src = tp["src"]
            dx = E.Act(src.B, src.H, src.W, src.cs, x3, dev, zero=lp["stride"] > 1)
            if lp["stride"] == 1:
                one, zero = ones_zeros(lp["wd"].shape[1], dev)
                E.conv_to_act(d_raw, 0, d_raw.cs, lp["wd"], lp["kh"], lp["kw"], I, one, zero, L.ACT_NONE, dx,
                              cout_store=dx.cs, pad=(lp["kh"] - 1 - lp["pad"][0], lp["kw"] - 1 - lp["pad"][1]), Ho=src.H, Wo=src.W,
                              temporal=(T, kt))
            else:
                s = lp["stride"]
                row = dx.nseg * dx.cs
                for (rh, rw), (w, Mh, Mw, ph, pw) in lp["wd_phases"].items():
                    Hp, Wp = (src.H - rh + s - 1) // s, (src.W - rw + s - 1) // s
                    if Hp < 1 or Wp < 1:
                        continue
                    one, zero = ones_zeros(w.shape[1], dev)
                    E.conv(d_raw, 0, d_raw.cs, w, Mh, Mw, I, one, zero, L.ACT_NONE, out=dx.t, out_dtype=dx.dtype_code,
                           sb=dx.H * dx.W * row, sh=s * dx.W * row, sw=s * row, sc=1, cout_store=dx.cs, third=dx.cs,
                           pad=(ph, pw), Ho=Hp, Wo=Wp, out_elem_offset=(rh * dx.W + rw) * row, temporal=(T, kt))
            dy = dx
            continue
        d_st = E.Act(st.B, st.H, st.W, st.cs, x3, dev, zero=lp["stride"] > 1 or st.cs > E.pad_to(kt * I, 8))
        if lp["stride"] == 1:
            one, zero = ones_zeros(lp["wd"].shape[1], dev)
            E.conv_to_act(d_raw, 0, d_raw.cs, lp["wd"], lp["kh"], lp["kw"], kt * I, one, zero, L.ACT_NONE, d_st,
                          cout_store=st.cs, pad=(lp["kh"] - 1 - lp["pad"][0], lp["kw"] - 1 - lp["pad"][1]), Ho=st.H, Wo=st.W)
        else:
            s = lp["stride"]
            row = d_st.nseg * d_st.cs
            for (rh, rw), (w, Mh, Mw, ph, pw) in lp["wd_phases"].items():
                Hp, Wp = (st.H - rh + s - 1) // s, (st.W - rw + s - 1) // s
                if Hp < 1 or Wp < 1:
                    continue
                one, zero = ones_zeros(w.shape[1], dev)
                E.conv(d_raw, 0, d_raw.cs, w, Mh, Mw, kt * I, one, zero, L.ACT_NONE, out=d_st.t, out_dtype=d_st.dtype_code,
                       sb=d_st.H * d_st.W * row, sh=s * d_st.W * row, sw=s * row, sc=1, cout_store=st.cs, third=d_st.cs,
                       pad=(ph, pw), Ho=Hp, Wo=Wp, out_elem_offset=(rh * d_st.W + rw) * row)
        src = tp["src"]
        if st is src:
            dy = d_st
        else:
            dy = E.Act(src.B, src.H, src.W, src.cs, x3, dev)
            L.check(L.lib().sos_time_unstack(L.ptr(d_st.t), B, T, src.H * src.W, tp["src_C"], d_st.cs, d_st.nseg, kt,
                                             L.ptr(dy.t), dy.cs, L.stream_ptr()), "sos_time_unstack")


def gather_ranges(gather_np, W):
    lo = np.searchsorted(gather_np, np.arange(W), side="left").astype(np.int32)
    hi = np.searchsorted(gather_np, np.arange(W), side="right").astype(np.int32)
    return lo, hi


def feat_grad_to_nhwc(dfeat, row, third, c_off, C, B, H, W, Wo, x3, lo=None, hi=None):
    dev = dfeat.device
    out = E.Act(B, H, W, E.pad_to(C, 16), x3, dev, zero=True)
    fv = L.View()
    fv.ptr, fv.npix, fv.row, fv.c_off, fv.C, fv.x3, fv.third = dfeat.data_ptr(), 1, row, c_off, C, (1 if x3 else 0), third
    ov = E.view(out, 0, C)
    L.check(L.lib().sos_feat_to_nhwc(ctypes.byref(fv), B, H, W, Wo, L.ptr(lo), L.ptr(hi), ctypes.byref(ov), L.stream_ptr()),
            "sos_feat_to_nhwc")
    return out


def lstm_train_plan(lstm, cin_store, x3):
    H = lstm.hidden_size
    perm, inv = E.lstm_gate_perm(H, lstm.weight_ih_l0.device)
    w_ih = lambda: torch.cat([lstm.weight_ih_l0, lstm.weight_ih_l0_reverse], dim=0).detach()[perm]
    bias = torch.cat([lstm.bias_ih_l0 + lstm.bias_hh_l0, lstm.bias_ih_l0_reverse + lstm.bias_hh_l0_reverse]).detach()[perm]
    w = E.pack_weight(lambda: w_ih()[:, :, None, None], cin_store, x3)
    wd = E.pack_weight(lambda: w_ih().t().contiguous()[:, :, None, None], E.pad_to(8 * H, 16), x3)
    dev = w.device
    return dict(w=w, wd=wd, wpk=E.lstm_pack(lstm, x3), H=H, I=lstm.input_size, cin_store=cin_store, inv=inv,
                scale=E.pad_vec(torch.ones(8 * H, device=dev), w.shape[1], 1.0), shift=E.pad_vec(bias, w.shape[1]))


def lstm_forward_train(lp, feat_dims, B, T, x3, dev):
    H = lp["H"]
    xproj = torch.empty((B, T, 8 * H), dtype=torch.float32, device=dev)
    E.conv(None, 0, lp["cin_store"], lp["w"], 1, 1, 8 * H, lp["scale"], lp["shift"], L.ACT_NONE, out=xproj,
           out_dtype=L.DT_F32, sb=T * 8 * H, sh=0, sw=8 * H, sc=1, Ho=1, Wo=T, in_dims=feat_dims)
    h = E.Act(B, 1, T, E.pad_to(2 * H, 16), x3, dev, zero=True)
    Bp = (B + 15) // 16 * 16
    gates = torch.empty((Bp, T, 2, 4 * H), dtype=torch.float32, device=dev)
    csave = torch.empty((Bp, T, 2, H), dtype=torch.float32, device=dev)
    E.lstm(xproj, lp["wpk"], B, T, H, h, gates, csave)
    return h, dict(gates=gates, csave=csave, h=h, feat_dims=feat_dims)


def lstm_backward(lp, tape, dh, grads, prefix, B, T, x3, dev):
    H, I = lp["H"], lp["I"]
    dgates = torch.empty((B, T, 2, 4 * H), dtype=torch.float32, device=dev)
    L.check(L.lib().sos_lstm_bidir_bwd(L.ptr(dh.t), dh.nseg * dh.cs, dh.dtype_code, dh.cs, L.ptr(tape["gates"]),
                                       L.ptr(tape["csave"]), L.ptr(lp["wpk"]["bh"]), L.ptr(lp["wpk"]["bl"]), B, T, H, L.ptr(dgates), L.stream_ptr()),
            "sos_lstm_bidir_bwd")
    dga = E.Act(B, 1, T, E.pad_to(8 * H, 16), x3, dev, zero=(8 * H) % 16 != 0)
    pack_grad(dgates, None, L.ACT_NONE, B, T, 8 * H, T * 8 * H, 8 * H, 1, dga, scaled=True)
    inv = lp["inv"]
    db = colsum(dga, 0, 8 * H)[inv]
    grads[f"{prefix}.bias_ih_l0"] = db[:4 * H]
    grads[f"{prefix}.bias_hh_l0"] = db[:4 * H]
    grads[f"{prefix}.bias_ih_l0_reverse"] = db[4 * H:]
    grads[f"{prefix}.bias_hh_l0_reverse"] = db[4 * H:]
    ft, fB, fH, fW, fcs, fnseg = tape["feat_dims"]
    feat_act = E.Act.__new__(E.Act)
    feat_act.t, feat_act.B, feat_act.H, feat_act.W, feat_act.cs, feat_act.x3, feat_act.nseg = ft, fB, 1, fW, fcs, x3, fnseg
    dwih = torch.empty((8 * H, I), dtype=torch.float32, device=dev)
    E.wgrad(dga, 0, 8 * H, feat_act, 0, I, 1, 1, dwih)
    dwih = dwih[inv]
    grads[f"{prefix}.weight_ih_l0"] = dwih[:4 * H]
    grads[f"{prefix}.weight_ih_l0_reverse"] = dwih[4 * H:]
    hact = tape["h"]
    for d, sfx, pad_l in ((0, "", 1), (1, "_reverse", -1)):
        dwhh = torch.empty((4 * H, 2 * H), dtype=torch.float32, device=dev)
        E.wgrad(dga, d * 4 * H, 4 * H, hact, 0, 2 * H, 1, 1, dwhh, pad=(0, pad_l))
        grads[f"{prefix}.weight_hh_l0{sfx}"] = dwhh[inv[:4 * H], d * H:(d + 1) * H]
    nseg = 3 if x3 else 1
    dfeat = torch.empty((B, T, nseg * I), dtype=E.act_dtype(), device=dev)
    one, zero = ones_zeros(lp["wd"].shape[1], dev)
    E.conv(dga, 0, dga.cs, lp["wd"], 1, 1, I, one, zero, L.ACT_NONE, out=dfeat,
           out_dtype=L.DT_BF16X3 if x3 else L.DT_BF16, sb=T * nseg * I, sh=0, sw=nseg * I, sc=1, third=I, Ho=1, Wo=T)
    return dfeat


def linear_train_plan(lin, cin_store, x3):
    w = E.pack_weight(lambda: lin.weight[:, :, None, None], cin_store, x3)
    wd = E.pack_weight(lambda: lin.weight.detach().t().contiguous()[:, :, None, None], E.pad_to(lin.out_features, 16), x3)
    return dict(w=w, wd=wd, lin=lin, cout=lin.out_features, cin=lin.in_features, cin_store=cin_store,
                scale=E.pad_vec(torch.ones(lin.out_features, device=w.device), w.shape[1], 1.0),
                shift=E.pad_vec(lin.bias, w.shape[1]))


def linear_backward(lp, a_in, dz, grads, prefix, x3, dev):
    dw = torch.empty((lp["cout"], lp["cin"]), dtype=torch.float32, device=dev)
    E.wgrad(dz, 0, lp["cout"], a_in, 0, lp["cin"], 1, 1, dw, defer=type(grads) is dict)
    grads[f"{prefix}.weight"] = dw
    grads[f"{prefix}.bias"] = colsum(dz, 0, lp["cout"])
    d_in = E.Act(a_in.B, 1, a_in.W, a_in.cs, x3, dev)
    one, zero = ones_zeros(lp["wd"].shape[1], dev)
    E.conv_to_act(dz, 0, dz.cs, lp["wd"], 1, 1, lp["cin"], one, zero, L.ACT_NONE, d_in, cout_store=a_in.cs, Ho=1,
                  Wo=a_in.W)
    return d_in


def reflect_fold(padded, H, W, pad, dst, dst_off, C, accumulate=True):
    pv, ov = E.view(padded, 0, C), E.view(dst, dst_off, C)
    L.check(L.lib().sos_reflect_fold(ctypes.byref(pv), H, W, pad, ctypes.byref(ov), 1 if accumulate else 0, L.stream_ptr()),
            "sos_reflect_fold")


def copy_crop(src, src_off, dst, dst_off, C):
    sv, dv = E.view(src, src_off, C), E.view(dst, dst_off, C)
    L.check(L.lib().sos_copy_crop(ctypes.byref(sv), src.H, src.W, ctypes.byref(dv), dst.H, dst.W, L.stream_ptr()),
            "sos_copy_crop")


def down_train_plan(blk, x3, in_perm=None, first=False):
    import torch.nn as nn
    conv = blk.block[1]
    has_bn = len(blk.block) > 2 and isinstance(blk.block[2], nn.BatchNorm2d)
    prelu = blk.block[-1] if isinstance(blk.block[-1], nn.PReLU) else None
    k, s, d = conv.kernel_size[0], conv.stride[0], conv.dilation[0]
    cin_store = E.pad_to(conv.in_channels, 16)
    cout_cs = E.pad_to(conv.out_channels, 16)
    wf = lambda: conv.weight.detach().float()
    wperm = lambda: wf() if in_perm is None else wf()[:, in_perm]
    fold = E.wfold_spec(conv, (k - 1) // 2 * d, L.PAD_REFLECT) if (first and in_perm is None) else None
    if fold is not None:
        cin_store = E.pad_to(fold["kw"] * fold["I"], 16)
        return dict(w=E.pack_weight(lambda: fold["fold"](wf()), cin_store, x3), conv=conv, bn=blk.block[2] if has_bn else None,
                    prelu=prelu, k=k, kw=1, stride=s, dil=d, pad=(k - 1) // 2 * d, pad_w=0, cout=conv.out_channels,
                    cin=fold["kw"] * fold["I"], cin_store=cin_store, in_perm=None, wtaps=fold["wtaps"], unfold=fold["unfold"])
    plan = dict(w=E.pack_weight(wf, cin_store, x3, in_perm), conv=conv, bn=blk.block[2] if has_bn else None, prelu=prelu,
                k=k, kw=k, stride=s, dil=d, pad=(k - 1) // 2 * d, pad_w=(k - 1) // 2 * d, cout=conv.out_channels,
                cin=conv.in_channels, cin_store=cin_store, in_perm=in_perm)
    if s == 1:
        plan["wd"] = E.pack_weight(lambda: wperm().flip(2, 3).transpose(0, 1).contiguous(), cout_cs, x3)
    else:
        assert s == 2 and d == 1
        phases = {}
        for ph in (0, 1):
            for pw in (0, 1):
                Mh, Mw = (k + 1 - ph) // 2, (k + 1 - pw) // 2
                a = [ph + 2 * (Mh - 1 - t) for t in range(Mh)]
                b = [pw + 2 * (Mw - 1 - t) for t in range(Mw)]
                sub = lambda a=a, b=b: wperm()[:, :, a][:, :, :, b].transpose(0, 1).contiguous()
                phases[(ph, pw)] = (E.pack_weight(sub, cout_cs, x3), Mh, Mw)
        plan["wd_phases"] = phases
    return plan


def up_train_plan(blk, x3):
    ct, bn, prelu = blk.block[0], blk.block[1], blk.block[2]
    cin_store = E.pad_to(ct.in_channels, 16)
    w = lambda: ct.weight.detach().float()
    taps = {0: [1], 1: [2, 0]}
    phases = {}
    for ph in (0, 1):
        for pw in (0, 1):
            sub = lambda ph=ph, pw=pw: w()[:, :, taps[ph]][:, :, :, taps[pw]].permute(1, 0, 2, 3).contiguous()
            phases[(ph, pw)] = E.pack_weight(sub, cin_store, x3)
    wd = E.pack_weight(w, E.pad_to(ct.out_channels, 16), x3)
    return dict(phases=phases, wd=wd, ct=ct, bn=bn, prelu=prelu, cout=ct.out_channels, cin=ct.in_channels,
                cin_store=cin_store)


def down_forward_train(lp, src, cin_off, dst, c_off, Ho, Wo, x3):
    dev = src.t.device
    cs = E.pad_to(lp["cout"], 16)
    one, zero = ones_zeros(lp["w"].shape[1], dev)
    raw = E.Act(src.B, Ho, Wo, cs, x3, dev)
    st = E.conv_to_act(src, cin_off, lp["cin_store"], lp["w"], lp["k"], lp["kw"], lp["cout"], one, zero, L.ACT_NONE, raw,
                       cout_store=cs, stride=lp["stride"], dil=(lp["dil"], lp["dil"]), pad=(lp["pad"], lp["pad_w"]),
                       pad_mode=L.PAD_REFLECT, Ho=Ho, Wo=Wo, stats_c=lp["cout"] if (FUSED_STATS and FUSED_STATS_UNET) else 0)
    saved = E.bn_train(raw, 0, lp["cout"], lp["bn"], L.ACT_PRELU, lp["prelu"].weight, dst, c_off, stats=st)
    return dict(kind="down", lp=lp, src=src, cin_off=cin_off, dst=dst, c_off=c_off, raw=raw, saved=saved)


def up_forward_train(lp, src, dst, c_off, x3):
    dev = src.t.device
    cs = E.pad_to(lp["cout"], 16)
    raw = E.Act(src.B, 2 * src.H, 2 * src.W, cs, x3, dev, zero=cs > lp["cout"])
    row = raw.nseg * raw.cs
    for (ph, pw), w in lp["phases"].items():
        one, zero = ones_zeros(w.shape[1], dev)
        E.conv(src, 0, lp["cin_store"], w, 1 + ph, 1 + pw, lp["cout"], one, zero, L.ACT_NONE, out=raw.t,
               out_dtype=raw.dtype_code, sb=raw.H * raw.W * row, sh=2 * raw.W * row, sw=2 * row, sc=1,
               cout_store=lp["cout"], third=raw.cs, Ho=src.H, Wo=src.W, out_elem_offset=(ph * raw.W + pw) * row)
    if (dst.H, dst.W) == (raw.H, raw.W):
        saved = E.bn_train(raw, 0, lp["cout"], lp["bn"], L.ACT_PRELU, lp["prelu"].weight, dst, c_off)
    else:
        yfull = E.Act(raw.B, raw.H, raw.W, cs, x3, dev, zero=cs > E.pad_to(lp["cout"], 8))
        saved = E.bn_train(raw, 0, lp["cout"], lp["bn"], L.ACT_PRELU, lp["prelu"].weight, yfull, 0)
        copy_crop(yfull, 0, dst, c_off, lp["cout"])
    return dict(kind="up", lp=lp, src=src, dst=dst, c_off=c_off, raw=raw, saved=saved)


class GradBufs:

    def __init__(self, x3):
        self.x3, self.bufs, self.written = x3, {}, {}

    def of(self, act):
        k = id(act)
        if k not in self.bufs:
            self.bufs[k] = E.Act(act.B, act.H, act.W, act.cs, self.x3, act.t.device)
        return self.bufs[k]

    def _zero(self, act, lo, hi):
        g = self.of(act)
        g.t.view(g.B, g.H, g.W, g.nseg, g.cs)[..., lo:hi].zero_()

    def first_write(self, act, c_off, C):
        iv = self.written.setdefault(id(act), [])
        lo, hi = c_off, c_off + C
        hit = [(max(a, lo), min(b, hi)) for a, b in iv if a < hi and lo < b]
        fresh = not hit
        if hit:
            pos = lo
            for a, b in sorted(hit):
                if a > pos:
                    self._zero(act, pos, a)
                pos = max(pos, b)
            if pos < hi:
                self._zero(act, pos, hi)
        iv.append((lo, hi))
        return fresh

    def read(self, act, c_off, C):
        iv = self.written.setdefault(id(act), [])
        lo, hi = c_off, c_off + C
        pos = lo
        for a, b in sorted((max(a, lo), min(b, hi)) for a, b in iv if a < hi and lo < b):
            if a > pos:
                self._zero(act, pos, a)
            pos = max(pos, b)
        if pos < hi:
            self._zero(act, pos, hi)
            iv.append((lo, hi))
        return self.of(act)


def reflect_fold_border(padded, H, W, pad, dst, dst_off, C):
    pv, ov = E.view(padded, 0, C), E.view(dst, dst_off, C)
    L.check(L.lib().sos_reflect_fold_border(ctypes.byref(pv), H, W, pad, ctypes.byref(ov), L.stream_ptr()), "sos_reflect_fold_border")


FOLD_FUSED = os.environ.get("SOS_FOLD_FUSED", "1") != "0"


def _reflect_dgrad(lp, d_raw, src, cin_off, gb, x3):
    dev = d_raw.t.device
    p, k, d = lp["pad"], lp["k"], lp["dil"]
    H, W = src.H, src.W
    cin_cs = E.pad_to(lp["cin"], 16)
    fused = FOLD_FUSED and lp["cin"] % 8 == 0 and p > 0
    dst = gb.of(src)
    accumulate = not gb.first_write(src, cin_off, lp["cin"])
    if not fused and not accumulate and lp["cin"] % 8:
        gb._zero(src, cin_off, cin_off + lp["cin"])
        accumulate = True
    dpad = E.Act(src.B, H + 2 * p, W + 2 * p, cin_cs, x3, dev, zero=(lp["stride"] != 1 and not fused))
    drow = dst.nseg * dst.cs
    if lp["stride"] == 1:
        one, zero = ones_zeros(lp["wd"].shape[1], dev)
        if fused:
            E.conv(d_raw, 0, d_raw.cs, lp["wd"], k, k, lp["cin"], one, zero, L.ACT_NONE, out=dst.t, out_dtype=dst.dtype_code,
                   sb=H * W * drow, sh=0, sw=drow, sc=1, c_off=cin_off, cout_store=lp["cin"], third=dst.cs, dil=(d, d),
                   pad=((k - 1) * d, (k - 1) * d), Ho=dpad.H, Wo=dpad.W, accumulate=accumulate, fold=(dpad, p, H, W, 1, 0, 1, 0))
        else:
            E.conv_to_act(d_raw, 0, d_raw.cs, lp["wd"], k, k, lp["cin"], one, zero, L.ACT_NONE, dpad, cout_store=cin_cs,
                          dil=(d, d), pad=((k - 1) * d, (k - 1) * d), Ho=dpad.H, Wo=dpad.W)
    else:
        row = dpad.nseg * dpad.cs
        for (ph, pw), (w, Mh, Mw) in lp["wd_phases"].items():
            Ho, Wo = (dpad.H - ph + 1) // 2, (dpad.W - pw + 1) // 2
            one, zero = ones_zeros(w.shape[1], dev)
            if fused:
                E.conv(d_raw, 0, d_raw.cs, w, Mh, Mw, lp["cin"], one, zero, L.ACT_NONE, out=dst.t, out_dtype=dst.dtype_code,
                       sb=H * W * drow, sh=0, sw=drow, sc=1, c_off=cin_off, cout_store=lp["cin"], third=dst.cs,
                       pad=(Mh - 1, Mw - 1), Ho=Ho, Wo=Wo, accumulate=accumulate, fold=(dpad, p, H, W, 2, ph, 2, pw))
            else:
                E.conv(d_raw, 0, d_raw.cs, w, Mh, Mw, lp["cin"], one, zero, L.ACT_NONE, out=dpad.t, out_dtype=dpad.dtype_code,
                       sb=dpad.H * dpad.W * row, sh=2 * dpad.W * row, sw=2 * row, sc=1, cout_store=cin_cs, third=dpad.cs,
                       pad=(Mh - 1, Mw - 1), Ho=Ho, Wo=Wo, out_elem_offset=(ph * dpad.W + pw) * row)
    if fused:
        reflect_fold_border(dpad, H, W, p, dst, cin_off, lp["cin"])
    else:
        reflect_fold(dpad, H, W, p, dst, cin_off, lp["cin"], accumulate=accumulate)


_INV_PERM = {}


def down_backward(t, gb, grads, name, x3, need_src_grad=True):
    lp, raw = t["lp"], t["raw"]
    dev = raw.t.device
    d_raw = E.Act(raw.B, raw.H, raw.W, raw.cs, x3, dev, zero=raw.cs > E.pad_to(lp["cout"], 8))
    dgamma, dbeta, dslope = bn_bwd(gb.read(t["dst"], t["c_off"], lp["cout"]), t["c_off"], raw, 0, lp["cout"], t["saved"],
                                   lp["bn"].weight, L.ACT_PRELU, lp["prelu"].weight, d_raw)
    grads[f"{name}.block.2.weight"], grads[f"{name}.block.2.bias"], grads[f"{name}.block.3.weight"] = dgamma, dbeta, dslope
    dw = torch.empty((lp["cout"], lp["cin"], lp["k"], lp["kw"]), dtype=torch.float32, device=dev)
    E.wgrad(d_raw, 0, lp["cout"], t["src"], t["cin_off"], lp["cin"], lp["k"], lp["kw"], dw, stride=lp["stride"],
            dil=(lp["dil"], lp["dil"]), pad=(lp["pad"], lp["pad_w"]), pad_mode=L.PAD_REFLECT,
            defer="unfold" not in lp and lp["in_perm"] is None and type(grads) is dict)
    if "unfold" in lp:
        dw = lp["unfold"](dw)
    if lp["in_perm"] is not None:
        key = (tuple(lp["in_perm"]), str(dw.device))
        inv = _INV_PERM.get(key)
        if inv is None:
            inv = torch.empty(len(lp["in_perm"]), dtype=torch.long)
            inv[torch.tensor(lp["in_perm"])] = torch.arange(len(lp["in_perm"]))
            inv = _INV_PERM[key] = inv.to(dw.device)
        dw = dw[:, inv].contiguous()
    grads[f"{name}.block.1.weight"] = dw
    if need_src_grad:
        if "unfold" in lp:
            raise RuntimeError("down_backward: a block planned with first=True (folded horizontal taps) has no input gradient")
        _reflect_dgrad(lp, d_raw, t["src"], t["cin_off"], gb, x3)


def up_backward(t, gb, grads, name, x3):
    lp, raw, src = t["lp"], t["raw"], t["src"]
    dev = raw.t.device
    gdst = gb.read(t["dst"], t["c_off"], lp["cout"])
    if (gdst.H, gdst.W) == (raw.H, raw.W):
        dy_full, dy_off = gdst, t["c_off"]
    else:
        dy_full, dy_off = E.Act(raw.B, raw.H, raw.W, raw.cs, x3, dev, zero=raw.cs > E.pad_to(lp["cout"], 8)), 0
        copy_crop(gdst, t["c_off"], dy_full, 0, lp["cout"])
    d_raw = E.Act(raw.B, raw.H, raw.W, raw.cs, x3, dev, zero=raw.cs > E.pad_to(lp["cout"], 8))
    dgamma, dbeta, dslope = bn_bwd(dy_full, dy_off, raw, 0, lp["cout"], t["saved"], lp["bn"].weight, L.ACT_PRELU,
                                   lp["prelu"].weight, d_raw)
    grads[f"{name}.block.1.weight"], grads[f"{name}.block.1.bias"], grads[f"{name}.block.2.weight"] = dgamma, dbeta, dslope
    dw = torch.empty_like(lp["ct"].weight, dtype=torch.float32)
    E.wgrad(src, 0, lp["cin"], d_raw, 0, lp["cout"], 3, 3, dw, stride=2, pad=(1, 1), defer=type(grads) is dict)
    grads[f"{name}.block.0.weight"] = dw
    gsrc = gb.of(src)
    one, zero = ones_zeros(lp["wd"].shape[1], dev)
    E.conv_to_act(d_raw, 0, d_raw.cs, lp["wd"], 3, 3, lp["cin"], one, zero, L.ACT_NONE, gsrc, cout_store=lp["cin"],
                  stride=2, pad=(1, 1), Ho=src.H, Wo=src.W, accumulate=not gb.first_write(src, 0, lp["cin"]))
```

Baseline: 562.2.

## Scatter backward gradients into the optimizer's flat buffer with one gather kernel

Backward gradient buffers now come from one persistent workspace. It is recorded on the first pass, verified, then reused. A single multi-tensor HIP kernel copies or gathers (through precomputed index tables for permuted or sliced grads) directly into the fused Adam flat gradient buffer. This replaces per-parameter torch allocations, index/slice ops and the foreach_copy in the optimizer, cutting many small kernel launches and allocations per step. It adds a record/verify state machine and relies on the backward pass keeping the same allocation sequence. It also caches a ones vector for scale vectors.

```diff
diff --git a/include/sos_hip.h b/include/sos_hip.h
--- a/include/sos_hip.h
+++ b/include/sos_hip.h
@@ -194,6 +194,10 @@
 int sos_gather_pack_multi(const sos_pack_entry* entries, int n_entries, const int32_t* chunks, int64_t n_chunks,
                           sos_stream_t stream);
 
+typedef struct sos_scatter_entry { const int64_t* idx; const float* src; float* dst; int64_t n; } sos_scatter_entry;
+int sos_grad_scatter_multi(const sos_scatter_entry* entries, int n_entries, const int32_t* chunks, int64_t n_chunks,
+                           sos_stream_t stream);
+
 int sos_reflect_fold(const sos_view* padded, int H, int W, int pad, const sos_view* out, int accumulate,
                      sos_stream_t stream);
 int sos_reflect_fold_border(const sos_view* padded, int H, int W, int pad, const sos_view* out, sos_stream_t stream);
diff --git a/listening-to-sound-of-silence-for-speech-denoising_amd/_lib.py b/listening-to-sound-of-silence-for-speech-denoising_amd/_lib.py
--- a/listening-to-sound-of-silence-for-speech-denoising_amd/_lib.py
+++ b/listening-to-sound-of-silence-for-speech-denoising_amd/_lib.py
@@ -102,6 +102,7 @@
     "sos_adam_step": [_P, _P, _P, _P, _L, _F, _F, _F, _F, _F, _L, _F, _P, _P],
     "sos_adam_multi_step": [_P, _I, _P, _L, _F, _F, _F, _F, _F, _L, _F, _P, _P],
     "sos_gather_pack_multi": [_P, _I, _P, _L, _P],
+    "sos_grad_scatter_multi": [_P, _I, _P, _L, _P],
     "sos_amax_f32": [_P, _L, _P, _P],
     "sos_loss_scale": [_P, _F, _P, _P, _P],
     "sos_scale_f32": [_P, _L, _P, _P],
diff --git a/listening-to-sound-of-silence-for-speech-denoising_amd/agent.py b/listening-to-sound-of-silence-for-speech-denoising_amd/agent.py
--- a/listening-to-sound-of-silence-for-speech-denoising_amd/agent.py
+++ b/listening-to-sound-of-silence-for-speech-denoising_amd/agent.py
@@ -5,6 +5,7 @@
 
 from . import _lib as L
 from . import transform
+from . import engine as E
 from .engine import bump_version
 
 PHASE_TRAINING, PHASE_TESTING = "training", "testing"
@@ -111,6 +112,13 @@
                                           tab=torch.tensor(rows, dtype=torch.int64, device=dev),
                                           chunks=torch.tensor(chunks, dtype=torch.int32, device=dev))
         return ent
+
+    def flat_grad_views(self, params):
+        ent = self._tables.get(0)
+        if len(self.param_groups) != 1 or ent is None or ent["n"] != len(params) or any(not self.state.get(p) for p in params):
+            return None
+        key = tuple((p.data_ptr(), self.state[p]["exp_avg"].data_ptr(), self.state[p]["exp_avg_sq"].data_ptr()) for p in params)
+        return (ent["views"], ent["flat_g"]) if ent["key"] == key else None
 
     @torch.no_grad()
     def step(self, closure=None):
@@ -131,7 +139,8 @@
                         self._skip_base[p] = self.guard[3:4].clone()
                 st["step"] += 1
             ent = self._table(gi, ps)
-            torch._foreach_copy_(ent["views"], [p.grad.reshape(-1) for p in ps])
+            if any(p.grad.data_ptr() != v.data_ptr() for p, v in zip(ps, ent["views"])):
+                torch._foreach_copy_(ent["views"], [p.grad.reshape(-1) for p in ps])
             work.append((group, ps, ent))
         skip = None
         if self.guard is not None and work:
@@ -455,11 +464,19 @@
             ag.backward_gate = gate
         elif gate is not None:
             ag.stream.wait_event(gate)
+        scatter = (E.GRAD_SCATTER and net is not None and getattr(ag, "bucketer", None) is None
+                   and isinstance(getattr(ag, "optimizer", None), FusedAdam) and getattr(net, "grad_sink_factory", 0) is None)
+        if scatter:
+            if ag.__dict__.get("_gscatter") is None or ag._gscatter.net is not net:
+                ag._gscatter = E.GradScatter(net, ag.optimizer.flat_grad_views)
+            net.grad_sink_factory = ag._gscatter.begin
         try:
             with torch.cuda.stream(ag.stream):
                 outs.append(ag.train_func(data))
         finally:
             ag.backward_gate = None
+            if scatter:
+                net.grad_sink_factory = None
             if k == 0 and gate is not None:
                 net.after_stage2_backward = None
                 net.before_lstm_forward = None
diff --git a/listening-to-sound-of-silence-for-speech-denoising_amd/common_nets.py b/listening-to-sound-of-silence-for-speech-denoising_amd/common_nets.py
--- a/listening-to-sound-of-silence-for-speech-denoising_amd/common_nets.py
+++ b/listening-to-sound-of-silence-for-speech-denoising_amd/common_nets.py
@@ -156,7 +156,7 @@
     w_ih = torch.cat([lstm.weight_ih_l0, lstm.weight_ih_l0_reverse], dim=0).detach()[perm]
     bias = torch.cat([lstm.bias_ih_l0 + lstm.bias_hh_l0, lstm.bias_ih_l0_reverse + lstm.bias_hh_l0_reverse]).detach()[perm]
     w = E.pack_weight(w_ih[:, :, None, None], cin_store, x3)
-    return dict(w=w, scale=E.pad_vec(torch.ones(8 * H, device=w.device), w.shape[1], 1.0),
+    return dict(w=w, scale=E.ones_vec(w.shape[1], w.device),
                 shift=E.pad_vec(bias, w.shape[1]), wpk=E.lstm_pack(lstm, x3), H=H, cin_store=cin_store)
 
 
@@ -173,7 +173,7 @@
 def linear_plan(lin, cin_store, x3, absolute=False):
     wt, bias = (lin.weight.abs(), lin.bias.abs()) if absolute else (lin.weight, lin.bias)
     w = E.pack_weight(wt[:, :, None, None], cin_store, x3)
-    return dict(w=w, scale=E.pad_vec(torch.ones(lin.out_features, device=w.device), w.shape[1], 1.0),
+    return dict(w=w, scale=E.ones_vec(w.shape[1], w.device),
                 shift=E.pad_vec(bias, w.shape[1]), cout=lin.out_features, cin_store=cin_store)
 
 
diff --git a/listening-to-sound-of-silence-for-speech-denoising_amd/csrc/train.hip b/listening-to-sound-of-silence-for-speech-denoising_amd/csrc/train.hip
--- a/listening-to-sound-of-silence-for-speech-denoising_amd/csrc/train.hip
+++ b/listening-to-sound-of-silence-for-speech-denoising_amd/csrc/train.hip
@@ -264,3 +264,45 @@
                        (const PackEntry*)entries, (const int2*)chunks);
     return sos_check_launch("sos_gather_pack_multi");
 }
+
+
+struct ScatterEntry { const long long* idx; const float* src; float* dst; long long n; };
+__global__ __launch_bounds__(256) void grad_scatter_kernel(const ScatterEntry* __restrict__ tab, const int2* __restrict__ chunks) {
+    const int2 c = chunks[blockIdx.x];
+    const ScatterEntry e = tab[c.x];
+    const long long lo = (long long)c.y * SOS_ADAM_CHUNK;
+    const long long hi = lo + SOS_ADAM_CHUNK < e.n ? lo + SOS_ADAM_CHUNK : e.n;
+    if (!e.idx) {
+        for (long long i0 = lo + threadIdx.x; i0 < hi; i0 += 4 * 256) {
+            float v[4];
+#pragma unroll
+            for (int u = 0; u < 4; ++u) v[u] = i0 + u * 256 < hi ? e.src[i0 + u * 256] : 0.f;
+#pragma unroll
+            for (int u = 0; u < 4; ++u)
+                if (i0 + u * 256 < hi) e.dst[i0 + u * 256] = v[u];
+        }
+        return;
+    }
+    for (long long i0 = lo + threadIdx.x; i0 < hi; i0 += 4 * 256) {
+        long long a[4];
+        float v[4];
+#pragma unroll
+        for (int u = 0; u < 4; ++u) a[u] = i0 + u * 256 < hi ? e.idx[i0 + u * 256] : 0;
+#pragma unroll
+        for (int u = 0; u < 4; ++u) v[u] = a[u] ? *(const float*)a[u] : 0.f;
+#pragma unroll
+        for (int u = 0; u < 4; ++u)
+            if (i0 + u * 256 < hi) e.dst[i0 + u * 256] = v[u];
+    }
+}
+extern "C" int sos_grad_scatter_multi(const sos_scatter_entry* entries, int n_entries, const int32_t* chunks, int64_t n_chunks,
+                                      sos_stream_t stream) {
+    static_assert(sizeof(sos_scatter_entry) == sizeof(ScatterEntry), "sos_scatter_entry layout");
+    if (!entries || !chunks || n_entries < 1 || n_chunks < 1 || n_chunks > 0x7fffffff) {
+        sos_set_error("sos_grad_scatter_multi: bad args");
+        return SOS_EINVAL;
+    }
+    hipLaunchKernelGGL(grad_scatter_kernel, dim3((unsigned)n_chunks), dim3(256), 0, (hipStream_t)stream,
+                       (const ScatterEntry*)entries, (const int2*)chunks);
+    return sos_check_launch("sos_grad_scatter_multi");
+}
diff --git a/listening-to-sound-of-silence-for-speech-denoising_amd/denoiser/networks.py b/listening-to-sound-of-silence-for-speech-denoising_amd/denoiser/networks.py
--- a/listening-to-sound-of-silence-for-speech-denoising_amd/denoiser/networks.py
+++ b/listening-to-sound-of-silence-for-speech-denoising_amd/denoiser/networks.py
@@ -57,7 +57,7 @@
     if has_bn:
         scale, shift = E.fold_bn(blk.block[2], w.shape[1])
     else:
-        scale = E.pad_vec(torch.ones(conv.out_channels, device=w.device), w.shape[1], 1.0)
+        scale = E.ones_vec(w.shape[1], w.device)
         shift = E.pad_vec(conv.bias, w.shape[1])
     prelu = blk.block[-1] if isinstance(blk.block[-1], nn.PReLU) else None
     k = conv.kernel_size[0]
@@ -233,8 +233,8 @@
         gb = TO.GradBufs(x3)
         u64 = tape["u64"]
         grads[f"{prefix}.up2.1.block.1.bias"] = TO.colsum(d_out, 0, 2)
-        dw = torch.empty((2, 64, 3, 3), dtype=torch.float32, device=dev)
-        E.wgrad(d_out, 0, 2, u64, 0, 64, 3, 3, dw, pad=(1, 1), pad_mode=L.PAD_REFLECT, defer=type(grads) is dict)
+        dw = E.galloc((2, 64, 3, 3), dev)
+        E.wgrad(d_out, 0, 2, u64, 0, 64, 3, 3, dw, pad=(1, 1), pad_mode=L.PAD_REFLECT, defer=E.local_sink(grads))
         grads[f"{prefix}.up2.1.block.1.weight"] = dw
         last = dict(wd=plan["up2_1_wd"], pad=1, k=3, dil=1, stride=1, cin=64)
         TO._reflect_dgrad(last, d_out, u64, 0, gb, x3)
@@ -399,12 +399,13 @@
 
     @staticmethod
     def backward(ctx, g_npred, g_out):
-        with E.deferred_reductions():
-            grads = ctx.net._backward(ctx.tape, g_npred, g_out)
+        try:
+            with E.deferred_reductions():
+                grads = ctx.net._backward(ctx.tape, g_npred, g_out)
+        finally:
+            E.close_grad_pass()
         ctx.tape = None
-        if getattr(ctx.net, "grad_sink_factory", None) is not None:
-            return (None, None, None) + (None,) * len(list(ctx.net.parameters()))
-        return (None, None, None) + tuple(grads[name].reshape(p.shape) for name, p in ctx.net.named_parameters())
+        return E.deliver_grads(ctx.net, grads, 3)
 
 
 class JointModel(nn.Module):
diff --git a/listening-to-sound-of-silence-for-speech-denoising_amd/detector/networks.py b/listening-to-sound-of-silence-for-speech-denoising_amd/detector/networks.py
--- a/listening-to-sound-of-silence-for-speech-denoising_amd/detector/networks.py
+++ b/listening-to-sound-of-silence-for-speech-denoising_amd/detector/networks.py
@@ -25,12 +25,13 @@
 
     @staticmethod
     def backward(ctx, g):
-        with E.deferred_reductions():
-            grads = ctx.net._backward(ctx.tape, g)
+        try:
+            with E.deferred_reductions():
+                grads = ctx.net._backward(ctx.tape, g)
+        finally:
+            E.close_grad_pass()
         ctx.tape = None
-        if getattr(ctx.net, "grad_sink_factory", None) is not None:
-            return (None, None, None, None) + (None,) * len(list(ctx.net.parameters()))
-        return (None, None, None, None) + tuple(grads[name].reshape(p.shape) for name, p in ctx.net.named_parameters())
+        return E.deliver_grads(ctx.net, grads, 4)
 
 
 class AudioVisualNet(nn.Module):
diff --git a/listening-to-sound-of-silence-for-speech-denoising_amd/engine.py b/listening-to-sound-of-silence-for-speech-denoising_amd/engine.py
--- a/listening-to-sound-of-silence-for-speech-denoising_amd/engine.py
+++ b/listening-to-sound-of-silence-for-speech-denoising_amd/engine.py
@@ -313,10 +313,204 @@
         return plan
 
 
+GRAD_SCATTER = _os.environ.get("SOS_GRAD_SCATTER", "1") != "0"
+
+
+def galloc(shape, device):
+    ws = getattr(_TLS, "grad_ws", None)
+    if ws is not None:
+        return ws.alloc(tuple(shape), device)
+    return torch.empty(tuple(shape), dtype=torch.float32, device=device)
+
+
+def local_sink(grads):
+    return type(grads) is dict or isinstance(grads, _ScatterSink)
+
+
+def close_grad_pass():
+    _TLS.grad_ws = None
+
+
+def deliver_grads(net, grads, n_inputs):
+    params = list(net.named_parameters())
+    finish = getattr(grads, "finish", None)
+    owned = finish() if finish is not None else getattr(net, "grad_sink_factory", None) is not None
+    if owned:
+        return (None,) * (n_inputs + len(params))
+    return (None,) * n_inputs + tuple(grads[name].reshape(p.shape) for name, p in params)
+
+
+def put_grad(grads, name, src, post=None):
+    put = getattr(grads, "put", None)
+    if put is not None:
+        put(name, src, post)
+    else:
+        grads[name] = src if post is None else post(src)
+
+
+class _ScatterSink(dict):
+
+    def __init__(self, gs, state):
+        super().__init__()
+        self.gs, self.state, self.k, self.allocs, self.puts = gs, state, 0, [], []
+
+    def alloc(self, shape, device):
+        gs = self.gs
+        if self.state == "record":
+            t = torch.empty(shape, dtype=torch.float32, device=device)
+            self.allocs.append(t)
+            return t
+        n = 1
+        for d in shape:
+            n *= int(d)
+        device = torch.device(device)
+        if (self.k >= len(gs.slots) or gs.slots[self.k][1] != n or device.type != gs.W.device.type
+                or device.index not in (None, gs.W.device.index)):
+            raise RuntimeError("GradScatter: the backward pass changed its sequence of gradient buffers")
+        off = gs.slots[self.k][0]
+        self.k += 1
+        return gs.W[off:off + n].view(shape)
+
+    def put(self, name, src, post):
+        if self.state == "on":
+            self.puts.append(name)
+            return
+        self.puts.append((name, src, post))
+        dict.__setitem__(self, name, src if post is None else post(src))
+
+    def __setitem__(self, name, v):
+        self.put(name, v, None)
+
+    def finish(self):
+        _TLS.grad_ws = None
+        return self.gs._finish(self)
+
+
+class GradScatter:
+
+    def __init__(self, net, flat_views):
+        self.net, self.flat_views = net, flat_views
+        self.state, self.rec, self.W, self.slots = "record", None, None, None
+
+    def begin(self):
+        params = list(self.net.parameters())
+        state = self.state
+        if not GRAD_SCATTER or any(p.grad is not None for p in params):
+            state = "off"
+        elif state == "record" and self.rec is not None:
+            self._build()
+            state = self.state
+        elif state in ("verify", "on"):
+            if state == "verify" and self.verdict is not None and self.verdict[1].query():
+                self.state = state = "off" if int(self.verdict[0][0]) else "on"
+                self.verdict = None
+            fv = self.flat_views(self.params)
+            if fv is None or fv[1].data_ptr() != self.flat.data_ptr():
+                self.state = state = "record"
+        sink = _ScatterSink(self, state)
+        _TLS.grad_ws = sink if state != "off" else None
+        return sink
+
+    def _build(self):
+        allocs, puts = self.rec
+        self.rec = None
+        self.state = "off"
+        names = [n for n, _, _ in puts]
+        named = dict(self.net.named_parameters())
+        if not puts or len(set(names)) != len(names) or any(n not in named for n in names):
+            return
+        self.params = [p for n, p in named.items() if n in set(names)]
+        fv = self.flat_views(self.params)
+        if fv is None:
+            self.state = "record"
+            return
+        views, self.flat = fv
+        view_of = {id(p): v for p, v in zip(self.params, views)}
+        dev = self.flat.device
+        slot_of, slots, total = {}, [], 0
+        for k, t in enumerate(allocs):
+            slot_of[t.data_ptr()] = k
+            slots.append((total, t.numel()))
+            total += (t.numel() + 63) // 64 * 64
+        W = torch.empty(max(total, 1), dtype=torch.float32, device=dev)
+        ids = torch.arange(1, total + 1, dtype=torch.int64, device=dev)
+        rows, chunks, tabs = [], [], []
+        for name, src, post in puts:
+            k = slot_of.get(src.data_ptr())
+            p = named[name]
+            if k is None or slots[k][1] != src.numel() or not src.is_contiguous() or src.dtype != torch.float32:
+                return
+            off, n = slots[k]
+            if post is None:
+                if n != p.numel():
+                    return
+                rows.append([0, W.data_ptr() + 4 * off, view_of[id(p)].data_ptr(), n])
+            else:
+                m = post(ids[off:off + n].view(src.shape)).reshape(-1)
+                if m.numel() != p.numel() or m.dtype != torch.int64:
+                    return
+                addr = (W.data_ptr() + 4 * (m - 1)).contiguous()
+                tabs.append(addr)
+                rows.append([addr.data_ptr(), 0, view_of[id(p)].data_ptr(), p.numel()])
+            chunks += [[len(rows) - 1, c] for c in range((p.numel() + L.ADAM_CHUNK - 1) // L.ADAM_CHUNK)]
+        self.W, self.slots, self.tabs, self.names = W, slots, tabs, names
+        self.pviews = [(named[n], view_of[id(named[n])].view(named[n].shape)) for n in names]
+        self.table = upload(rows, torch.int64, dev)
+        self.chunks = upload(chunks, torch.int32, dev)
+        self.n, self.nchunks = len(rows), len(chunks)
+        self.state, self.verdict = "verify", None
+
+    def scatter(self):
+        L.check(L.lib().sos_grad_scatter_multi(L.ptr(self.table), self.n, L.ptr(self.chunks), self.nchunks, L.stream_ptr()),
+                "sos_grad_scatter_multi")
+
+    def _finish(self, sink):
+        if sink.state == "off":
+            return False
+        if sink.state == "record":
+            self.rec = (sink.allocs, sink.puts)
+            return False
+        if sink.state == "verify":
+            if [n for n, _, _ in sink.puts] != self.names or sink.k != len(self.slots):
+                self.state = "off"
+                return False
+            torch._foreach_copy_([v.reshape(-1) for _, v in self.pviews], [sink[n].reshape(-1) for n in self.names])
+            keep = self.flat.clone()
+            self.flat.fill_(float("nan"))
+            self.scatter()
+            bad = (self.flat.view(torch.int32) != keep.view(torch.int32)).any().to(torch.int32).reshape(1)
+            self.flat.copy_(keep)
+            if self.verdict is None:
+                host = torch.empty(1, dtype=torch.int32, pin_memory=True)
+                host.copy_(bad, non_blocking=True)
+                done = torch.cuda.Event()
+                done.record()
+                self.verdict = (host, done)
+        else:
+            if sink.puts != self.names or sink.k != len(self.slots):
+                raise RuntimeError("GradScatter: the backward pass changed its sequence of parameter gradients")
+            self.scatter()
+        for p, v in self.pviews:
+            p.grad = v
+        return True
+
+
 def pad_vec(v, n, fill=0.0):
     out = torch.full((n,), fill, dtype=torch.float32, device=v.device)
     out[:v.numel()] = v.detach().float().reshape(-1)
     return out
+
+
+_ONES = {}
+
+
+def ones_vec(n, device):
+    key = (int(n), str(device))
+    if torch.device(device).type == "cuda" and torch.cuda.is_current_stream_capturing():
+        return torch.ones(n, dtype=torch.float32, device=device)
+    if key not in _ONES:
+        _ONES[key] = torch.ones(n, dtype=torch.float32, device=device)
+    return _ONES[key]
 
 
 def fold_bn(bn, cout_pad):
@@ -421,6 +615,18 @@
 
 
 def lstm_gate_perm(H, device):
+    key = (int(H), str(device))
+    if torch.device(device).type == "cuda" and torch.cuda.is_current_stream_capturing():
+        return _lstm_gate_perm(H, device)
+    if key not in _GATE_PERM:
+        _GATE_PERM[key] = _lstm_gate_perm(H, device)
+    return _GATE_PERM[key]
+
+
+_GATE_PERM = {}
+
+
+def _lstm_gate_perm(H, device):
     n = torch.arange(8 * H, device=device)
     d, r = n // (4 * H), n % (4 * H)
     perm = d * 4 * H + (r % 4) * H + r // 4
diff --git a/listening-to-sound-of-silence-for-speech-denoising_amd/train_ops.py b/listening-to-sound-of-silence-for-speech-denoising_amd/train_ops.py
--- a/listening-to-sound-of-silence-for-speech-denoising_amd/train_ops.py
+++ b/listening-to-sound-of-silence-for-speech-denoising_amd/train_ops.py
@@ -24,7 +24,7 @@
     nblk = L.lib().sos_bn_stats_blocks(v.npix)
     partial = torch.empty((2, C, nblk), dtype=torch.float32, device=dev)
     L.check(L.lib().sos_bn_stats(ctypes.byref(v), L.ptr(partial), L.stream_ptr()), "sos_bn_stats")
-    out = torch.empty(C, dtype=torch.float32, device=dev)
+    out = E.galloc((C,), dev)
     scratch = torch.empty((2, C), dtype=torch.float32, device=dev)
     L.check(L.lib().sos_bn_finalize(L.ptr(partial), nblk, C, 1, None, None, 1.0, 0.0, None, None, None, L.ptr(scratch[0]),
                                     L.ptr(scratch[1]), L.ptr(out), None, L.stream_ptr()), "sos_bn_finalize(colsum)")
@@ -44,9 +44,9 @@
     nblk = L.lib().sos_bn_stats_blocks(xv.npix)
     partial = torch.empty((3, C, nblk), dtype=torch.float32, device=dev)
     coef = torch.empty((4, C), dtype=torch.float32, device=dev)
-    dgamma = torch.empty(C, dtype=torch.float32, device=dev)
-    dbeta = torch.empty(C, dtype=torch.float32, device=dev)
-    dslope = torch.empty(1, dtype=torch.float32, device=dev) if slope is not None else None
+    dgamma = E.galloc((C,), dev)
+    dbeta = E.galloc((C,), dev)
+    dslope = E.galloc((1,), dev) if slope is not None else None
     L.check(L.lib().sos_bn_bwd(ctypes.byref(dyv), ctypes.byref(xv), L.ptr(saved["scale"]), L.ptr(saved["shift"]),
                                L.ptr(saved.get("mean")), L.ptr(saved.get("invstd")), L.ptr(gamma), act, L.ptr(slope),
                                L.ptr(partial), L.ptr(coef), L.ptr(dgamma), L.ptr(dbeta), L.ptr(dslope), ctypes.byref(dxv),
@@ -119,7 +119,7 @@
 def encoder_backward(plan, tape, dy, grads, prefix, x3, need_input_grad=False):
     dev = dy.t.device
     cur = torch.cuda.current_stream(dev)
-    side = _side_stream(dev, cur) if (WGRAD_SIDE and type(grads) is dict and not torch.cuda.is_current_stream_capturing()) else None
+    side = _side_stream(dev, cur) if (WGRAD_SIDE and E.local_sink(grads) and not torch.cuda.is_current_stream_capturing()) else None
     gs = E.cur_gs()
     try:
         return _encoder_backward(plan, tape, dy, grads, prefix, x3, need_input_grad, dev, cur, side, gs)
@@ -140,15 +140,15 @@
         if side is not None and "unfold" not in lp:
             side.wait_stream(cur)
             with torch.cuda.stream(side):
-                dw = torch.empty(dw_shape, dtype=torch.float32, device=dev)
+                dw = E.galloc(dw_shape, dev)
                 E.wgrad(d_raw, 0, lp["cout"], tp["inp"], 0, lp["cin"], lp["kh"], lp["kw"], dw, dil=lp["dil"], pad=lp["pad"], gs=gs)
             d_raw.t.record_stream(side)
             dw.record_stream(cur)
         else:
-            dw = torch.empty(dw_shape, dtype=torch.float32, device=dev)
+            dw = E.galloc(dw_shape, dev)
             E.wgrad(d_raw, 0, lp["cout"], tp["inp"], 0, lp["cin"], lp["kh"], lp["kw"], dw, dil=lp["dil"], pad=lp["pad"],
-                    defer="unfold" not in lp and type(grads) is dict)
-        grads[f"{prefix}.{i}.block.0.weight"] = lp["unfold"](dw) if "unfold" in lp else dw
+                    defer="unfold" not in lp and E.local_sink(grads))
+        E.put_grad(grads, f"{prefix}.{i}.block.0.weight", dw, lp.get("unfold"))
         if i == 0 and not need_input_grad:
             break
         inp = tp["inp"]
@@ -353,7 +353,7 @@
     wd = E.pack_weight(lambda: w_ih().t().contiguous()[:, :, None, None], E.pad_to(8 * H, 16), x3)
     dev = w.device
     return dict(w=w, wd=wd, wpk=E.lstm_pack(lstm, x3), H=H, I=lstm.input_size, cin_store=cin_store, inv=inv,
-                scale=E.pad_vec(torch.ones(8 * H, device=dev), w.shape[1], 1.0), shift=E.pad_vec(bias, w.shape[1]))
+                scale=E.ones_vec(w.shape[1], w.device), shift=E.pad_vec(bias, w.shape[1]))
 
 
 def lstm_forward_train(lp, feat_dims, B, T, x3, dev):
@@ -378,24 +378,32 @@
     dga = E.Act(B, 1, T, E.pad_to(8 * H, 16), x3, dev, zero=(8 * H) % 16 != 0)
     pack_grad(dgates, None, L.ACT_NONE, B, T, 8 * H, T * 8 * H, 8 * H, 1, dga, scaled=True)
     inv = lp["inv"]
-    db = colsum(dga, 0, 8 * H)[inv]
-    grads[f"{prefix}.bias_ih_l0"] = db[:4 * H]
-    grads[f"{prefix}.bias_hh_l0"] = db[:4 * H]
-    grads[f"{prefix}.bias_ih_l0_reverse"] = db[4 * H:]
-    grads[f"{prefix}.bias_hh_l0_reverse"] = db[4 * H:]
+    db = colsum(dga, 0, 8 * H)
+    done = {}
+
+    def torch_rows(t):
+        r = done.get(t.data_ptr())
+        if r is None:
+            r = done[t.data_ptr()] = t[inv]
+        return r
+
+    fwd_rows, rev_rows = (lambda t: torch_rows(t)[:4 * H]), (lambda t: torch_rows(t)[4 * H:])
+    E.put_grad(grads, f"{prefix}.bias_ih_l0", db, fwd_rows)
+    E.put_grad(grads, f"{prefix}.bias_hh_l0", db, lambda t: fwd_rows(t).clone())
+    E.put_grad(grads, f"{prefix}.bias_ih_l0_reverse", db, rev_rows)
+    E.put_grad(grads, f"{prefix}.bias_hh_l0_reverse", db, lambda t: rev_rows(t).clone())
     ft, fB, fH, fW, fcs, fnseg = tape["feat_dims"]
     feat_act = E.Act.__new__(E.Act)
     feat_act.t, feat_act.B, feat_act.H, feat_act.W, feat_act.cs, feat_act.x3, feat_act.nseg = ft, fB, 1, fW, fcs, x3, fnseg
-    dwih = torch.empty((8 * H, I), dtype=torch.float32, device=dev)
+    dwih = E.galloc((8 * H, I), dev)
     E.wgrad(dga, 0, 8 * H, feat_act, 0, I, 1, 1, dwih)
-    dwih = dwih[inv]
-    grads[f"{prefix}.weight_ih_l0"] = dwih[:4 * H]
-    grads[f"{prefix}.weight_ih_l0_reverse"] = dwih[4 * H:]
+    E.put_grad(grads, f"{prefix}.weight_ih_l0", dwih, fwd_rows)
+    E.put_grad(grads, f"{prefix}.weight_ih_l0_reverse", dwih, rev_rows)
     hact = tape["h"]
     for d, sfx, pad_l in ((0, "", 1), (1, "_reverse", -1)):
-        dwhh = torch.empty((4 * H, 2 * H), dtype=torch.float32, device=dev)
+        dwhh = E.galloc((4 * H, 2 * H), dev)
         E.wgrad(dga, d * 4 * H, 4 * H, hact, 0, 2 * H, 1, 1, dwhh, pad=(0, pad_l))
-        grads[f"{prefix}.weight_hh_l0{sfx}"] = dwhh[inv[:4 * H], d * H:(d + 1) * H]
+        E.put_grad(grads, f"{prefix}.weight_hh_l0{sfx}", dwhh, lambda t, d=d: t[inv[:4 * H], d * H:(d + 1) * H])
     nseg = 3 if x3 else 1
     dfeat = torch.empty((B, T, nseg * I), dtype=E.act_dtype(), device=dev)
     one, zero = ones_zeros(lp["wd"].shape[1], dev)
@@ -408,13 +416,13 @@
     w = E.pack_weight(lambda: lin.weight[:, :, None, None], cin_store, x3)
     wd = E.pack_weight(lambda: lin.weight.detach().t().contiguous()[:, :, None, None], E.pad_to(lin.out_features, 16), x3)
     return dict(w=w, wd=wd, lin=lin, cout=lin.out_features, cin=lin.in_features, cin_store=cin_store,
-                scale=E.pad_vec(torch.ones(lin.out_features, device=w.device), w.shape[1], 1.0),
+                scale=E.ones_vec(w.shape[1], w.device),
                 shift=E.pad_vec(lin.bias, w.shape[1]))
 
 
 def linear_backward(lp, a_in, dz, grads, prefix, x3, dev):
-    dw = torch.empty((lp["cout"], lp["cin"]), dtype=torch.float32, device=dev)
-    E.wgrad(dz, 0, lp["cout"], a_in, 0, lp["cin"], 1, 1, dw, defer=type(grads) is dict)
+    dw = E.galloc((lp["cout"], lp["cin"]), dev)
+    E.wgrad(dz, 0, lp["cout"], a_in, 0, lp["cin"], 1, 1, dw, defer=E.local_sink(grads))
     grads[f"{prefix}.weight"] = dw
     grads[f"{prefix}.bias"] = colsum(dz, 0, lp["cout"])
     d_in = E.Act(a_in.B, 1, a_in.W, a_in.cs, x3, dev)
@@ -621,12 +629,11 @@
     dgamma, dbeta, dslope = bn_bwd(gb.read(t["dst"], t["c_off"], lp["cout"]), t["c_off"], raw, 0, lp["cout"], t["saved"],
                                    lp["bn"].weight, L.ACT_PRELU, lp["prelu"].weight, d_raw)
     grads[f"{name}.block.2.weight"], grads[f"{name}.block.2.bias"], grads[f"{name}.block.3.weight"] = dgamma, dbeta, dslope
-    dw = torch.empty((lp["cout"], lp["cin"], lp["k"], lp["kw"]), dtype=torch.float32, device=dev)
+    dw = E.galloc((lp["cout"], lp["cin"], lp["k"], lp["kw"]), dev)
     E.wgrad(d_raw, 0, lp["cout"], t["src"], t["cin_off"], lp["cin"], lp["k"], lp["kw"], dw, stride=lp["stride"],
             dil=(lp["dil"], lp["dil"]), pad=(lp["pad"], lp["pad_w"]), pad_mode=L.PAD_REFLECT,
-            defer="unfold" not in lp and lp["in_perm"] is None and type(grads) is dict)
-    if "unfold" in lp:
-        dw = lp["unfold"](dw)
+            defer="unfold" not in lp and lp["in_perm"] is None and E.local_sink(grads))
+    post = lp.get("unfold")
     if lp["in_perm"] is not None:
         key = (tuple(lp["in_perm"]), str(dw.device))
         inv = _INV_PERM.get(key)
@@ -634,8 +641,9 @@
             inv = torch.empty(len(lp["in_perm"]), dtype=torch.long)
             inv[torch.tensor(lp["in_perm"])] = torch.arange(len(lp["in_perm"]))
             inv = _INV_PERM[key] = inv.to(dw.device)
-        dw = dw[:, inv].contiguous()
-    grads[f"{name}.block.1.weight"] = dw
+        unfold = post
+        post = lambda t: (t if unfold is None else unfold(t))[:, inv].contiguous()
+    E.put_grad(grads, f"{name}.block.1.weight", dw, post)
     if need_src_grad:
         if "unfold" in lp:
             raise RuntimeError("down_backward: a block planned with first=True (folded horizontal taps) has no input gradient")
@@ -655,8 +663,8 @@
     dgamma, dbeta, dslope = bn_bwd(dy_full, dy_off, raw, 0, lp["cout"], t["saved"], lp["bn"].weight, L.ACT_PRELU,
                                    lp["prelu"].weight, d_raw)
     grads[f"{name}.block.1.weight"], grads[f"{name}.block.1.bias"], grads[f"{name}.block.2.weight"] = dgamma, dbeta, dslope
-    dw = torch.empty_like(lp["ct"].weight, dtype=torch.float32)
-    E.wgrad(src, 0, lp["cin"], d_raw, 0, lp["cout"], 3, 3, dw, stride=2, pad=(1, 1), defer=type(grads) is dict)
+    dw = E.galloc(lp["ct"].weight.shape, dev)
+    E.wgrad(src, 0, lp["cin"], d_raw, 0, lp["cout"], 3, 3, dw, stride=2, pad=(1, 1), defer=E.local_sink(grads))
     grads[f"{name}.block.0.weight"] = dw
     gsrc = gb.of(src)
     one, zero = ones_zeros(lp["wd"].shape[1], dev)
```

New measurement: 562.9 (median of 2 runs). About the same (+0.1%).
